# torognes/vsearch

Measured on AMD Instinct MI355X. Metric: GCUPS (useful DP cells/s of the search16 global-alignment path: DP + traceback + CIGAR), higher is better.
Workload: dtype int16

## Files before the change

include/vsx.h:

```cpp
#ifndef VSX_H
#define VSX_H

#include <stddef.h>
#include <stdint.h>

#ifdef __cplusplus
extern "C" {
#endif

#define VSX_API_VERSION 1000
#define VSX_SCORE_SENTINEL 32767

#define VSX_OK         0
#define VSX_EINVAL    -1
#define VSX_ENODEVICE -2
#define VSX_ENOMEM    -3
#define VSX_EHIP      -4

typedef struct vsx_ctx vsx_ctx;
typedef struct vsx_seqset vsx_seqset;
typedef struct vsx_plan vsx_plan;

typedef struct vsx_scoring {
  int64_t match;
  int64_t mismatch;
  int64_t gap_open_query_left;
  int64_t gap_open_target_left;
  int64_t gap_open_query_interior;
  int64_t gap_open_target_interior;
  int64_t gap_open_query_right;
  int64_t gap_open_target_right;
  int64_t gap_ext_query_left;
  int64_t gap_ext_target_left;
  int64_t gap_ext_query_interior;
  int64_t gap_ext_target_interior;
  int64_t gap_ext_query_right;
  int64_t gap_ext_target_right;
  int32_t n_mismatch;
} vsx_scoring;

typedef struct vsx_results {
  uint64_t   n_pairs;
  int16_t  * score;
  uint16_t * aligned;
  uint16_t * matches;
  uint16_t * mismatches;
  uint16_t * gaps;
  uint64_t * cigar_off;
  char     * cigar_blob;
  uint64_t   cigar_bytes;
  uint8_t  * verdict;
} vsx_results;

#define VSX_VERDICT_UNDECIDED 0
#define VSX_VERDICT_ACCEPTED  1
#define VSX_VERDICT_WEAK      2
#define VSX_VERDICT_REJECTED  3
typedef struct vsx_filter {
  int32_t iddef;
  int32_t leftjust, rightjust;
  int32_t pad;
  double  id, weak_id, maxid, mid, query_cov, target_cov;
  int64_t maxsubs, maxgaps, mincols, maxdiffs;
} vsx_filter;
int vsx_plan_set_filter(vsx_plan * plan, const vsx_filter * f);

typedef struct vsx_timing {
  float    forward_ms;
  float    traceback_ms;
  float    total_ms;
  uint32_t forward_launches;
  uint32_t traceback_launches;
  uint64_t cells;
  uint64_t dir_bytes;
} vsx_timing;

typedef struct vsx_plan_info {
  uint64_t tasks;
  uint64_t tasks_tilted;
  uint64_t tasks_tracked;
  uint32_t rows_dominant;
  uint32_t chunks;
  uint64_t tasks_max3;
  uint64_t tasks_sparse;
  uint64_t waves;
  uint64_t tasks_pair;
} vsx_plan_info;

const char * vsx_version_string(void);
int vsx_device_count(void);
const char * vsx_last_error(void);

int vsx_create(vsx_ctx ** out, const vsx_scoring * scoring, int device);
void vsx_destroy(vsx_ctx * ctx);


int vsx_seqset_create(vsx_ctx * ctx, vsx_seqset ** out, uint64_t n,
                      const char * blob, uint64_t blob_bytes,
                      const uint64_t * offsets, const uint32_t * lengths);
int vsx_seqset_create_from_device(vsx_ctx * ctx, vsx_seqset ** out, uint64_t n,
                                  const void * d_blob, uint64_t blob_bytes,
                                  const uint64_t * offsets, const uint32_t * lengths);
int vsx_seqset_create_both_strands(vsx_ctx * ctx, vsx_seqset ** out, uint64_t n,
                                   const char * blob, uint64_t blob_bytes,
                                   const uint64_t * offsets, const uint32_t * lengths);
void vsx_seqset_destroy(vsx_seqset * s);
uint64_t vsx_seqset_count(const vsx_seqset * s);

int vsx_plan_create(vsx_ctx * ctx, vsx_plan ** out,
                    const vsx_seqset * queries, const vsx_seqset * targets,
                    uint64_t n_pairs, const uint32_t * qidx, const uint32_t * tidx,
                    uint64_t dir_budget_bytes);
int vsx_plan_run(vsx_plan * plan);
int vsx_plan_sync(vsx_plan * plan, vsx_timing * timing );
int vsx_plan_fetch(vsx_plan * plan, vsx_results * out);
int vsx_plan_describe(const vsx_plan * plan, vsx_plan_info * info);
#define VSX_HIT_RECORD_BYTES 24
int vsx_plan_export_hits(vsx_plan * plan, void * d_dst, uint64_t dst_bytes);
int vsx_plan_export_runs(vsx_plan * plan, void * d_dst, uint64_t dst_bytes, uint64_t * n_runs);
int64_t vsx_cigar_from_runs(const uint32_t * runs, uint32_t n, char * dst, uint64_t cap);
void vsx_plan_destroy(vsx_plan * plan);

int vsx_align_pairs_filtered(vsx_ctx * ctx, const vsx_seqset * queries, const vsx_seqset * targets,
                             uint64_t n_pairs, const uint32_t * qidx, const uint32_t * tidx,
                             const vsx_filter * filter, vsx_results * out);
int vsx_align_pairs(vsx_ctx * ctx, const vsx_seqset * queries, const vsx_seqset * targets,
                    uint64_t n_pairs, const uint32_t * qidx, const uint32_t * tidx,
                    vsx_results * out);
void vsx_results_free(vsx_results * r);

typedef struct vsx_ranked {
  uint64_t   n_pairs, n_hits;
  uint32_t * pair;
  int16_t  * score;
  uint16_t * aligned, * matches, * mismatches, * gaps;
  uint8_t  * verdict;
  double   * id;
  uint64_t * cigar_off;
  char     * cigar_blob;
  uint64_t   cigar_bytes;
  uint64_t   n_undecided;
  uint32_t * undecided;
} vsx_ranked;
int vsx_align_pairs_ranked(vsx_ctx * ctx, const vsx_seqset * queries, const vsx_seqset * targets,
                           uint64_t n_pairs, const uint32_t * qidx, const uint32_t * tidx,
                           const vsx_filter * filter, int keep_weak, vsx_ranked * out);
void vsx_ranked_free(vsx_ranked * r);

#ifdef __cplusplus
}
#endif
#endif
```

profiles/valu_budget.py:

```python
#!/usr/bin/env python3
import argparse
import collections
import os
import re
import shutil
import subprocess
import sys
import tempfile

LLVM = "/opt/rocm/llvm/bin"
ROOT = os.path.dirname(os.path.dirname(os.path.abspath(__file__)))


def mangled(args):
    a = [x.strip() for x in args.split(",")]
    enc = "".join(("Li%sE" % x) if x.lstrip("-").isdigit() else ("Lb%dE" % (x == "true")) for x in a)
    return "_Z18vsx_forward_kernelI" + enc + "Ev12VsxDevParamsPK7VsxTaskPKhS5_PjP15HIP_vector_typeIjLj2EEP10VsxSlotOutj"


def extract(lib, sym, tmp):
    shutil.copy(lib, os.path.join(tmp, "lib.so"))
    subprocess.run([LLVM + "/llvm-objdump", "--offloading", "lib.so"], cwd=tmp, capture_output=True, check=True)
    for f in sorted(os.listdir(tmp)):
        if "gfx950" not in f:
            continue
        p = os.path.join(tmp, f)
        syms = subprocess.run([LLVM + "/llvm-readelf", "-s", "--wide", p], capture_output=True, text=True).stdout
        if (" " + sym + "\n") in syms:
            return p, syms
    sys.exit("kernel %s not found in %s" % (sym, lib))


def meta(syms, sym):
    out = {}
    for k in ("num_vgpr", "numbered_sgpr", "private_seg_size"):
        m = re.search(r"\s([0-9a-f]+)\s+0\s+NOTYPE\s+LOCAL\s+DEFAULT\s+ABS\s+" + re.escape(sym) + r"\." + k + r"\n", syms)
        out[k] = int(m.group(1), 16) if m else None
    m = re.search(r"\s([0-9a-f]+)\s+(\d+)\s+FUNC\s+\S+\s+\S+\s+\S+\s+" + re.escape(sym) + r"\n", syms)
    out["start"], out["size"] = int(m.group(1), 16), int(m.group(2))
    return out


def disasm(co, sym, start):
    txt = subprocess.run([LLVM + "/llvm-objdump", "-d", "--mcpu=gfx950", "--disassemble-symbols=" + sym, co],
                         capture_output=True, text=True, check=True).stdout
    ins = []
    for line in txt.splitlines():
        m = re.match(r"\s+(\S+)\s*(.*?)\s*//\s*([0-9A-F]+):", line)
        if not m:
            continue
        op, rest, addr = m.group(1), m.group(2), int(m.group(3), 16) - start
        t = re.search(r"<" + re.escape(sym) + r"\+0x([0-9a-f]+)>", line)
        ins.append((addr, op, rest, int(t.group(1), 16) if t else None))
    return ins


def is_valu(op):
    return op.startswith("v_")


def category(op, rest):
    if op in ("v_pk_maximum3_f16", "v_pk_max_u16", "v_subrev_u32_e32", "v_sub_u32_e32", "v_subrev_u32_e64", "v_sub_u32_e64"):
        return "row body"
    if op == "v_mov_b32_dpp":
        return "DPP hand-overs (feed, H, F)"
    if op == "v_add_u32_sdwa":
        return "profile row addresses"
    if op in ("v_pk_ashrrev_i16", "v_bfi_b32"):
        return "leave-column tracking"
    if op in ("v_lshl_add_u32", "v_lshlrev_b32_e32", "v_or_b32_e32", "v_and_or_b32") and "s" in rest.split(",")[1]:
        return "feed-slot addresses"
    if op in ("v_lshl_add_u64", "v_add_co_u32_e32", "v_addc_co_u32_e32", "v_mad_u64_u32"):
        return "checkpoint addresses"
    if op == "v_mov_b32_e32":
        return "register copies"
    return None


def budget(body, R, S):
    c = collections.Counter()
    quota = {"v_perm_b32": R * S, "v_add_u32_e32": R * S}
    npk = sum(1 for op, _ in body if op == "v_pk_sub_i16")
    nashr = sum(1 for op, _ in body if op == "v_pk_ashrrev_i16")
    pk = [("row body", S), ("last row's own e / hf subtractions", 2 * S), ("leave-column tracking", nashr)]
    for op, rest in body:
        if not is_valu(op):
            continue
        k = category(op, rest)
        if k is None and op in quota:
            if op == "v_add_u32_e32" and re.search(r"0x(1|2)000(1|2)\b", rest):
                k = "leave-column tracking"
            elif quota[op] > 0:
                quota[op] -= 1
                k = "row body"
            else:
                k = "checkpoint pack" if op == "v_perm_b32" else "other"
        if k is None and op == "v_pk_sub_i16":
            for i, (name, n) in enumerate(pk):
                if n > 0:
                    pk[i] = (name, n - 1)
                    k = name
                    break
            else:
                k = "checkpoint pack"
        c[k or "other"] += 1
    return c, npk


def main():
    ap = argparse.ArgumentParser()
    ap.add_argument("--lib", default=os.path.join(ROOT, "vsearch_amd", "libvsx.so"))
    ap.add_argument("--kernel", default="16,true,false,true,true,true,1,false,true", help="template arguments of vsx_forward_kernel")
    ap.add_argument("--rows", type=int, default=None, help="R (default: the first template argument)")
    ap.add_argument("--loop", type=int, default=None, help="loop index to budget (default: most v_pk_maximum3_f16)")
    ap.add_argument("--ops", action="store_true", help="print the opcode histogram of the loop too")
    a = ap.parse_args()
    R = a.rows or int(a.kernel.split(",")[0])
    sym = mangled(a.kernel)
    tmp = tempfile.mkdtemp(prefix="vsx_budget_")
    try:
        co, syms = extract(a.lib, sym, tmp)
        md = meta(syms, sym)
        ins = disasm(co, sym, md["start"])
    finally:
        shutil.rmtree(tmp, ignore_errors=True)
    print("vsx_forward_kernel<%s>  (%s)" % (a.kernel, os.path.relpath(a.lib, ROOT) if a.lib.startswith(ROOT) else a.lib))
    print("  code %d B, %d instructions, %d VALU;  VGPR %s  SGPR %s  scratch %s B" % (
        md["size"], len(ins), sum(is_valu(op) for _, op, _, _ in ins), md["num_vgpr"], md["numbered_sgpr"], md["private_seg_size"]))
    idx = {addr: k for k, (addr, _, _, _) in enumerate(ins)}
    heads = collections.OrderedDict()
    for k, (addr, op, _, tgt) in enumerate(ins):
        if op.startswith("s_branch") or op.startswith("s_cbranch"):
            if tgt is not None and tgt <= addr and tgt in idx:
                h = idx[tgt]
                heads.setdefault(h, []).append(k)
    loops = []
    for h, bs in heads.items():
        first_back, last = min(bs), max(bs)
        main_path = set(range(h, first_back + 1))
        for k in range(h, first_back + 1):
            addr, op, _, tgt = ins[k]
            if op.startswith("s_cbranch") and tgt is not None and tgt > addr and tgt in idx and idx[tgt] <= first_back + 1:
                for j in range(k + 1, idx[tgt]):
                    main_path.discard(j)
        cond = [j for j in range(h, last + 1) if j not in main_path]
        mp = sorted(main_path)
        loops.append(dict(head=h, end=last, main=mp, cond=cond,
                          max3=sum(1 for j in mp if ins[j][1] == "v_pk_maximum3_f16"),
                          valu_main=sum(1 for j in mp if is_valu(ins[j][1])), valu_cond=sum(1 for j in cond if is_valu(ins[j][1]))))
    print("  loops (offset range: VALU on the always-taken path + in branch-guarded regions, v_pk_maximum3_f16):")
    for n, L in enumerate(loops):
        print("    [%d] +0x%04x..+0x%04x: %4d + %4d VALU, %3d max3" % (n, ins[L["head"]][0], ins[L["end"]][0], L["valu_main"], L["valu_cond"], L["max3"]))
    if not loops:
        return
    n = a.loop if a.loop is not None else max(range(len(loops)), key=lambda i: (loops[i]["max3"], -i))
    L = loops[n]
    S = max(1, round(L["max3"] / R))
    body = [(ins[j][1], ins[j][2]) for j in L["main"]]
    cond = [(ins[j][1], ins[j][2]) for j in L["cond"]]
    cm, _ = budget(body, R, S)
    per_step = L["valu_main"] / S + L["valu_cond"] / 16.0
    print("  loop [%d]: %d steps per iteration (R = %d)" % (n, S, R))
    print("    VALU per two steps, always-taken path: %.1f" % (2.0 * L["valu_main"] / S))
    print("    VALU in branch-guarded regions (once per 16 steps): %d" % L["valu_cond"])
    print("    VALU per 16-step block: %.0f   per step: %.2f   (row body %d per step = %.1f %%)" % (
        16 * per_step, per_step, 6 * R, 100.0 * 6 * R / per_step))
    print("    per step, by category (always-taken path / S, + branch-guarded / 16):")
    order = ["row body", "DPP hand-overs (feed, H, F)", "profile row addresses", "feed-slot addresses", "last row's own e / hf subtractions",
             "leave-column tracking", "checkpoint pack", "checkpoint addresses", "register copies", "other"]
    for k in order:
        v = cm.get(k, 0) / S
        if v:
            print("      %-38s %6.2f" % (k, v))
    if L["valu_cond"]:
        print("      %-38s %6.2f  (%d VALU / 16)" % ("16-step block boundary (guarded)", L["valu_cond"] / 16.0, L["valu_cond"]))
    if a.ops:
        for name, lst in (("always-taken path", body), ("branch-guarded", cond)):
            h = collections.Counter(op for op, _ in lst if is_valu(op))
            print("    %s opcodes: %s" % (name, ", ".join("%s %d" % kv for kv in h.most_common())))


if __name__ == "__main__":
    main()
```

vsearch_amd/_lib.py:

```python
import ctypes as C
import os

HERE = os.path.dirname(os.path.abspath(__file__))
LIB_PATH = os.environ.get("VSX_LIBRARY") or os.path.join(HERE, "libvsx.so")

VSX_OK, VSX_EINVAL, VSX_ENODEVICE, VSX_ENOMEM, VSX_EHIP = 0, -1, -2, -3, -4
SENTINEL = 32767

SYMBOLS = [
    "vsx_version_string", "vsx_device_count", "vsx_last_error", "vsx_create", "vsx_destroy",
    "vsx_seqset_create", "vsx_seqset_create_both_strands", "vsx_seqset_create_from_device", "vsx_seqset_destroy", "vsx_seqset_count",
    "vsx_plan_create", "vsx_plan_run", "vsx_plan_sync", "vsx_plan_fetch", "vsx_plan_export_hits", "vsx_plan_export_runs",
    "vsx_cigar_from_runs", "vsx_plan_destroy",
    "vsx_align_pairs", "vsx_align_pairs_filtered", "vsx_align_pairs_ranked", "vsx_ranked_free", "vsx_plan_set_filter", "vsx_results_free", "vsx_plan_describe",
]
SEARCH_SYMBOLS = ["vsx_search_opts_default", "vsx_searcher_create", "vsx_searcher_destroy", "vsx_searcher_db_text", "vsx_search_batch",
                  "vsx_search_batch_meta", "vsx_searcher_set_meta",
                  "vsx_hits_free", "vsx_search_candidates", "vsx_search_candidates_batch", "vsx_candidates_free", "vsx_lma_align", "vsx_allpairs_block", "vsx_allpairs_rows", "vsx_allpairs_stream", "vsx_cluster_fast", "vsx_cluster_out_free", "vsx_msa", "vsx_msa_out_free",
                  "vsx_msa_device", "vsx_msa_device_batch", "vsx_dust_mask", "vsx_abundance_ratio_cmp",
                  "vsx_multi_searcher_create", "vsx_multi_searcher_destroy", "vsx_multi_searcher_devices", "vsx_multi_searcher_replica",
                  "vsx_multi_search_batch", "vsx_multi_allpairs"]


class Candidates(C.Structure):
    _fields_ = [("n_queries", C.c_uint64), ("start", C.POINTER(C.c_uint64)), ("target", C.POINTER(C.c_uint32)),
                ("count", C.POINTER(C.c_uint32)), ("seconds", C.c_double), ("kernel_ms", C.c_double),
                ("index_build_ms", C.c_double), ("index_postings", C.c_uint64), ("postings_streamed", C.c_uint64),
                ("bytes_streamed", C.c_uint64)]


class SearchOpts(C.Structure):
    _fields_ = [("id", C.c_double), ("weak_id", C.c_double), ("maxaccepts", C.c_int64), ("maxrejects", C.c_int64),
                ("wordlength", C.c_int64), ("minwordmatches", C.c_int64), ("iddef", C.c_int32), ("soft_mask", C.c_int32),
                ("maxsubs", C.c_int64), ("maxgaps", C.c_int64), ("mincols", C.c_int64), ("maxdiffs", C.c_int64),
                ("query_cov", C.c_double), ("target_cov", C.c_double), ("maxid", C.c_double), ("mid", C.c_double),
                ("leftjust", C.c_int32), ("rightjust", C.c_int32),
                ("minqt", C.c_double), ("maxqt", C.c_double), ("minsl", C.c_double), ("maxsl", C.c_double),
                ("idprefix", C.c_int64), ("idsuffix", C.c_int64), ("selfid", C.c_int32), ("threads", C.c_int32),
                ("window", C.c_int64), ("gap_infinite", C.c_uint32), ("strand_both", C.c_uint32),
                ("maxqsize", C.c_int64), ("mintsize", C.c_int64), ("minsizeratio", C.c_double), ("maxsizeratio", C.c_double),
                ("self", C.c_int32), ("sizeorder", C.c_int32), ("cluster_unoise", C.c_int32), ("qmask", C.c_int32),
                ("unoise_alpha", C.c_double), ("hardmask", C.c_int32)]


class SeqMeta(C.Structure):
    _fields_ = [("abundance", C.POINTER(C.c_uint64)), ("label", C.POINTER(C.c_char_p))]


class Hit(C.Structure):
    _fields_ = [("query", C.c_uint32), ("target", C.c_uint32), ("count", C.c_uint32),
                ("accepted", C.c_uint8), ("weak", C.c_uint8), ("used_fallback", C.c_uint8), ("strand", C.c_uint8),
                ("nwscore", C.c_int32), ("nwdiff", C.c_int32), ("nwgaps", C.c_int32), ("nwindels", C.c_int32),
                ("nwalignmentlength", C.c_int32), ("matches", C.c_int32), ("mismatches", C.c_int32),
                ("internal_alignmentlength", C.c_int32), ("internal_gaps", C.c_int32), ("internal_indels", C.c_int32),
                ("trim_q_left", C.c_int32), ("trim_q_right", C.c_int32), ("trim_t_left", C.c_int32), ("trim_t_right", C.c_int32),
                ("shortest", C.c_int32), ("longest", C.c_int32),
                ("nwid", C.c_double), ("id", C.c_double), ("id0", C.c_double), ("id1", C.c_double), ("id2", C.c_double),
                ("id3", C.c_double), ("id4", C.c_double), ("cigar_off", C.c_uint64)]


class Hits(C.Structure):
    _fields_ = [("n_queries", C.c_uint64), ("n_hits", C.c_uint64), ("first", C.POINTER(C.c_uint64)),
                ("hit", C.POINTER(Hit)), ("cigar_blob", C.POINTER(C.c_char)), ("cigar_bytes", C.c_uint64),
                ("pairs_aligned", C.c_uint64), ("cells_aligned", C.c_uint64), ("stages", C.c_uint64),
                ("sentinel_pairs", C.c_uint64), ("seconds_kmer", C.c_double), ("seconds_align", C.c_double),
                ("seconds_total", C.c_double)]


class Scoring(C.Structure):
    _fields_ = [(n, C.c_int64) for n in (
        "match", "mismatch", "gap_open_query_left", "gap_open_target_left", "gap_open_query_interior",
        "gap_open_target_interior", "gap_open_query_right", "gap_open_target_right",
        "gap_ext_query_left", "gap_ext_target_left", "gap_ext_query_interior", "gap_ext_target_interior",
        "gap_ext_query_right", "gap_ext_target_right")] + [("n_mismatch", C.c_int32)]


class Results(C.Structure):
    _fields_ = [("n_pairs", C.c_uint64), ("score", C.POINTER(C.c_int16)), ("aligned", C.POINTER(C.c_uint16)),
                ("matches", C.POINTER(C.c_uint16)), ("mismatches", C.POINTER(C.c_uint16)),
                ("gaps", C.POINTER(C.c_uint16)), ("cigar_off", C.POINTER(C.c_uint64)),
                ("cigar_blob", C.POINTER(C.c_char)), ("cigar_bytes", C.c_uint64), ("verdict", C.POINTER(C.c_uint8))]


class Ranked(C.Structure):
    _fields_ = [("n_pairs", C.c_uint64), ("n_hits", C.c_uint64), ("pair", C.POINTER(C.c_uint32)), ("score", C.POINTER(C.c_int16)),
                ("aligned", C.POINTER(C.c_uint16)), ("matches", C.POINTER(C.c_uint16)), ("mismatches", C.POINTER(C.c_uint16)),
                ("gaps", C.POINTER(C.c_uint16)), ("verdict", C.POINTER(C.c_uint8)), ("id", C.POINTER(C.c_double)),
                ("cigar_off", C.POINTER(C.c_uint64)), ("cigar_blob", C.POINTER(C.c_char)), ("cigar_bytes", C.c_uint64),
                ("n_undecided", C.c_uint64), ("undecided", C.POINTER(C.c_uint32))]


class Filter(C.Structure):
    _fields_ = [("iddef", C.c_int32), ("leftjust", C.c_int32), ("rightjust", C.c_int32), ("pad", C.c_int32),
                ("id", C.c_double), ("weak_id", C.c_double), ("maxid", C.c_double), ("mid", C.c_double),
                ("query_cov", C.c_double), ("target_cov", C.c_double),
                ("maxsubs", C.c_int64), ("maxgaps", C.c_int64), ("mincols", C.c_int64), ("maxdiffs", C.c_int64)]


class PlanInfo(C.Structure):
    _fields_ = [("tasks", C.c_uint64), ("tasks_tilted", C.c_uint64), ("tasks_tracked", C.c_uint64),
                ("rows_dominant", C.c_uint32), ("chunks", C.c_uint32), ("tasks_max3", C.c_uint64),
                ("tasks_sparse", C.c_uint64), ("waves", C.c_uint64), ("tasks_pair", C.c_uint64)]


class Timing(C.Structure):
    _fields_ = [("forward_ms", C.c_float), ("traceback_ms", C.c_float), ("total_ms", C.c_float),
                ("forward_launches", C.c_uint32), ("traceback_launches", C.c_uint32),
                ("cells", C.c_uint64), ("dir_bytes", C.c_uint64)]


class ClusterOut(C.Structure):
    _fields_ = [("n", C.c_uint64), ("n_clusters", C.c_uint64), ("clusterno", C.POINTER(C.c_uint32)), ("hits", Hits)]


class MsaOut(C.Structure):
    _fields_ = [("alnlen", C.c_uint64), ("n_rows", C.c_uint64), ("conslen", C.c_uint64), ("rows", C.POINTER(C.c_char)),
                ("consensus", C.POINTER(C.c_char)), ("profile", C.POINTER(C.c_uint64))]


_lib = None


def load():
    global _lib
    if _lib is not None:
        return _lib
    if not os.path.exists(LIB_PATH):
        raise ImportError(
            f"{LIB_PATH} not found: build the HIP extension first (python -c 'import __graft_entry__ as g; "
            "g.build()' or make -C vsearch_amd/csrc). vsearch_amd has no CPU fallback.")
    lib = C.CDLL(LIB_PATH)
    vp = C.c_void_p
    lib.vsx_version_string.restype = C.c_char_p
    lib.vsx_last_error.restype = C.c_char_p
    lib.vsx_device_count.restype = C.c_int
    lib.vsx_create.argtypes = [C.POINTER(vp), C.POINTER(Scoring), C.c_int]
    lib.vsx_destroy.argtypes = [vp]
    lib.vsx_destroy.restype = None
    lib.vsx_seqset_create.argtypes = [vp, C.POINTER(vp), C.c_uint64, vp, C.c_uint64, vp, vp]
    lib.vsx_seqset_create_both_strands.argtypes = [vp, C.POINTER(vp), C.c_uint64, vp, C.c_uint64, vp, vp]
    lib.vsx_seqset_create_from_device.argtypes = [vp, C.POINTER(vp), C.c_uint64, vp, C.c_uint64, vp, vp]
    lib.vsx_seqset_destroy.argtypes = [vp]
    lib.vsx_seqset_destroy.restype = None
    lib.vsx_seqset_count.argtypes = [vp]
    lib.vsx_seqset_count.restype = C.c_uint64
    lib.vsx_plan_create.argtypes = [vp, C.POINTER(vp), vp, vp, C.c_uint64, vp, vp, C.c_uint64]
    lib.vsx_plan_run.argtypes = [vp]
    lib.vsx_plan_sync.argtypes = [vp, C.POINTER(Timing)]
    lib.vsx_plan_fetch.argtypes = [vp, C.POINTER(Results)]
    lib.vsx_plan_export_hits.argtypes = [vp, vp, C.c_uint64]
    lib.vsx_plan_export_runs.argtypes = [vp, vp, C.c_uint64, C.POINTER(C.c_uint64)]
    lib.vsx_cigar_from_runs.argtypes = [vp, C.c_uint32, vp, C.c_uint64]
    lib.vsx_cigar_from_runs.restype = C.c_int64
    lib.vsx_plan_destroy.argtypes = [vp]
    lib.vsx_plan_destroy.restype = None
    lib.vsx_plan_describe.argtypes = [vp, C.POINTER(PlanInfo)]
    lib.vsx_align_pairs.argtypes = [vp, vp, vp, C.c_uint64, vp, vp, C.POINTER(Results)]
    lib.vsx_align_pairs_filtered.argtypes = [vp, vp, vp, C.c_uint64, vp, vp, C.POINTER(Filter), C.POINTER(Results)]
    lib.vsx_align_pairs_ranked.argtypes = [vp, vp, vp, C.c_uint64, vp, vp, C.POINTER(Filter), C.c_int, C.POINTER(Ranked)]
    lib.vsx_ranked_free.argtypes = [C.POINTER(Ranked)]
    lib.vsx_ranked_free.restype = None
    lib.vsx_plan_set_filter.argtypes = [vp, C.POINTER(Filter)]
    lib.vsx_results_free.argtypes = [C.POINTER(Results)]
    lib.vsx_results_free.restype = None
    lib.vsx_search_opts_default.argtypes = [C.POINTER(SearchOpts)]
    lib.vsx_search_opts_default.restype = None
    lib.vsx_searcher_create.argtypes = [vp, C.POINTER(vp), C.POINTER(SearchOpts), C.c_uint64, vp, C.c_uint64, vp, vp]
    lib.vsx_searcher_destroy.argtypes = [vp]
    lib.vsx_searcher_destroy.restype = None
    lib.vsx_search_batch.argtypes = [vp, C.c_uint64, vp, C.c_uint64, vp, vp, C.POINTER(Hits)]
    lib.vsx_search_batch_meta.argtypes = [vp, C.c_uint64, vp, C.c_uint64, vp, vp, C.POINTER(SeqMeta), C.POINTER(Hits)]
    lib.vsx_searcher_set_meta.argtypes = [vp, C.POINTER(SeqMeta)]
    lib.vsx_hits_free.argtypes = [C.POINTER(Hits)]
    lib.vsx_hits_free.restype = None
    lib.vsx_search_candidates.argtypes = [vp, C.c_char_p, C.c_uint32, vp, vp, C.c_uint64]
    lib.vsx_search_candidates.restype = C.c_int64
    lib.vsx_search_candidates_batch.argtypes = [vp, C.c_int32, C.c_uint64, vp, C.c_uint64, vp, vp, C.POINTER(Candidates)]
    lib.vsx_candidates_free.argtypes = [C.POINTER(Candidates)]
    lib.vsx_candidates_free.restype = None
    lib.vsx_allpairs_block.argtypes = [vp, C.c_int32, C.c_uint64, C.c_uint64, C.POINTER(Hits)]
    lib.vsx_allpairs_rows.argtypes = [vp, C.c_int32, vp, C.c_uint64, C.POINTER(Hits)]
    lib.vsx_allpairs_stream.argtypes = [vp, C.c_int32, C.c_uint64, C.c_uint64, C.c_uint64, vp, vp]
    lib.vsx_dust_mask.argtypes = [vp, C.c_uint64, vp, vp, C.c_int32]
    lib.vsx_multi_searcher_create.argtypes = [C.POINTER(vp), vp, vp, C.c_int32, vp, C.c_uint64, vp, C.c_uint64, vp, vp, vp]
    lib.vsx_multi_searcher_destroy.argtypes = [vp]
    lib.vsx_multi_searcher_destroy.restype = None
    lib.vsx_multi_searcher_devices.argtypes = [vp]
    lib.vsx_multi_searcher_devices.restype = C.c_int32
    lib.vsx_multi_searcher_replica.argtypes = [vp, C.c_int32]
    lib.vsx_multi_searcher_replica.restype = vp
    lib.vsx_multi_search_batch.argtypes = [vp, C.c_uint64, vp, C.c_uint64, vp, vp, vp, C.POINTER(Hits)]
    lib.vsx_multi_allpairs.argtypes = [vp, C.c_int32, C.c_uint64, C.c_uint64, C.POINTER(Hits)]
    lib.vsx_abundance_ratio_cmp.argtypes = [C.c_int64, C.c_double, C.c_int64]
    lib.vsx_abundance_ratio_cmp.restype = C.c_int
    lib.vsx_cluster_fast.argtypes = [vp, C.c_uint64, C.POINTER(ClusterOut)]
    lib.vsx_cluster_out_free.argtypes = [C.POINTER(ClusterOut)]
    lib.vsx_cluster_out_free.restype = None
    lib.vsx_msa.argtypes = [C.c_uint32, vp, vp, vp, vp, C.POINTER(MsaOut)]
    lib.vsx_msa_device.argtypes = [vp, C.c_uint32, vp, vp, vp, vp, C.POINTER(MsaOut)]
    lib.vsx_msa_device_batch.argtypes = [vp, C.c_uint32, vp, vp, vp, vp, vp, C.POINTER(MsaOut)]
    lib.vsx_msa_out_free.argtypes = [C.POINTER(MsaOut)]
    lib.vsx_msa_out_free.restype = None
    lib.vsx_lma_align.argtypes = [C.POINTER(Scoring), C.c_char_p, C.c_uint64, C.c_char_p, C.c_uint64] + \
        [C.POINTER(C.c_int64)] * 5 + [C.POINTER(vp)]
    _lib = lib
    return lib


class VsxError(RuntimeError):
    def __init__(self, code, where):
        msg = load().vsx_last_error().decode(errors="replace")
        super().__init__(f"{where}: error {code}: {msg}")
        self.code = code


def check(code, where):
    if code != VSX_OK:
        raise VsxError(code, where)
```

vsearch_amd/csrc/ubench_valu.hip:

```cpp
#include <hip/hip_runtime.h>
#include <cstdio>
#include <cstdlib>

#define CK(x) do { hipError_t e = (x); if (e != hipSuccess) { fprintf(stderr, "%s:%d %s\n", __FILE__, __LINE__, hipGetErrorString(e)); exit(1); } } while (0)

#define BODY16(INS) \
  asm volatile(INS(%0) INS(%1) INS(%2) INS(%3) INS(%4) INS(%5) INS(%6) INS(%7) \
               INS(%8) INS(%9) INS(%10) INS(%11) INS(%12) INS(%13) INS(%14) INS(%15) \
               : "+v"(r[0]), "+v"(r[1]), "+v"(r[2]), "+v"(r[3]), "+v"(r[4]), "+v"(r[5]), "+v"(r[6]), "+v"(r[7]), \
                 "+v"(r[8]), "+v"(r[9]), "+v"(r[10]), "+v"(r[11]), "+v"(r[12]), "+v"(r[13]), "+v"(r[14]), "+v"(r[15]) \
               : "v"(b), "v"(c) : "vcc")

#define I_PK_ADD(x)   "v_pk_add_i16 " #x ", " #x ", %16 clamp\n"
#define I_PK_SUB(x)   "v_pk_sub_i16 " #x ", " #x ", %16 clamp\n"
#define I_PK_MAX(x)   "v_pk_max_i16 " #x ", " #x ", %16\n"
#define I_PK_MIN(x)   "v_pk_min_u16 " #x ", " #x ", %16\n"
#define I_PK_LSHR(x)  "v_pk_lshrrev_b16 " #x ", 1, " #x "\n"
#define I_PK_ASHR(x)  "v_pk_ashrrev_i16 " #x ", 15, " #x "\n"
#define I_PK_MAD(x)   "v_pk_mad_u16 " #x ", " #x ", %16, %17\n"
#define I_PK_MUL(x)   "v_pk_mul_lo_u16 " #x ", " #x ", %16\n"
#define I_XOR(x)      "v_xor_b32 " #x ", " #x ", %16\n"
#define I_ANDOR(x)    "v_and_or_b32 " #x ", " #x ", %16, %17\n"
#define I_LSHR(x)     "v_lshrrev_b32 " #x ", 1, " #x "\n"
#define I_BFI(x)      "v_bfi_b32 " #x ", %16, " #x ", %17\n"
#define I_LSHLOR(x)   "v_lshl_or_b32 " #x ", " #x ", 1, %16\n"
#define I_ADD32(x)    "v_add_u32 " #x ", " #x ", %16\n"
#define I_ADD3(x)     "v_add3_u32 " #x ", " #x ", %16, %17\n"
#define I_MAX32(x)    "v_max_i32 " #x ", " #x ", %16\n"
#define I_MAX3_32(x)  "v_max3_i32 " #x ", " #x ", %16, %17\n"
#define I_ADD16(x)    "v_add_i16 " #x ", " #x ", %16 clamp\n"
#define I_MAX16(x)    "v_max_i16 " #x ", " #x ", %16\n"
#define I_MAX3_16(x)  "v_max3_i16 " #x ", " #x ", %16, %17\n"
#define I_DPP(x)      "v_mov_b32_dpp " #x ", %16 row_shr:1 row_mask:0xf bank_mask:0xf\n"
#define I_PERM(x)     "v_perm_b32 " #x ", " #x ", %16, %17\n"
#define I_CNDMASK(x)  "v_cndmask_b32 " #x ", " #x ", %16, vcc\n"
#define I_CMP16(x)    "v_cmp_gt_i16 vcc, " #x ", %16\n"
#define I_MOV(x)      "v_mov_b32 " #x ", %16\n"
#define I_ALIGNBIT(x) "v_alignbit_b32 " #x ", " #x ", %16, 1\n"
#define I_DOT2(x)     "v_dot2_u32_u16 " #x ", " #x ", %16, %17\n"
#define I_SAD16(x)    "v_sad_u16 " #x ", " #x ", %16, %17\n"
#define I_MAD_I32_I16(x) "v_mad_i32_i16 " #x ", " #x ", %16, %17\n"

#define I_SUB32(x)    "v_sub_u32 " #x ", " #x ", %16\n"
#define I_SUBREV32(x) "v_subrev_u32 " #x ", " #x ", %16\n"
#define I_MIN32(x)    "v_min_i32 " #x ", " #x ", %16\n"
#define I_MAXU32(x)   "v_max_u32 " #x ", " #x ", %16\n"
#define I_ASHR32(x)   "v_ashrrev_i32 " #x ", 31, " #x "\n"
#define I_AND32(x)    "v_and_b32 " #x ", " #x ", %16\n"
#define I_OR32(x)     "v_or_b32 " #x ", " #x ", %16\n"
#define I_LSHL32(x)   "v_lshlrev_b32 " #x ", 1, " #x "\n"
#define I_ADDCO(x)    "v_add_co_u32 " #x ", vcc, " #x ", %16\n"
#define I_ADDC(x)     "v_addc_co_u32 " #x ", vcc, " #x ", %16, vcc\n"
#define I_MIN16(x)    "v_min_i16 " #x ", " #x ", %16\n"
#define I_ADDU16(x)   "v_add_u16 " #x ", " #x ", %16\n"
#define I_SUBU16(x)   "v_sub_u16 " #x ", " #x ", %16\n"
#define I_CMP32(x)    "v_cmp_lt_i32 vcc, " #x ", %16\n"
#define I_LSHLADD(x)  "v_lshl_add_u32 " #x ", " #x ", 1, %16\n"
#define I_MADU24(x)   "v_mad_u32_u24 " #x ", " #x ", %16, %17\n"
#define I_MULU24(x)   "v_mul_u32_u24 " #x ", " #x ", %16\n"
#define I_SUBI32C(x)  "v_sub_i32 " #x ", " #x ", %16 clamp\n"
#define I_MED3(x)     "v_med3_i32 " #x ", " #x ", %16, %17\n"
#define I_BFE(x)      "v_bfe_u32 " #x ", " #x ", 8, 8\n"
#define I_ADDSDWA(x)  "v_add_u32_sdwa " #x ", " #x ", %16 dst_sel:DWORD dst_unused:UNUSED_PAD src0_sel:DWORD src1_sel:BYTE_1\n"
#define I_MAX16SDWA(x) "v_max_i16_sdwa " #x ", " #x ", %16 dst_sel:WORD_1 dst_unused:UNUSED_PRESERVE src0_sel:WORD_1 src1_sel:WORD_1\n"
#define I_MOVDPP(x)   "v_mov_b32_dpp " #x ", %16 row_ror:15 row_mask:0xf bank_mask:0xf\n"
#define I_ADDDPP(x)   "v_add_u32_dpp " #x ", %16, " #x " row_shr:1 row_mask:0xf bank_mask:0xf\n"
#define I_MOV64(x)    "v_mov_b64 %18, %19\n"
#define I_PKMAX3F(x)  "v_pk_maximum3_f16 " #x ", " #x ", %16, %17\n"
#define I_PKMAXU(x)   "v_pk_max_u16 " #x ", " #x ", %16\n"
#define I_MIXAM(x)    "v_add_u32 " #x ", " #x ", %16\n" "v_pk_max_u16 " #x ", " #x ", %17\n"
#define I_MIXAM3(x)   "v_add_u32 " #x ", " #x ", %16\n" "v_pk_maximum3_f16 " #x ", " #x ", %16, %17\n"

#define DEFK(NAME, INS) \
  __global__ void __launch_bounds__(256) NAME(int iters, int * out, int seed) { \
    int r[16]; int b = seed + threadIdx.x, c = seed * 7 + 3; \
    for (int i = 0; i < 16; ++i) r[i] = i * 1315423911 + threadIdx.x; \
    for (int it = 0; it < iters; ++it) { \
      BODY16(INS); BODY16(INS); BODY16(INS); BODY16(INS); BODY16(INS); BODY16(INS); BODY16(INS); BODY16(INS); } \
    int acc = 0; for (int i = 0; i < 16; ++i) acc ^= r[i]; \
    if (acc == 0x12345678) out[0] = acc; }

DEFK(k_pk_add, I_PK_ADD)
DEFK(k_pk_sub, I_PK_SUB)
DEFK(k_pk_max, I_PK_MAX)
DEFK(k_pk_min, I_PK_MIN)
DEFK(k_pk_lshr, I_PK_LSHR)
DEFK(k_pk_ashr, I_PK_ASHR)
DEFK(k_pk_mad, I_PK_MAD)
DEFK(k_pk_mul, I_PK_MUL)
DEFK(k_xor, I_XOR)
DEFK(k_andor, I_ANDOR)
DEFK(k_lshr, I_LSHR)
DEFK(k_bfi, I_BFI)
DEFK(k_lshlor, I_LSHLOR)
DEFK(k_add32, I_ADD32)
DEFK(k_add3, I_ADD3)
DEFK(k_max32, I_MAX32)
DEFK(k_max3_32, I_MAX3_32)
DEFK(k_add16, I_ADD16)
DEFK(k_max16, I_MAX16)
DEFK(k_max3_16, I_MAX3_16)
DEFK(k_dpp, I_DPP)
DEFK(k_perm, I_PERM)
DEFK(k_cndmask, I_CNDMASK)
DEFK(k_cmp16, I_CMP16)
DEFK(k_mov, I_MOV)
DEFK(k_alignbit, I_ALIGNBIT)
DEFK(k_dot2, I_DOT2)
DEFK(k_sad16, I_SAD16)
DEFK(k_mad_i32_i16, I_MAD_I32_I16)

DEFK(k2_sub32, I_SUB32)
DEFK(k2_subrev32, I_SUBREV32)
DEFK(k2_min32, I_MIN32)
DEFK(k2_maxu32, I_MAXU32)
DEFK(k2_ashr32, I_ASHR32)
DEFK(k2_and32, I_AND32)
DEFK(k2_or32, I_OR32)
DEFK(k2_lshl32, I_LSHL32)
DEFK(k2_addco, I_ADDCO)
DEFK(k2_addc, I_ADDC)
DEFK(k2_min16, I_MIN16)
DEFK(k2_addu16, I_ADDU16)
DEFK(k2_subu16, I_SUBU16)
DEFK(k2_cmp32, I_CMP32)
DEFK(k2_lshladd, I_LSHLADD)
DEFK(k2_madu24, I_MADU24)
DEFK(k2_mulu24, I_MULU24)
DEFK(k2_subi32c, I_SUBI32C)
DEFK(k2_med3, I_MED3)
DEFK(k2_bfe, I_BFE)
DEFK(k2_addsdwa, I_ADDSDWA)
DEFK(k2_max16sdwa, I_MAX16SDWA)
DEFK(k2_movdpp, I_MOVDPP)
DEFK(k2_adddpp, I_ADDDPP)
DEFK(k3_pkmax3f, I_PKMAX3F)
DEFK(k3_pkmaxu, I_PKMAXU)
DEFK(k3_mix_add_max, I_MIXAM)
DEFK(k3_mix_add_max3, I_MIXAM3)

template <int MODE>
__global__ void __launch_bounds__(256) k_rowbody(int iters, int * out, int seed)
{
  typedef unsigned short us2 __attribute__((ext_vector_type(2)));
  auto pmaxu = [](unsigned a, unsigned b) -> unsigned {
    return __builtin_bit_cast(unsigned, __builtin_elementwise_max(__builtin_bit_cast(us2, a), __builtin_bit_cast(us2, b)));
  };
  unsigned H[16], E[16], pa[4], pb[4];
  for (int i = 0; i < 16; ++i) { H[i] = 0x80008000u + (unsigned) (i * 77 + (int) threadIdx.x); E[i] = 0x80008000u - (unsigned) (i * 13 + seed); }
  for (int i = 0; i < 4; ++i) { pa[i] = 0x06000600u + (unsigned) seed * (unsigned) i; pb[i] = 0x00060006u + (unsigned) i; }
  unsigned F = 0x80008000u, diag = 0x80008000u;
  const unsigned go = 0x00120012u;
  for (int it = 0; it < iters; ++it)
    {
      unsigned Hd = diag;
#pragma unroll
      for (int r = 0; r < 16; ++r)
        {
          const unsigned V = __builtin_amdgcn_perm(pb[r >> 2], pa[r >> 2], 0x0C040C00u + 0x00010001u * (unsigned) (r & 3));
          const unsigned h0 = Hd + V;
          if (MODE == 1)
            {
              const unsigned m = pmaxu(h0, E[r]);
              const unsigned mg = m - go;
              const unsigned h2 = pmaxu(m, F);
              F = pmaxu(F, mg);
              Hd = H[r];
              H[r] = h2;
              E[r] = pmaxu(E[r], h2 - go);
            }
          else
            {
              const unsigned Fin = (MODE == 2) ? go + (unsigned) r : F;
              const unsigned h1 = pmaxu(h0, Fin);
              const unsigned h2 = pmaxu(h1, E[r]);
              Hd = H[r];
              H[r] = h2;
              const unsigned he = h2 - go;
              if (MODE == 2) F ^= pmaxu(Fin, he); else F = pmaxu(F, he);
              E[r] = pmaxu(E[r], he);
            }
        }
      diag = H[15] + (unsigned) it;
      pa[it & 3] ^= F;
    }
  unsigned acc = F;
  for (int i = 0; i < 16; ++i) acc ^= H[i] ^ E[i];
  if (acc == 0x12345678u) out[0] = (int) acc;
}

typedef void (*kfn)(int, int *, int);

static void run(const char * name, kfn k, int waves_per_simd)
{
  int * out; CK(hipMalloc(&out, 4));
  const int iters = 1000;
  const int blocks = 256 * waves_per_simd;
  hipEvent_t e0, e1; CK(hipEventCreate(&e0)); CK(hipEventCreate(&e1));
  hipLaunchKernelGGL(k, dim3(blocks), dim3(256), 0, 0, 10, out, 1);
  CK(hipDeviceSynchronize());
  CK(hipEventRecord(e0));
  hipLaunchKernelGGL(k, dim3(blocks), dim3(256), 0, 0, iters, out, 1);
  CK(hipEventRecord(e1));
  CK(hipEventSynchronize(e1));
  float ms; CK(hipEventElapsedTime(&ms, e0, e1));
  double instr = (double) iters * 8 * 16 * blocks * 256;
  double rate = instr / (ms * 1e-3) / 1e12;
  printf("%-22s w/simd=%d %8.3f ms  %7.2f T lane-instr/s  (%.1f lanes/clk/SIMD @2.4GHz)\n", name, waves_per_simd, ms, rate,
         rate * 1e12 / (1024 * 2.4e9));
  CK(hipFree(out));
}

static void run_rowbody(int waves_per_simd, int mode)
{
  int * out; CK(hipMalloc(&out, 4));
  const int iters = 20000;
  const int blocks = 256 * waves_per_simd;
  hipEvent_t e0, e1; CK(hipEventCreate(&e0)); CK(hipEventCreate(&e1));
  auto launch = [&](int n) {
    if (mode == 0) hipLaunchKernelGGL(k_rowbody<0>, dim3(blocks), dim3(256), 0, 0, n, out, 1);
    if (mode == 1) hipLaunchKernelGGL(k_rowbody<1>, dim3(blocks), dim3(256), 0, 0, n, out, 1);
    if (mode == 2) hipLaunchKernelGGL(k_rowbody<2>, dim3(blocks), dim3(256), 0, 0, n, out, 1);
  };
  launch(10);
  CK(hipDeviceSynchronize());
  CK(hipEventRecord(e0));
  launch(iters);
  CK(hipEventRecord(e1));
  CK(hipEventSynchronize(e1));
  float ms; CK(hipEventElapsedTime(&ms, e0, e1));
  const int per_row = (mode == 1) ? 8 : ((mode == 2) ? 8 : 7);
  const double wave_instr_per_simd = (double) iters * 16 * per_row * waves_per_simd;
  const double cycles = ms * 1e-3 * 2.4e9;
  const char * what[] = {"kernel row body, F chain of 4 per row (perm, add, 2 max, sub, 2 max)", "F chain of 1 per row (perm, add, max, sub, 2 max, sub, max)",
                         "no chain (+1 xor per row)"};
  printf("%-70s x 16 rows  w/simd=%d %8.3f ms  %.3f cycles per instruction  %.1f cycles per lane-row\n",
         what[mode], waves_per_simd, ms, cycles / wave_instr_per_simd, per_row * cycles / wave_instr_per_simd);
  CK(hipFree(out));
}

int main()
{
  hipDeviceProp_t p; CK(hipGetDeviceProperties(&p, 0));
  printf("device %s  CUs %d  clock %d kHz  arch %s\n", p.name, p.multiProcessorCount, p.clockRate, p.gcnArchName);
  if (getenv("UB_ROWBODY")) { for (int m = 0; m < 3; ++m) for (int w = 1; w <= 8; w *= 2) run_rowbody(w, m); run_rowbody(3, 0); return 0; }
#define R(NAME) run(#NAME, NAME, 4);
  if (getenv("UB_MAX3")) { R(k3_pkmaxu) R(k3_pkmax3f) R(k_add32) R(k3_mix_add_max) R(k3_mix_add_max3) return 0; }
  if (getenv("UB_NEW")) { R(k2_sub32) R(k2_subrev32) R(k2_min32) R(k2_maxu32) R(k2_ashr32) R(k2_and32) R(k2_or32) R(k2_lshl32) R(k2_addco) R(k2_addc) R(k2_min16) R(k2_addu16) R(k2_subu16) R(k2_cmp32) R(k2_lshladd) R(k2_madu24) R(k2_mulu24) R(k2_subi32c) R(k2_med3) R(k2_bfe) R(k2_addsdwa) R(k2_max16sdwa) R(k2_movdpp) R(k2_adddpp) return 0; }
  R(k_pk_add) R(k_pk_sub) R(k_pk_max) R(k_pk_min) R(k_pk_lshr) R(k_pk_ashr) R(k_pk_mad) R(k_pk_mul)
  R(k_xor) R(k_andor) R(k_lshr) R(k_bfi) R(k_lshlor) R(k_add32) R(k_add3) R(k_max32) R(k_max3_32)
  R(k_add16) R(k_max16) R(k_max3_16) R(k_dpp) R(k_perm) R(k_cndmask) R(k_cmp16) R(k_mov) R(k_alignbit)
  R(k_dot2) R(k_sad16) R(k_mad_i32_i16)
  if (getenv("UB_NEW")) { R(k2_sub32) R(k2_subrev32) R(k2_min32) R(k2_maxu32) R(k2_ashr32) R(k2_and32) R(k2_or32) R(k2_lshl32) R(k2_addco) R(k2_addc) R(k2_min16) R(k2_addu16) R(k2_subu16) R(k2_cmp32) R(k2_lshladd) R(k2_madu24) R(k2_mulu24) R(k2_subi32c) R(k2_med3) R(k2_bfe) R(k2_addsdwa) R(k2_max16sdwa) R(k2_movdpp) R(k2_adddpp) return 0; }
  run("k_pk_add", k_pk_add, 1); run("k_pk_add", k_pk_add, 2); run("k_pk_add", k_pk_add, 8);
  run("k_xor", k_xor, 1); run("k_xor", k_xor, 2); run("k_xor", k_xor, 8);
  return 0;
}
```

vsearch_amd/csrc/vsx_device.hip:

```cpp
#include <hip/hip_runtime.h>
#include <type_traits>
#include <cstdlib>
#include <atomic>
#include "vsx_internal.h"

typedef unsigned int u32;
typedef unsigned int u32x4 __attribute__((ext_vector_type(4)));
typedef unsigned int u32x3 __attribute__((ext_vector_type(3)));
typedef short s2 __attribute__((ext_vector_type(2)));
typedef unsigned short us2 __attribute__((ext_vector_type(2)));

#define DEV __device__ __forceinline__
struct __attribute__((aligned(4))) Pair2 { unsigned int x, y; };

#define SIGN2 0x80008000u

DEV s2 S2(u32 x) { return __builtin_bit_cast(s2, x); }
DEV us2 U2(u32 x) { return __builtin_bit_cast(us2, x); }
DEV u32 UI(s2 x) { return __builtin_bit_cast(u32, x); }
DEV u32 UI(us2 x) { return __builtin_bit_cast(u32, x); }

DEV u32 sadd(u32 a, u32 b) { return UI(__builtin_elementwise_add_sat(S2(a), S2(b))); }
DEV u32 ssub(u32 a, u32 b) { return UI(__builtin_elementwise_sub_sat(S2(a), S2(b))); }
DEV u32 pmax(u32 a, u32 b) { return UI(__builtin_elementwise_max(S2(a), S2(b))); }
DEV u32 pmin(u32 a, u32 b) { return UI(__builtin_elementwise_min(S2(a), S2(b))); }
DEV u32 pminu(u32 a, u32 b) { return UI(__builtin_elementwise_min(U2(a), U2(b))); }
DEV u32 pmaxu(u32 a, u32 b) { return UI(__builtin_elementwise_max(U2(a), U2(b))); }
DEV u32 psubw(u32 a, u32 b) { return UI((us2) (U2(a) - U2(b))); }
DEV u32 pmad(u32 a, u32 b, u32 c) { return UI((us2) (U2(a) * U2(b) + U2(c))); }
DEV u32 pashr15(u32 a) { return UI((s2) (S2(a) >> (s2){15, 15})); }
DEV u32 bfi(u32 mask, u32 a, u32 b) { return (a & mask) | (b & ~mask); }
DEV u32 a_pk_minu(u32 a, u32 b) { u32 r; asm("v_pk_min_u16 %0, %1, %2" : "=v"(r) : "v"(a), "s"(b)); return r; }
DEV u32 a_pk_mad(u32 a, u32 b, u32 c) { u32 r; asm("v_pk_mad_u16 %0, %1, %2, %3" : "=v"(r) : "v"(a), "v"(b), "s"(c)); return r; }
DEV u32 a_bfi(u32 mask, u32 a, u32 b) { u32 r; asm("v_bfi_b32 %0, %1, %2, %3" : "=v"(r) : "s"(mask), "v"(a), "v"(b)); return r; }
DEV u32 a_bfi_v(u32 mask, u32 a, u32 b) { u32 r; asm("v_bfi_b32 %0, %1, %2, %3" : "=v"(r) : "v"(mask), "v"(a), "v"(b)); return r; }
DEV u32 a_bfi_vs(u32 mask, u32 a, u32 b) { u32 r; asm("v_bfi_b32 %0, %1, %2, %3" : "=v"(r) : "v"(mask), "v"(a), "s"(b)); return r; }
DEV u32 a_lshr1(u32 a) { u32 r; asm("v_lshrrev_b32 %0, 1, %1" : "=v"(r) : "v"(a)); return r; }
DEV u32 a_pk_ashr15(u32 a) { u32 r; asm("v_pk_ashrrev_i16 %0, 15, %1 op_sel_hi:[0,1]" : "=v"(r) : "v"(a)); return r; }
DEV u32 funnel(u32 acc, u32 d) { return a_bfi(SIGN2, d, a_lshr1(acc)); }
DEV u32 pack16(int v) { const u32 x = (u32) v & 0xffffu; return x | (x << 16); }

DEV u32 dpp_shr1(u32 feed, u32 src) { return (u32) __builtin_amdgcn_update_dpp((int) feed, (int) src, 0x111, 0xF, 0xF, false); }
DEV u32 dpp_rol1(u32 src) { return (u32) __builtin_amdgcn_update_dpp((int) src, (int) src, 0x12F, 0xF, 0xF, false); }


#define VSX_COLCK_G 64
#define VSX_COLCK_DW(R_, lane_, block_) ((((size_t) ((lane_) / VSX_COLCK_G) * (size_t) ((2 * (R_)) / 4) + (size_t) (block_)) * VSX_COLCK_G + (size_t) ((lane_) % VSX_COLCK_G)) * 4)
#define VSX_RB 1
#define VSX_ROWCK_PAIR_DW(TILT_) ((TILT_) ? 192 : 256)
#define VSX_COLCK_NBH(RT_) (((RT_) + ((RT_) + 1) / 2 + 3) / 4)
#define VSX_COLCK_NB(R_, TILT_) ((TILT_) ? (VSX_MID(R_, true) ? 2 * VSX_COLCK_NBH((R_) / 2) : ((R_) + ((R_) + 1) / 2 + 3) / 4) : (2 * (R_)) / 4)
#ifndef VSX_CK_TASKMAJOR
#define VSX_CK_TASKMAJOR 1
#endif
#define VSX_CK_SLOT(TILT_, g_, l_) (((TILT_) && VSX_CK_TASKMAJOR) ? ((l_) * 4 + (g_)) : ((g_) * 16 + (l_)))
#ifndef VSX_COLCK_CG
#define VSX_COLCK_CG 64
#endif
#define VSX_CKT_BLOCK_DW 768
#define VSX_COLCK_NCHUNK(R_) ((VSX_COLCK_NB(R_, true) + 2) / 3)
#define VSX_COLCK_CDW(NB_, lane_, block_) ((((size_t) ((lane_) / VSX_COLCK_CG) * (size_t) (NB_) + (size_t) (block_)) * VSX_COLCK_CG + (size_t) ((lane_) % VSX_COLCK_CG)) * 4)
#ifndef VSX_FWD_WAVES
#define VSX_FWD_WAVES(R_, TILT_) ((R_) <= 16 ? 4 : ((R_) <= 24 ? 3 : 2))
#endif
#ifndef VSX_FWD_WAVES_ONE
#define VSX_FWD_WAVES_ONE(R_, TILT_) ((R_) == 26 ? 3 : VSX_FWD_WAVES(R_, TILT_))
#endif
typedef _Float16 f16x2 __attribute__((ext_vector_type(2)));
DEV u32 pk_max3_bits(u32 a, u32 b, u32 c)
{
  const f16x2 x = __builtin_bit_cast(f16x2, a), y = __builtin_bit_cast(f16x2, b), z = __builtin_bit_cast(f16x2, c);
  return __builtin_bit_cast(u32, __builtin_elementwise_maximum(__builtin_elementwise_maximum(x, y), z));
}
#ifndef VSX_FWD_WAVES_NQ
#define VSX_FWD_WAVES_NQ(R_, NQ_) ((NQ_) == 4 ? 2 : ((R_) <= 24 ? 3 : 2))
#endif
template <int R, bool GENERIC, bool TRACK, bool CKPT, bool TILT = false, bool MAX3 = false, int NQ = 1, bool PAIR = false, bool ONE = false>
__global__ void __launch_bounds__(PAIR ? 256 : 64) __attribute__((amdgpu_waves_per_eu(NQ == 1 ? (ONE ? VSX_FWD_WAVES_ONE(R, TILT) : VSX_FWD_WAVES(R, TILT)) : VSX_FWD_WAVES_NQ(R, NQ), 8)))
vsx_forward_kernel(const VsxDevParams P, const VsxTask * __restrict__ tasks,
                   const uint8_t * __restrict__ qc, const uint8_t * __restrict__ tc,
                   u32 * __restrict__ dir, uint2 * strip, VsxSlotOut * __restrict__ slot_out, const u32 ntasks)
{
  constexpr int ND = (R + 3) / 4;
  constexpr bool TOPPAD = CKPT && GENERIC && !TRACK;
  static_assert(!TILT || TOPPAD, "tilted coordinates exist for the TOPPAD class only");
  const int tl = TILT ? P.tilt : 0;
  static_assert(!MAX3 || TILT, "the MAX3 arithmetic is a sub-class of TILT");
  constexpr u32 BIAS16 = MAX3 ? 0x3E00u : (TILT ? 0x8000u : 0u);
  constexpr u32 BIAS = BIAS16 * 0x10001u;
  constexpr u32 CK_REBIAS = 0u;
  auto bpack = [](int v) -> u32 { return pack16(v + (int) BIAS16); };
  auto vadd = [](u32 a, u32 b) -> u32 { return TILT ? a + b : sadd(a, b); };
  auto vsubk = [](u32 a, u32 b) -> u32 { return TILT ? a - b : ssub(a, b); };
  auto vsub = [](u32 a, u32 b) -> u32 { return TILT ? psubw(a, b) : ssub(a, b); };
  auto vmax = [](u32 a, u32 b) -> u32 { return TILT ? pmaxu(a, b) : pmax(a, b); };
  constexpr bool MIDCK = VSX_MID(R, TILT);
  constexpr int RT = MIDCK ? R / 2 : R;
  constexpr bool CKST = TILT && (VSX_CKT != 0);
  static_assert(!(MAX3 && CKST), "the transposed A/B layout predates the MAX3 class");
  constexpr bool QPL = TILT && (VSX_QPL != 0);
  constexpr bool QP8 = CKST || QPL;
  constexpr int RP = (R + 3) & ~3;
  static_assert(NQ == 1 || NQ == 2 || NQ == 4, "tasks per wave");
  static_assert(NQ == 1 || (TILT && VSX_QPL != 0 && !VSX_CKT), "the sparse-task classes exist for the look-ahead TILT kernels only");
  static_assert(!PAIR || (NQ == 1 && TILT && VSX_QPL != 0 && VSX_FEED2 != 0 && !VSX_CKT && GENERIC), "the pair-profile classes extend the FEED2 look-ahead kernels");
  constexpr int WPB = PAIR ? 4 : 1;
  constexpr int QPBYTES = 16 * 16 * RP;
  constexpr int RPP = ((RP / 4) & 1) ? RP : RP + 4;
  __shared__ __attribute__((aligned(16))) u32 PPf[PAIR ? 16 * 16 * RPP : 4];
  __shared__ __attribute__((aligned(16))) int16_t QP[(GENERIC && !PAIR) ? (QP8 ? (NQ * QPBYTES) / 2 : 16 * 16 * R) : 8];
  uint8_t * const QPb = reinterpret_cast<uint8_t *>(QP);
  __shared__ __attribute__((aligned(16))) u32 RS[CKST ? 64 * 12 : 4];
  constexpr int FSZ = (TILT && VSX_QPL ? 2 : 1) * 4 * 16;
  __shared__ uint4 FEED4a[FSZ * WPB];
  __shared__ u32 FEEDFa[FSZ * WPB], FEEDN[GENERIC ? 1 : 4 * 16];
  constexpr bool FEED2 = (VSX_FEED2 != 0) && TOPPAD && (TILT && (VSX_QPL != 0));
  __shared__ uint2 FEEDBa[FEED2 ? 2 * 4 * 16 * WPB : 1];

  const int wv = PAIR ? __builtin_amdgcn_readfirstlane((int) (threadIdx.x >> 6)) : 0;
  uint4 * const FEED4 = FEED4a + wv * FSZ;
  u32 * const FEEDF = FEEDFa + wv * FSZ;
  uint2 * const FEEDB = FEEDBa + (FEED2 ? wv * FSZ : 0);
  const int lane = PAIR ? (int) (threadIdx.x & 63) : (int) threadIdx.x;
  const int gw = lane >> 4;
  constexpr int GPT = 4 / NQ;
  const int sq = (NQ == 1) ? 0 : gw / GPT;
  const int g = (NQ == 1) ? gw : gw % GPT;
  const int l = lane & 15;
  const u32 tix = PAIR ? blockIdx.x * 4u + (u32) wv : ((NQ == 1) ? blockIdx.x : blockIdx.x * (u32) NQ + (u32) sq);
  const bool sub_on = (NQ == 1 && !PAIR) ? true : (tix < ntasks);
  const VsxTask & T = tasks[sub_on ? tix : ntasks - 1];
  uint8_t * const QPl = reinterpret_cast<uint8_t *>(QP) + ((NQ == 1) ? 0 : sq * QPBYTES);

  const int Q = (int) T.qlen;
  const int total_lanes = (Q + R - 1) / R;
  const int rcnt0 = Q - (total_lanes - 1) * R;
  const int rc0 = __builtin_amdgcn_readfirstlane(rcnt0);
  static_assert(!PAIR || ONE, "the pair-profile classes are planned for single-strip queries only");
  const int nstrips = (NQ == 1 && !ONE) ? (total_lanes + 15) >> 4 : 1;
  const int steps = (NQ == 1) ? (int) T.steps : __builtin_amdgcn_readfirstlane((int) T.steps);

  const int DA = sub_on ? (int) T.tlen[2 * g] : 0;
  const int DB = sub_on ? (int) T.tlen[2 * g + 1] : 0;
  const int DpA = (DA + 3) & ~3;
  const int DpB = (DB + 3) & ~3;
  const int Dpg = DpA > DpB ? DpA : DpB;
  const uint8_t * __restrict__ tA = tc + T.toff[2 * g];
  const uint8_t * __restrict__ tB = tc + T.toff[2 * g + 1];
  const uint8_t * __restrict__ qq = qc + T.qoff;

  const u32 qrt_i_pk = pack16(P.qrt_i);
  u32 hmin = 0, hmax = 0;
  u32 score = 0;
  u32 lv1 = 0xFFFFFFFFu, leave = 0;

  for (int s = 0; s < nstrips; ++s)
    {
      const int L = 16 * s + l;
      const bool lane_on = (L < total_lanes) && (Dpg > 0);
      const bool first = (L == 0);
      const int pad = TOPPAD ? R - rcnt0 : 0;
      const int i0 = first ? -pad : rcnt0 + (L - 1) * R;

      if (GENERIC)
        {
          __syncthreads();
          if (PAIR)
            {
              for (int idx = (int) threadIdx.x; idx < 16 * 16 * RP; idx += 256)
                {
                  const int pr = idx / (16 * RP), row = idx % (16 * RP);
                  const int Lr = 16 * s + row / RP, rr = row % RP;
                  int va = 0, vb = 0;
                  if (rr < R)
                    {
                      if (Lr == 0 && rr < pad) va = vb = -P.top_step + 2 * tl;
                      else if (Lr < total_lanes)
                        {
                          const int gi = (Lr == 0) ? rr - pad : rcnt0 + (Lr - 1) * R + rr;
                          const int qs = (int) qq[gi];
                          va = P.matrix[(1 << (pr >> 2)) * 16 + qs];
                          vb = P.matrix[(1 << (pr & 3)) * 16 + qs];
                        }
                    }
                  PPf[(pr * 16 + row / RP) * RPP + rr] = ((u32) va & 0xffu) | (((u32) vb & 0xffu) << 16);
                }
            }
          else if (QP8)
            {
              constexpr int LPT = 64 / NQ;
              for (int idx = (NQ == 1) ? lane : lane % LPT; idx < 16 * 16 * RP; idx += LPT)
                {
                  const int code = idx / (16 * RP), row = idx % (16 * RP);
                  const int Lr = 16 * s + row / RP, rr = row % RP;
                  int v = 0;
                  if (rr < R)
                    {
                      if (Lr == 0 && rr < pad) v = -P.top_step + 2 * tl;
                      else if (Lr < total_lanes)
                        {
                          const int gi = (Lr == 0) ? rr - pad : rcnt0 + (Lr - 1) * R + rr;
                          v = P.matrix[code * 16 + (int) qq[gi]];
                        }
                    }
                  QPl[idx] = (uint8_t) v;
                }
            }
          else
          for (int idx = lane; idx < 16 * 16 * R; idx += 64)
            {
              const int code = idx / (16 * R), row = idx % (16 * R);
              const int Lr = 16 * s + row / R, rr = row % R;
              int v = 0;
              if (TOPPAD && Lr == 0 && rr < pad) v = -P.top_step + 2 * tl;
              else if (Lr < total_lanes && (TOPPAD || !(Lr == 0 && rr >= rcnt0)))
                {
                  const int gi = (Lr == 0) ? rr - pad : rcnt0 + (Lr - 1) * R + rr;
                  v = P.matrix[code * 16 + (int) qq[gi]];
                }
              QP[idx] = (int16_t) v;
            }
          __syncthreads();
        }

      u32 hprev[R];
      u32 hnext[R];
      u32 E[R];
      u32 ac[R];
#pragma unroll
      for (int r = 0; r < R; ++r)
        {
          int i = i0 + r;
          const bool dummy = TOPPAD && first && r < pad;
          if (i > Q - 1) i = Q - 1;
          if (i < 0) i = 0;
          const u32 a = qq[i];
          ac[r] = a | (a << 16);
          u32 hl = bpack(P.hleft[i]);
          u32 e0 = vsub(hl, (i < Q - 1) ? P.qrq_i_pk : P.qrq_r_pk);
          if (dummy)
            {
              const int sh = (r - pad - 1) * tl;
              hl = bpack(((r == pad - 1) ? 0 : -P.top_open) + sh);
              e0 = vsub(bpack(-P.top_open - P.top_step + sh), P.qrq_i_pk);
            }
          hprev[r] = hl;
          hnext[r] = hl;
          E[r] = e0;
        }
      u32 diag = first ? bpack(((TOPPAD && pad > 0) ? -P.top_open : 0) - (pad + 2) * tl) : bpack(P.hleft[i0 - 1]);
      const bool lastpos = (L == total_lanes - 1);
      const u32 qrq_last = lastpos ? P.qrq_r_pk : P.qrq_i_pk;
      const u32 rq_last = lastpos ? P.rq_r_pk : P.rq_i_pk;

      u32 sym = 0, nd = 0, qrt = 0, rt = 0;
      u32 symf = 0;
      u32 outH = 0, outF = 0;
      u32 f_sym = 0, f_nd = 0, f_qrt = 0, f_rt = 0, f_H = 0, f_F = 0;
      u32 rawA = 0, rawB = 0;
      int rawH = 0;
      uint2 rawS = make_uint2(0, 0);
      const uint2 * strip_in = strip + T.strip_off + (size_t) (((s + 1) & 1) * 4 + g) * (size_t) steps;
      uint2 * strip_outp = strip + T.strip_off + (size_t) ((s & 1) * 4 + g) * (size_t) steps;

      auto prefetch = [&](int blk) {
        const int c = 16 * blk + l;
        rawA = (c < DA) ? (u32) tA[c] : 0u;
        rawB = (c < DB) ? (u32) tB[c] : 0u;
        if (s == 0) rawH = P.htop[c];
        else if (c < Dpg) rawS = strip_in[c];
      };
      prefetch(0);

      auto build_feed = [&](int blk, auto lean_tag) __attribute__((always_inline)) {
              constexpr bool LEAN = FEED2 && decltype(lean_tag)::value;
              const int c = 16 * blk + l;
              if (LEAN)
                {
                  f_H = (s == 0) ? bpack(rawH - pad * tl) : rawS.x;
                  f_F = (s == 0) ? vsub(f_H, qrt_i_pk) : rawS.y;
                  const u32 f_off = PAIR ? (((rawA >> 1) - (rawA >> 3)) * 4u + ((rawB >> 1) - (rawB >> 3))) * (u32) (16 * RPP * 4)
                                         : (rawA * (u32) (16 * RP) | ((rawB * (u32) (16 * RP)) << 16));
                  FEED4[(blk & 1) * 64 + gw * 16 + l] = make_uint4(f_off, 0u, f_H, f_F);
                  prefetch(blk + 1);
                  return;
                }
              auto mne = [&](u32 code) -> int {
                const bool unamb = (code != 0) && ((code & (code - 1)) == 0);
                return unamb ? P.mismatch : ((P.n_mismatch && code == 15) ? P.mismatch : 0);
              };
              const u32 ndA = (u32) (mne(rawA) - P.match) & 0xffffu;
              const u32 ndB = (u32) (mne(rawB) - P.match) & 0xffffu;
              const u32 qA = (u32) ((c < DA - 1) ? P.qrt_i : P.qrt_r) & 0xffffu;
              const u32 qB = (u32) ((c < DB - 1) ? P.qrt_i : P.qrt_r) & 0xffffu;
              const u32 rA = (u32) ((c < DA - 1) ? P.rt_i : P.rt_r) & 0xffffu;
              const u32 rB = (u32) ((c < DB - 1) ? P.rt_i : P.rt_r) & 0xffffu;
              const u32 sA = rawA | ((c == DA - 1) ? 0x100u : 0u) | ((c < DpA) ? 0x200u : 0u);
              const u32 sB = rawB | ((c == DB - 1) ? 0x100u : 0u) | ((c < DpB) ? 0x200u : 0u);
              f_sym = sA | (sB << 16);
              f_nd = ndA | (ndB << 16);
              f_qrt = qA | (qB << 16);
              f_rt = rA | (rB << 16);
              if (s == 0)
                {
                  f_H = bpack(rawH - pad * tl);
                  f_F = vsub(f_H, f_qrt);
                }
              else
                {
                  f_H = rawS.x;
                  f_F = rawS.y;
                }
              const int fo = QPL ? (blk & 1) * 64 : 0;
              if (FEED2)
                {
                  const u32 f_off = PAIR ? (((rawA >> 1) - (rawA >> 3)) * 4u + ((rawB >> 1) - (rawB >> 3))) * (u32) (16 * RPP * 4)
                                         : (rawA * (u32) (16 * RP) | ((rawB * (u32) (16 * RP)) << 16));
                  FEED4[fo + gw * 16 + l] = make_uint4(f_off, f_sym, f_H, f_F);
                  FEEDB[fo + gw * 16 + l] = make_uint2(f_qrt, f_rt);
                }
              else
                {
                  FEED4[fo + gw * 16 + l] = make_uint4(f_sym, f_qrt, f_rt, f_H);
                  FEEDF[fo + gw * 16 + l] = f_F;
                }
              if (!GENERIC) FEEDN[gw * 16 + l] = f_nd;
              prefetch(blk + 1);
      };
      constexpr int PD = RP / 4;
      u32 profA[2][(QPL && !PAIR) ? PD : 1], profB[2][(QPL && !PAIR) ? PD : 1];
      auto load_profile = [&](u32 (&buf)[2][(QPL && !PAIR) ? PD : 1], u32 sy) __attribute__((always_inline)) {
        if (PAIR) return;
        const u32 cd = sy & 0x000F000Fu;
        constexpr int QPA = (RP % 16 == 0) ? 16 : ((RP % 8 == 0) ? 8 : 4);
        if (FEED2)
          {
            const uint8_t * pa = QPl + l * RP + (sy & 0xFFFFu);
            const uint8_t * pb = QPl + l * RP + (sy >> 16);
            constexpr int PDN = (QPL && !PAIR) ? PD : 1;
            if constexpr (PAIR) { }
            else if constexpr (QPA == 16)
              {
#pragma unroll
                for (int k = 0; k < PDN; k += 4)
                  {
                    const uint4 va = *reinterpret_cast<const uint4 *>(pa + 4 * k), vb = *reinterpret_cast<const uint4 *>(pb + 4 * k);
                    buf[0][k] = va.x; buf[0][k + 1] = va.y; buf[0][k + 2] = va.z; buf[0][k + 3] = va.w;
                    buf[1][k] = vb.x; buf[1][k + 1] = vb.y; buf[1][k + 2] = vb.z; buf[1][k + 3] = vb.w;
                  }
              }
            else if constexpr (QPA == 8)
              {
#pragma unroll
                for (int k = 0; k < PDN; k += 2)
                  {
                    const uint2 va = *reinterpret_cast<const uint2 *>(pa + 4 * k), vb = *reinterpret_cast<const uint2 *>(pb + 4 * k);
                    buf[0][k] = va.x; buf[0][k + 1] = va.y;
                    buf[1][k] = vb.x; buf[1][k + 1] = vb.y;
                  }
              }
            else
              {
#pragma unroll
                for (int k = 0; k < PDN; ++k)
                  { buf[0][k] = reinterpret_cast<const u32 *>(pa)[k]; buf[1][k] = reinterpret_cast<const u32 *>(pb)[k]; }
              }
            return;
          }
        const u32 * a = reinterpret_cast<const u32 *>(QPl + (cd & 0xFu) * (16 * RP) + l * RP);
        const u32 * b = reinterpret_cast<const u32 *>(QPl + (cd >> 16) * (16 * RP) + l * RP);
#pragma unroll
        for (int k = 0; k < ((QPL && !PAIR) ? PD : 1); ++k) { buf[0][k] = a[k]; buf[1][k] = b[k]; }
      };
      if (QPL)
        {
          build_feed(0, std::false_type {});
          sym = dpp_shr1(FEED4[gw * 16].x, 0u);
          load_profile(profA, sym);
        }

      const uint4 * const feed4_g = FEED4 + gw * 16;
      const u32 * const feedf_g = FEEDF + gw * 16;
      u32 pendH = 0, pendF = 0;
      u32 pendMH = 0, pendMF = 0, curMH = 0, curMF = 0;
      bool pend_on = false;
      const size_t ck_rowdw = ((((size_t) nstrips * steps + 1) & ~(size_t) 1) >> 1) * VSX_ROWCK_PAIR_DW(TILT);
      const size_t ck_nblk = ((size_t) steps + 15) >> 4;
      constexpr int CK_LANE_DW = TILT ? 3 : 4;
      constexpr size_t CK_COL_DW = TILT ? (size_t) 64 * 4 * VSX_COLCK_NB(R, true) : (size_t) 64 * (2 * R);
      const int ck_slot = VSX_CK_SLOT(TILT, gw, l);
      u32 * const rck_base = dir + T.dir_off + ((((size_t) s * steps) >> 1) * 64 + ck_slot) * CK_LANE_DW;
      u32 * const cck_base = dir + T.dir_off + ck_rowdw + (size_t) s * ck_nblk * CK_COL_DW;
      u32 * const mck_base = dir + T.dir_off + ck_rowdw + (size_t) nstrips * ck_nblk * CK_COL_DW
                             + ((((size_t) s * steps) >> 1) * 64 + ck_slot) * CK_LANE_DW;
      u32 * const rck_blk = dir + T.dir_off + (((size_t) s * steps) >> 3) * VSX_CKT_BLOCK_DW;
      u32 * const cck_blk = dir + T.dir_off + (((size_t) nstrips * steps) >> 3) * VSX_CKT_BLOCK_DW
                            + (size_t) s * ck_nblk * VSX_COLCK_NCHUNK(R) * VSX_CKT_BLOCK_DW;
      auto flush_block = [&](u32 * gdst) __attribute__((always_inline)) {
        __syncthreads();
#pragma unroll
        for (int k = 0; k < 3; ++k)
          {
            const u32x4 v = *reinterpret_cast<const u32x4 *>(RS + (k * 64 + lane) * 4);
            __builtin_nontemporal_store(v, reinterpret_cast<u32x4 *>(gdst + (k * 64 + lane) * 4));
          }
        __syncthreads();
      };

      auto step = [&](const int t, u32 (&hin)[R], u32 (&hout)[R], u32 (&pc)[2][(QPL && !PAIR) ? PD : 1], u32 (&pn)[2][(QPL && !PAIR) ? PD : 1],
                      auto interior_tag, auto odd_tag, auto steady_tag) __attribute__((always_inline)) {
          constexpr bool INTERIOR = decltype(interior_tag)::value;
          constexpr bool ODD = decltype(odd_tag)::value;
          constexpr bool STEADY = decltype(steady_tag)::value != 0;
          constexpr bool LEANFEED = decltype(steady_tag)::value == 2;
          u32 symn = 0;
          u32 pp[PAIR ? RP : 1];
          if (PAIR)
            {
              const u32 * ppa = PPf + (sym >> 2) + l * RPP;
#pragma unroll
              for (int k = 0; k < (PAIR ? RP : 0); k += 4)
                {
                  const uint4 v = *reinterpret_cast<const uint4 *>(ppa + k);
                  pp[k] = v.x; pp[k + 1] = v.y; pp[k + 2] = v.z; pp[k + 3] = v.w;
                }
            }
          if (QPL) { if ((t & 15) == 15) build_feed((t >> 4) + 1, std::integral_constant<bool, LEANFEED> {}); }
          else if ((t & 15) == 0) build_feed(t >> 4, std::false_type {});

          const int fo = QPL ? ((t >> 4) & 1) * 64 : 0;
          const u32 fslot = (u32) (fo + (t & 15));
          const uint4 fv = feed4_g[fslot];
          const u32 fF = FEED2 ? fv.w : feedf_g[fslot];
          if (QPL)
            {
              const int t1 = t + 1;
              symn = dpp_shr1(feed4_g[(u32) (((t1 >> 4) & 1) * 64 + (t1 & 15))].x, sym);
              load_profile(pn, symn);
            }
          else sym = dpp_shr1(fv.x, sym);
          if (!GENERIC) nd = dpp_shr1(FEEDN[gw * 16 + (t & 15)], nd);
          if (!INTERIOR)
            {
              if (FEED2)
                {
                  const uint2 fb = FEEDB[fo + gw * 16 + (t & 15)];
                  qrt = dpp_shr1(fb.x, qrt); rt = dpp_shr1(fb.y, rt);
                  symf = dpp_shr1(fv.y, symf);
                }
              else { qrt = dpp_shr1(fv.y, qrt); rt = dpp_shr1(fv.z, rt); }
            }
          const u32 inH = dpp_shr1(FEED2 ? fv.z : fv.w, outH);
          const u32 inF = dpp_shr1(fF, outF);

          const int j = t - l;
          const bool active = STEADY ? true : (lane_on && j >= 0 && j < Dpg);
          if (active)
            {
              const u32 code = sym & 0x000F000Fu;
              const int16_t * qpA = QP + (code & 0xFu) * (16 * R) + l * R;
              const int16_t * qpB = QP + (code >> 16) * (16 * R) + l * R;
              u32 pa = 0, pb = 0;
              u32 Hd = diag;
              u32 F = inF;
              u32 smn = 0x7FFF7FFFu, smx = 0x80008000u;
              u32 acc = 0, h2 = 0;
              u32 capH = 0, capF = 0, capmn = 0, capmx = 0;
              u32 dw[ND];
              u32 lastL = 0, lastEL = 0;
              u32 midH = 0, midF = 0;
              auto rows = [&](auto shared_tag) __attribute__((always_inline)) {
              constexpr bool SHARED = decltype(shared_tag)::value;
              constexpr bool LASTFAST = MAX3 && SHARED && CKPT;
#pragma unroll
              for (int r = 0; r < R; ++r)
                {
                  u32 V;
                  if (PAIR) V = pp[r];
                  else if (GENERIC && QP8)
                    {
                      if ((r & 3) == 0)
                        {
                          if (QPL) { pa = pc[0][r >> 2]; pb = pc[1][r >> 2]; }
                          else
                            {
                              pa = *reinterpret_cast<const u32 *>(QPb + (code & 0xFu) * (16 * RP) + l * RP + r);
                              pb = *reinterpret_cast<const u32 *>(QPb + (code >> 16) * (16 * RP) + l * RP + r);
                            }
                        }
                      V = __builtin_amdgcn_perm(pb, pa, 0x0C040C00u + 0x00010001u * (u32) (r & 3));
                    }
                  else if (GENERIC)
                    {
                      if (R % 2 == 0)
                        {
                          if ((r & 3) == 0 && r + 3 < R)
                            {
                              typedef typename std::conditional<R % 4 == 0, uint2, Pair2>::type Rows4;
                              const Rows4 va = *reinterpret_cast<const Rows4 *>(qpA + r);
                              const Rows4 vb = *reinterpret_cast<const Rows4 *>(qpB + r);
                              pa = va.x; pb = vb.x;
                              ac[r + 1] = va.y; ac[r + 2] = vb.y;
                            }
                          else if ((r & 3) == 0)
                            {
                              pa = *reinterpret_cast<const u32 *>(qpA + r);
                              pb = *reinterpret_cast<const u32 *>(qpB + r);
                            }
                          else if ((r & 3) == 2) { pa = ac[r - 1]; pb = ac[r]; }
                          V = (r & 1) ? __builtin_amdgcn_perm(pb, pa, 0x07060302u) : __builtin_amdgcn_perm(pb, pa, 0x05040100u);
                        }
                      else V = (u32) (uint16_t) qpA[r] | ((u32) (uint16_t) qpB[r] << 16);
                    }
                  else V = a_pk_mad(a_pk_minu(ac[r] ^ code, 0x00010001u), nd, P.match_pk);
                  const u32 h0 = vadd(Hd, V);
                  const bool ONE_MAX = MAX3 && (r < R - 1 || LASTFAST);
                  const u32 h1 = ONE_MAX ? 0u : vmax(h0, F);
                  h2 = ONE_MAX ? pk_max3_bits(h0, F, E[r]) : vmax(h1, E[r]);
                  if (TRACK) { smn = pmin(smn, h2); smx = pmax(smx, h2); }
                  Hd = hin[r];
                  hout[r] = h2;
                  const u32 qrq = (r == R - 1) ? qrq_last : P.qrq_i_pk;
                  const u32 rq = (r == R - 1) ? rq_last : P.rq_i_pk;
                  const u32 he = (r < R - 1) ? vsubk(h2, qrq) : vsub(h2, qrq);
                  const u32 hf = (SHARED && r < R - 1) ? he : vsub(h2, qrt);
                  const u32 f = (TILT && INTERIOR) ? F : vsub(F, rt);
                  const u32 e = (TILT && INTERIOR && r < R - 1) ? E[r] : vsub(E[r], rq);
                  if (CKPT && r == R - 1) { lastL = LASTFAST ? 0u : vsub(h1, E[r]); lastEL = vsub(he, e); }
                  if (!CKPT)
                    {
                      const u32 dU = ssub(h0, F);
                      const u32 dL = ssub(h1, E[r]);
                      const u32 dEU = ssub(hf, f);
                      const u32 dEL = ssub(he, e);
                      acc = funnel(funnel(funnel(funnel(acc, dU), dL), dEU), dEL);
                      if ((r & 3) == 3 || r == R - 1) dw[r >> 2] = acc;
                    }
                  F = vmax(f, hf);
                  E[r] = vmax(e, he);
                  if (MIDCK && r == RT - 1) { midH = h2; midF = F; }
                  if (!TOPPAD && __builtin_expect(rc0 == r + 1, 0)) { capH = h2; capF = F; capmn = smn; capmx = smx; }
                }
              };
              if (INTERIOR) rows(std::true_type {});
              else rows(std::false_type {});
              const u32 hl = (!TOPPAD && first) ? capH : h2;
              F = (!TOPPAD && first) ? capF : F;
              smn = (!TOPPAD && first) ? capmn : smn;
              smx = (!TOPPAD && first) ? capmx : smx;
              outH = hl;
              outF = F;
              diag = inH;
              if (CKPT)
                {
                  const u32 jpk = (u32) j | ((u32) j << 16);
                  if (!INTERIOR)
                    {
                      const u32 atlast = a_pk_ashr15((FEED2 ? symf : sym) << 7);
                      leave = a_bfi_v(atlast, a_bfi_v(a_pk_ashr15(lastL), lv1, jpk), leave);
                    }
                  const u32 lmask = a_pk_ashr15((MAX3 && INTERIOR) ? lastEL : (lastL | lastEL));
                  lv1 = STEADY ? a_bfi_vs(lmask, lv1, (u32) t * 0x00010001u) : a_bfi_v(lmask, lv1, jpk);
                }

              if (TRACK)
                {
                  const u32 vm = a_pk_ashr15(sym << 6);
                  hmin = pmin(hmin, a_bfi_v(vm, smn, 0x7FFF7FFFu));
                  hmax = pmax(hmax, a_bfi_v(vm, smx, 0x80008000u));
                }
              if (!INTERIOR)
                {
                  const u32 lm = a_pk_ashr15((FEED2 ? symf : sym) << 7);
                  score = a_bfi_v(lm, hl, score);
                }

              const size_t gt = (size_t) s * steps + t;
              if (CKPT)
                {
                  if (!ODD) { pendH = outH; pendF = outF; }
                  if (MIDCK) { if (!ODD) { pendMH = midH; pendMF = midF; } else { curMH = midH; curMF = midF; } }
                }
              else
                {
                  u32 * dp = dir + T.dir_off + (((gt >> 2) * 64 + lane) * 4 + (gt & 3)) * ND;
                  if (ND == 4) *reinterpret_cast<uint4 *>(dp) = make_uint4(dw[0], dw[1], dw[2], dw[3]);
                  else if (ND == 2) *reinterpret_cast<uint2 *>(dp) = make_uint2(dw[0], dw[1]);
                  else
                    {
#pragma unroll
                      for (int w = 0; w < ND; ++w) dp[w] = dw[w];
                    }
                }
              if (l == 15 && s + 1 < nstrips) strip_outp[j] = make_uint2(outH, outF);
            }
          if (CKPT && CKST)
            {
              if (!ODD) pend_on = active;
              else
                {
                  const u32 dpk = __builtin_amdgcn_perm(psubw(outH, outF), psubw(pendH, pendF), 0x06040200u);
                  u32 * rs = RS + ck_slot * 12;
                  const int i = t & 7;
                  *reinterpret_cast<uint2 *>(rs + (i - 1)) = make_uint2(pendH, outH);
                  rs[8 + (i >> 1)] = dpk;
                  if (i == 7) flush_block(rck_blk + (size_t) (t >> 3) * VSX_CKT_BLOCK_DW);
                }
            }
          else if (CKPT)
            {
              if (!ODD) pend_on = active;
              else if (pend_on || active)
                {
                  if (TILT && !CKST)
                    {
                      const size_t ckp = LEANFEED ? (size_t) ((t & ~15) >> 1) * 192 + (size_t) (((t & 15) >> 1) * 192) : (size_t) (t >> 1) * 192;
                      const u32 dpk = __builtin_amdgcn_perm(psubw(outH, outF), psubw(pendH, pendF), 0x06040200u);
                      __builtin_nontemporal_store((u32x3) {pendH + CK_REBIAS, outH + CK_REBIAS, dpk}, reinterpret_cast<u32x3 *>(rck_base + ckp));
                      if (MIDCK)
                        {
                          const u32 dpm = __builtin_amdgcn_perm(psubw(curMH, curMF), psubw(pendMH, pendMF), 0x06040200u);
                          __builtin_nontemporal_store((u32x3) {pendMH + CK_REBIAS, curMH + CK_REBIAS, dpm}, reinterpret_cast<u32x3 *>(mck_base + ckp));
                        }
                    }
                  else
                    __builtin_nontemporal_store((u32x4) {pendH, pendF, outH, outF}, reinterpret_cast<u32x4 *>(rck_base + (size_t) (t >> 1) * 256));
                }
            }
          if (CKPT && (t & 15) == 15)
            {
              u32 * cb = cck_base + (size_t) (t >> 4) * CK_COL_DW;
              if (TILT)
                {
                  constexpr int NF = R + (R + 1) / 2;
                  constexpr int NFH = RT + (RT + 1) / 2, ZH = 4 * VSX_COLCK_NBH(RT);
                  auto flatc = [&](int z) -> u32 {
                    if (MIDCK)
                      {
                        const int hh = z / ZH, zz = z % ZH, r00 = hh * RT;
                        if (zz < RT) return hout[r00 + zz] + CK_REBIAS;
                        if (zz < NFH)
                          {
                            const int r0 = r00 + 2 * (zz - RT), r1 = (r0 + 1 < r00 + RT) ? r0 + 1 : r0;
                            return __builtin_amdgcn_perm(psubw(hout[r1], E[r1]), psubw(hout[r0], E[r0]), 0x06040200u);
                          }
                        return 0u;
                      }
                    if (z < R) return hout[z] + CK_REBIAS;
                    if (z < NF)
                      {
                        const int r0 = 2 * (z - R), r1 = r0 + 1 < R ? r0 + 1 : r0;
                        return __builtin_amdgcn_perm(psubw(hout[r1], E[r1]), psubw(hout[r0], E[r0]), 0x06040200u);
                      }
                    return 0u;
                  };
                  if (CKST)
                    {
                      constexpr int NBC = VSX_COLCK_NB(R, true);
#pragma unroll
                      for (int c = 0; c < VSX_COLCK_NCHUNK(R); ++c)
                        {
#pragma unroll
                          for (int pc = 0; pc < 3; ++pc)
                            {
                              const int z = 4 * (3 * c + pc);
                              if (3 * c + pc < NBC)
                                *reinterpret_cast<u32x4 *>(RS + ck_slot * 12 + pc * 4) = (u32x4) {flatc(z), flatc(z + 1), flatc(z + 2), flatc(z + 3)};
                            }
// ... 1332 lines not shown
  u32 verdict = 0;
  double idv = 0.0;
  if (FL.enabled && nruns > 0) verdict = accept_verdict(FL, Q, D, (int) al, (int) ma, (int) mi, (int) ga, my[nruns - 1], my[0], &idv);
  if (verdict == 3u) nruns = 0;
  rank_note(FL, pair_ids[k], verdict, (int) so.score, idv);

  const unsigned long long base = atomicAdd(cursor, (unsigned long long) nruns);
  if (base + nruns <= runs_capacity)
    for (u32 x = 0; x < nruns; ++x) runs[base + x] = my[x];

  o.score = so.score;
  o.aligned = (uint16_t) al; o.matches = (uint16_t) ma; o.mismatches = (uint16_t) mi; o.gaps = (uint16_t) ga;
  o.pad = (uint16_t) verdict;
  o.nruns = nruns;
  o.run_off = base;
  out[pair_ids[k]] = o;
}

DEV u32 map4(u32 ch)
{
  const u32 c = ch | 0x20u;
  if (((ch | 0x20u) < 'a') || ((ch | 0x20u) > 'z') || ((ch & 0xC0u) != 0x40u)) return 0;
  switch (c)
    {
    case 'a': return 1;  case 'b': return 14; case 'c': return 2;  case 'd': return 13;
    case 'g': return 4;  case 'h': return 11; case 'k': return 12; case 'm': return 3;
    case 'n': return 15; case 'r': return 5;  case 's': return 6;  case 't': return 8;
    case 'u': return 8;  case 'v': return 7;  case 'w': return 9;  case 'y': return 10;
    default: return 0;
    }
}

__global__ void __launch_bounds__(256)
vsx_encode_kernel(const uint8_t * __restrict__ ascii, uint8_t * __restrict__ codes, uint64_t nbytes)
{
  __shared__ uint8_t lut[256];
  lut[threadIdx.x] = (uint8_t) map4(threadIdx.x);
  __syncthreads();
  const uint64_t nvec = nbytes >> 4;
  const uint64_t stride = (uint64_t) gridDim.x * blockDim.x;
  for (uint64_t v = (uint64_t) blockIdx.x * blockDim.x + threadIdx.x; v < nvec; v += stride)
    {
      const uint4 in = reinterpret_cast<const uint4 *>(ascii)[v];
      u32 w[4] = {in.x, in.y, in.z, in.w};
      u32 o[4];
#pragma unroll
      for (int x = 0; x < 4; ++x)
        o[x] = (u32) lut[w[x] & 0xff] | ((u32) lut[(w[x] >> 8) & 0xff] << 8) |
               ((u32) lut[(w[x] >> 16) & 0xff] << 16) | ((u32) lut[w[x] >> 24] << 24);
      reinterpret_cast<uint4 *>(codes)[v] = make_uint4(o[0], o[1], o[2], o[3]);
    }
  if (blockIdx.x == 0 && threadIdx.x < (nbytes & 15))
    {
      const uint64_t p = (nvec << 4) + threadIdx.x;
      codes[p] = lut[ascii[p]];
    }
}

__global__ void __launch_bounds__(256)
vsx_purity_kernel(const uint8_t * __restrict__ codes, const uint64_t * __restrict__ off,
                  const uint32_t * __restrict__ len, uint64_t nseq, uint8_t * __restrict__ impure)
{
  const uint64_t s = (uint64_t) blockIdx.x * 4 + (threadIdx.x >> 6);
  if (s >= nseq) return;
  const int lane = threadIdx.x & 63;
  const uint8_t * p = codes + off[s];
  const uint32_t n = len[s];
  int bad = 0;
  for (uint32_t x = lane; x < n; x += 64)
    {
      const u32 c = p[x];
      bad |= !((c != 0) && ((c & (c - 1)) == 0));
    }
  const unsigned long long any = __ballot(bad);
  if (lane == 0) impure[s] = any ? 1 : 0;
}

__global__ void __launch_bounds__(256)
vsx_max3_selftest_kernel(u32 * bad)
{
  const u32 x = blockIdx.x * 256u + threadIdx.x;
  if (x > 0x7BFFu) return;
  const u32 edge[8] = {0u, 1u, 0x03FFu, 0x0400u, 0x3C00u, 0x3E00u, 0x7BFEu, 0x7BFFu};
  u32 wrong = 0;
  for (u32 k = 0; k < 64; ++k)
    {
      const u32 h = (x * 2654435761u) ^ (k * 0x9E3779B9u);
      const u32 y = (k < 8) ? edge[k] : (h >> 7) % 0x7C00u;
      const u32 z = (k < 16) ? edge[(k + 3) & 7] : (h >> 17) % 0x7C00u;
      const u32 a = x | (y << 16), b = y | (z << 16), c = z | (x << 16);
      const u32 got = pk_max3_bits(a, b, c);
      const u32 m = x > y ? (x > z ? x : z) : (y > z ? y : z);
      if (got != (m | (m << 16))) ++wrong;
      const u32 pa = h ^ (x << 13), pb = (h * 0x85EBCA6Bu) ^ k;
      const u32 pg = __builtin_amdgcn_perm(pa, pb, 0x0B0A0908u);
      const u32 pe = ((pb >> 15) & 1u) * 0xFFu | (((pb >> 31) & 1u) * 0xFFu) << 8 | (((pa >> 15) & 1u) * 0xFFu) << 16 | (((pa >> 31) & 1u) * 0xFFu) << 24;
      if (pg != pe) atomicAdd(bad + 1, 1u);
    }
  if (wrong) atomicAdd(bad, wrong);
}
static std::atomic<int> g_tb_v1_dev[65];
extern "C" void vsx_internal_set_tb_v2(int device, int on) { g_tb_v1_dev[device < 0 || device > 64 ? 64 : device].store(on ? 0 : 1); }
extern "C" hipError_t vsx_launch_max3_selftest(u32 * d_bad, hipStream_t st)
{
  hipLaunchKernelGGL(vsx_max3_selftest_kernel, dim3((0x7C00 + 255) / 256), dim3(256), 0, st, d_bad);
  return hipGetLastError();
}

static const int kRows[] = {1, 4, 8, 10, 12, 14, 16, 18, 20, 22, 24, 26, 28, 32};

extern "C" const int * vsx_supported_rows(int * count)
{
  *count = (int) (sizeof(kRows) / sizeof(kRows[0]));
  return kRows;
}

extern "C" hipError_t vsx_launch_encode(const uint8_t * d_ascii, uint8_t * d_codes, uint64_t nbytes, hipStream_t st)
{
  if (nbytes == 0) return hipSuccess;
  uint64_t blocks = ((nbytes >> 4) + 255) / 256;
  if (blocks < 1) blocks = 1;
  if (blocks > 256 * 8) blocks = 256 * 8;
  hipLaunchKernelGGL(vsx_encode_kernel, dim3((unsigned) blocks), dim3(256), 0, st, d_ascii, d_codes, nbytes);
  return hipGetLastError();
}

extern "C" hipError_t vsx_launch_purity(const uint8_t * d_codes, const uint64_t * d_off, const uint32_t * d_len,
                                        uint64_t nseq, uint8_t * d_impure, hipStream_t st)
{
  if (nseq == 0) return hipSuccess;
  hipLaunchKernelGGL(vsx_purity_kernel, dim3((unsigned) ((nseq + 3) / 4)), dim3(256), 0, st,
                     d_codes, d_off, d_len, nseq, d_impure);
  return hipGetLastError();
}

#define VSX_FWD_GO(GRID_, ...) hipLaunchKernelGGL((vsx_forward_kernel<__VA_ARGS__>), dim3(GRID_), dim3(64), 0, st, P, d_tasks, q, t, dir, strip, slot, ntasks)
#define VSX_FWD_GO4(GRID_, ...) hipLaunchKernelGGL((vsx_forward_kernel<__VA_ARGS__>), dim3(GRID_), dim3(256), 0, st, P, d_tasks, q, t, dir, strip, slot, ntasks)
template <int R, bool CK>
static hipError_t launch_fwd2(int generic, int track, int nq, int one, const VsxDevParams & P, const VsxTask * d_tasks, uint32_t ntasks,
                              const uint8_t * q, const uint8_t * t, uint32_t * dir, uint2 * strip,
                              VsxSlotOut * slot, hipStream_t st)
{
  if (nq == 8)
    {
      if (!(P.tilt != 0 && CK && generic && !track) || (ntasks & 3u)) return hipErrorInvalidValue;
      if constexpr (CK && R >= 4 && VSX_QPL != 0 && VSX_FEED2 != 0 && !VSX_CKT)
        {
          if (!one) return hipErrorInvalidValue;
          if (P.max3) VSX_FWD_GO4(ntasks / 4, R, true, false, true, true, true, 1, true, true); else VSX_FWD_GO4(ntasks / 4, R, true, false, true, true, false, 1, true, true);
          return hipGetLastError();
        }
      else return hipErrorInvalidValue;
    }
  if (nq != 1)
    {
      if (!(P.tilt != 0 && CK && generic && !track && (nq == 2 || nq == 4))) return hipErrorInvalidValue;
      if constexpr (CK && R >= 4 && VSX_QPL != 0 && !VSX_CKT)
        {
          const uint32_t grid = (ntasks + (uint32_t) nq - 1) / (uint32_t) nq;
          if (nq == 2) { if (P.max3) VSX_FWD_GO(grid, R, true, false, true, true, true, 2); else VSX_FWD_GO(grid, R, true, false, true, true, false, 2); }
          else         { if (P.max3) VSX_FWD_GO(grid, R, true, false, true, true, true, 4); else VSX_FWD_GO(grid, R, true, false, true, true, false, 4); }
          return hipGetLastError();
        }
      else return hipErrorInvalidValue;
    }
  if (P.tilt != 0)
    {
      if (!(CK && generic && !track)) return hipErrorInvalidValue;
      if constexpr (CK)
        {
          if constexpr (R >= 4 && VSX_QPL != 0 && !VSX_CKT)
            {
              if (one)
                {
                  if (P.max3) VSX_FWD_GO(ntasks, R, true, false, true, true, true, 1, false, true);
                  else VSX_FWD_GO(ntasks, R, true, false, true, true, false, 1, false, true);
                  return hipGetLastError();
                }
            }
          if (P.max3 && !VSX_CKT) VSX_FWD_GO(ntasks, R, true, false, true, true, (VSX_CKT == 0));
          else VSX_FWD_GO(ntasks, R, true, false, true, true);
        }
    }
  else if (generic && track) VSX_FWD_GO(ntasks, R, true, true, CK);
  else if (generic) VSX_FWD_GO(ntasks, R, true, false, CK);
  else if (track) VSX_FWD_GO(ntasks, R, false, true, CK);
  else VSX_FWD_GO(ntasks, R, false, false, CK);
  return hipGetLastError();
}
#undef VSX_FWD_GO
#undef VSX_FWD_GO4

extern "C" hipError_t vsx_launch_forward(int rows, int generic, int track, int ckpt, int nq, int one, VsxDevParams P, const VsxTask * d_tasks, uint32_t ntasks,
                                         const uint8_t * q, const uint8_t * t, uint32_t * dir, uint2 * strip,
                                         VsxSlotOut * slot, hipStream_t st)
{
  if (ntasks == 0) return hipSuccess;
#define FWDR(RR) case RR: return ckpt ? launch_fwd2<RR, true>(generic, track, nq, one, P, d_tasks, ntasks, q, t, dir, strip, slot, st) \
                                       : launch_fwd2<RR, false>(generic, track, nq, one, P, d_tasks, ntasks, q, t, dir, strip, slot, st)
  switch (rows)
    {
    FWDR(1); FWDR(4); FWDR(8); FWDR(10); FWDR(12); FWDR(14); FWDR(16); FWDR(18); FWDR(20); FWDR(22); FWDR(24); FWDR(26); FWDR(28); FWDR(32);
    default: return hipErrorInvalidValue;
    }
#undef FWDR
}

extern "C" hipError_t vsx_launch_traceback(VsxDevParams P, const VsxTask * d_tasks, const uint32_t * d_pair_slot,
                                           const uint32_t * d_pair_ids, uint32_t npairs,
                                           const uint8_t * q, const uint8_t * t,
                                           const uint32_t * dir, const VsxSlotOut * slot,
                                           uint32_t * slab, const uint64_t * slab_off,
                                           uint32_t * runs, uint64_t runs_capacity, unsigned long long * cursor,
                                           VsxPairOut * out, hipStream_t st)
{
  if (npairs == 0) return hipSuccess;
  hipLaunchKernelGGL(vsx_traceback_kernel, dim3((npairs + 255) / 256), dim3(256), 0, st,
                     P, d_tasks, d_pair_slot, d_pair_ids, npairs, q, t, dir, slot, slab, slab_off,
                     runs, runs_capacity, cursor, out);
  return hipGetLastError();
}

template <int R, bool MID>
static hipError_t launch_tbtilt(const VsxDevParams & P, const VsxFilterDev & F, const VsxTask * d_tasks, const uint32_t * d_pair_slot,
                                const uint32_t * d_pair_ids, uint32_t npairs, const uint8_t * q, const uint8_t * t,
                                const uint32_t * ck, const VsxSlotOut * slot, uint32_t * slab, const uint64_t * slab_off,
                                uint32_t * runs, uint64_t cap, unsigned long long * cursor, VsxPairOut * out, hipStream_t st)
{
  if constexpr (R >= 4)
    hipLaunchKernelGGL((vsx_traceback_tilt_kernel<R, MID>), dim3((npairs + 63) / 64), dim3(64), 0, st,
                       P, F, d_tasks, d_pair_slot, d_pair_ids, npairs, q, t, ck, slot, slab, slab_off, runs, cap, cursor, out);
  return hipGetLastError();
}

template <int R, bool FAST, bool CK8 = false, bool MID = false>
static hipError_t launch_tbck(const VsxDevParams & P, const VsxFilterDev & F, const VsxTask * d_tasks, const uint32_t * d_pair_slot,
                              const uint32_t * d_pair_ids, uint32_t npairs, const uint8_t * q, const uint8_t * t,
                              const uint32_t * ck, const VsxSlotOut * slot, uint32_t * slab, const uint64_t * slab_off,
                              uint32_t * runs, uint64_t cap, unsigned long long * cursor, VsxPairOut * out, hipStream_t st)
{
  hipLaunchKernelGGL((vsx_traceback_ck_kernel<R, FAST, CK8, MID>), dim3((npairs + 127) / 128), dim3(128), 0, st,
                     P, F, d_tasks, d_pair_slot, d_pair_ids, npairs, q, t, ck, slot, slab, slab_off, runs, cap, cursor, out);
  return hipGetLastError();
}

extern "C" hipError_t vsx_launch_traceback_ck(int rows, int fast16, VsxDevParams P, VsxFilterDev F, const VsxTask * d_tasks, const uint32_t * d_pair_slot,
                                              const uint32_t * d_pair_ids, uint32_t npairs,
                                              const uint8_t * q, const uint8_t * t,
                                              const uint32_t * ck, const VsxSlotOut * slot,
                                              uint32_t * slab, const uint64_t * slab_off,
                                              uint32_t * runs, uint64_t runs_capacity, unsigned long long * cursor,
                                              VsxPairOut * out, hipStream_t st)
{
  if (npairs == 0) return hipSuccess;
  static const bool v1_env = std::getenv("VSX_TB_V1") != nullptr;
  int dev_now = 0;
  if (hipGetDevice(&dev_now) != hipSuccess) { (void) hipGetLastError(); dev_now = 64; }
  const bool v2 = g_tb_v1_dev[dev_now < 0 || dev_now > 64 ? 64 : dev_now].load(std::memory_order_relaxed) == 0 && !v1_env && !VSX_CKT;
#define TBCK(RR) case RR: return (fast16 && P.tilt != 0 && v2 && RR >= 4) ? launch_tbtilt<RR, VSX_MID(RR, true)>(P, F, d_tasks, d_pair_slot, d_pair_ids, npairs, q, t, ck, slot, slab, slab_off, runs, runs_capacity, cursor, out, st) \
                                 : (fast16 && P.tilt != 0) ? launch_tbck<RR, true, true, VSX_MID(RR, true)>(P, F, d_tasks, d_pair_slot, d_pair_ids, npairs, q, t, ck, slot, slab, slab_off, runs, runs_capacity, cursor, out, st) \
                                 : fast16 ? launch_tbck<RR, true>(P, F, d_tasks, d_pair_slot, d_pair_ids, npairs, q, t, ck, slot, slab, slab_off, runs, runs_capacity, cursor, out, st) \
                                        : launch_tbck<RR, false>(P, F, d_tasks, d_pair_slot, d_pair_ids, npairs, q, t, ck, slot, slab, slab_off, runs, runs_capacity, cursor, out, st)
  switch (rows)
    {
    TBCK(1); TBCK(4); TBCK(8); TBCK(10); TBCK(12); TBCK(14); TBCK(16); TBCK(18); TBCK(20); TBCK(22); TBCK(24); TBCK(26); TBCK(28); TBCK(32);
    default: return hipErrorInvalidValue;
    }
#undef TBCK
}

extern "C" uint64_t vsx_ckpt_dwords(uint64_t nstrips, uint64_t steps, uint64_t rows, int tilt)
{
  const uint64_t nblk = (steps + 15) >> 4;
  if (tilt && VSX_CKT)
    return ((nstrips * steps) >> 3) * VSX_CKT_BLOCK_DW + nstrips * nblk * (uint64_t) VSX_COLCK_NCHUNK(rows) * VSX_CKT_BLOCK_DW;
  const uint64_t rowck = (((nstrips * steps) + 1) >> 1) * VSX_ROWCK_PAIR_DW(tilt != 0);
  if (tilt)
    {
      const bool mid = VSX_MID(rows, true);
      const uint64_t rt = mid ? rows / 2 : rows;
      const uint64_t nbh = (rt + (rt + 1) / 2 + 3) / 4;
      const uint64_t nb = mid ? 2 * nbh : nbh;
      return rowck + nstrips * nblk * 64 * 4 * nb + (mid ? rowck : 0);
    }
  return rowck + nstrips * nblk * 64 * 2 * rows;
}
```

vsearch_amd/csrc/vsx_host.cpp:

```cpp
#include "../../include/vsx.h"
#include "vsx_internal.h"

#include <hip/hip_runtime.h>
#include <cstdlib>
extern "C" uint64_t vsx_internal_memory_pressure(int device);
extern "C" void vsx_internal_poison(void * p, size_t bytes)
{
  static const bool on = std::getenv("VSX_POISON") != nullptr;
  if (on && p && bytes) { (void) hipMemset(p, 0xA5, bytes); (void) hipDeviceSynchronize(); }
}

#include <algorithm>
#include <cinttypes>
#include <cstdarg>
#include <cstdio>
#include <cstdlib>
#include <cstring>
#include <sched.h>
#include <thread>
#include <atomic>
#include <condition_variable>
#include <mutex>
#include <chrono>
#include <deque>
// ... 143 lines not shown
        (void) hipFree(free_blocks[m].p);
        free_blocks.erase(free_blocks.begin() + (long) m);
      }
  }
  void retire() { trim(); std::lock_guard<std::mutex> lk(mu); retired = true; }
};

template <typename T>
struct PoolBuf {
  T * p = nullptr;
  size_t n = 0, bytes = 0;
  ScratchPool * pool = nullptr;
  ~PoolBuf() { release(); }
  void release() { if (p && pool) pool->put(p, bytes); else if (p) (void) hipFree(p); p = nullptr; n = 0; bytes = 0; }
  hipError_t alloc(ScratchPool * pl, size_t count)
  {
    release();
    pool = pl;
    if (count == 0) count = 1;
    void * q = nullptr;
    size_t got = count * sizeof(T);
    hipError_t e = pl ? pl->get(count * sizeof(T), &q, &got) : hipMalloc(&q, count * sizeof(T));
    if (e == hipSuccess) { p = static_cast<T *>(q); n = count; bytes = got; }
    return e;
  }
};

struct SharedBlock {
  void * p = nullptr;
  size_t bytes = 0;
  ScratchPool * pool = nullptr;
  ~SharedBlock() { if (p) { if (pool) pool->put(p, bytes); else (void) hipFree(p); } }
};
struct SharedSlot;
thread_local const SharedSlot * tl_acquiring_slot = nullptr;
struct SharedSlot {
  std::mutex mu;
  std::shared_ptr<SharedBlock> cur;
  hipError_t acquire(ScratchPool * pool, size_t bytes, std::shared_ptr<SharedBlock> & out, bool headroom = true)
  {
    std::lock_guard<std::mutex> lk(mu);
    struct Mark { const SharedSlot * prev; explicit Mark(const SharedSlot * s) : prev(tl_acquiring_slot) { tl_acquiring_slot = s; } ~Mark() { tl_acquiring_slot = prev; } } mark(this);
    if (cur && cur->bytes >= bytes) { out = cur; return hipSuccess; }
    cur.reset();
    auto b = std::make_shared<SharedBlock>();
    static const bool dbg = std::getenv("VSX_DEBUG_TIMING") != nullptr;
    const auto t0 = std::chrono::steady_clock::now();
    hipError_t e = pool->get(headroom ? bytes + bytes / 8 : bytes, &b->p, &b->bytes);
    if (dbg) std::fprintf(stderr, "  shared block: %zu bytes wanted (had %zu), got %zu in %.2f ms\n", bytes, cur ? cur->bytes : (size_t) 0, b->bytes,
                          std::chrono::duration<double>(std::chrono::steady_clock::now() - t0).count() * 1e3);
    if (e == hipErrorOutOfMemory) { (void) hipGetLastError(); e = pool->get(bytes, &b->p, &b->bytes); }
    if (e != hipSuccess) { b->p = nullptr; return e; }
    b->pool = pool;
    cur = b;
    out = b;
    return hipSuccess;
  }
  void reset() { std::lock_guard<std::mutex> lk(mu); cur.reset(); }
  void try_reset() { if (tl_acquiring_slot == this) return; if (mu.try_lock()) { cur.reset(); mu.unlock(); } }
  size_t bytes() { std::lock_guard<std::mutex> lk(mu); return cur ? cur->bytes : 0; }
};
template <typename T>
struct SharedBuf {
  std::shared_ptr<SharedBlock> blk;
  T * p = nullptr;
  hipError_t alloc(SharedSlot & slot, ScratchPool * pool, size_t count)
  {
    hipError_t e = slot.acquire(pool, std::max<size_t>(count, 1) * sizeof(T), blk);
    p = (e == hipSuccess) ? static_cast<T *>(blk->p) : nullptr;
    return e;
  }
};

}

struct vsx_ctx {
  int device = 0;
  hipStream_t stream = nullptr;
  hipStream_t stream2 = nullptr;
  hipStream_t stream_b = nullptr;
  hipStream_t stream_up = nullptr;
  hipStream_t stream_dn = nullptr;
  vsx_scoring sc {};
  bool force_fallback = false;
  bool tb_packed = false;
  bool ckpt = true;
  int pen[12] {};
  VsxDevParams P {};
  DevBuf<int16_t> d_htop, d_hleft, d_matrix;
  VsxDevParams Pt {};
  DevBuf<int16_t> d_htop_t, d_hleft_t, d_matrix_t;
  std::shared_ptr<ScratchPool> pool_owner = std::make_shared<ScratchPool>();
  ScratchPool & pool = *pool_owner;
  SharedSlot shared_dir[3], shared_slab;
  std::atomic<uint64_t> req_hwm[2] {{0}, {0}};
  hipEvent_t ev_tb[3] = {nullptr, nullptr, nullptr};
  bool ev_tb_used[3] = {false, false, false};
  int last_tb_slot = -1;
  std::atomic<unsigned> plan_seq {0};
  std::mutex slot_mu;
  int slot_refs[3] = {0, 0, 0};
  unsigned slot_stamp[3] = {0, 0, 0};
  std::mutex stage_mu;
  uint8_t * stage = nullptr;
  size_t stage_bytes = 0;
  std::vector<unsigned long long *> cursor_slots;
  ~vsx_ctx()
  {
    for (hipEvent_t e : ev_tb) if (e) (void) hipEventDestroy(e);
    if (stage) (void) hipHostFree(stage);
    for (auto * c : cursor_slots) (void) hipHostFree(c);
  }
};

#define VSX_SEQSET_POOLED_BYTES (64ull << 20)
struct vsx_seqset {
  vsx_ctx * ctx = nullptr;
  int device = 0;
  uint64_t n = 0;
  uint64_t bytes = 0;
  std::vector<uint64_t> off;
  std::vector<uint32_t> len;
  std::shared_ptr<ScratchPool> pool_ref;
  PoolBuf<uint8_t> d_codes;
  uint8_t * codes() const { return d_codes.p + VSX_CODE_SLACK; }
  PoolBuf<uint64_t> d_off;
  PoolBuf<uint32_t> d_len;
  PoolBuf<uint8_t> d_lower;
  uint64_t lower_bytes = 0;
  mutable std::mutex impure_mu;
  mutable std::vector<uint8_t> impure;
  mutable bool have_impure = false;
};

namespace {

struct Launch { int rows; int generic; int track; int tilt; int nq ; uint32_t first, count; uint32_t pair_first, pair_count;
                bool multi = false ; };

struct Chunk {
  uint32_t task_first = 0, task_count = 0;
  uint32_t pair_first = 0, pair_count = 0;
  std::vector<Launch> launches;
  uint64_t dir_dwords = VSX_CK_SLACK_DW, strip_elems = 0, slab_words = 0;
  hipEvent_t e0 = nullptr, e1 = nullptr, e1b = nullptr, e2 = nullptr;
};

}

extern "C" int vsx_internal_usable_cpus(void);
#ifndef VSX_PAIRPROF_DEFAULT
#define VSX_PAIRPROF_DEFAULT 1
#endif
static std::atomic<int> g_max3_state[64];
static std::mutex g_ctx_mu;
static std::vector<vsx_ctx *> g_ctxs;
template <typename T>
static T * dup_array(const std::vector<T> & v)
{
  T * p = (T *) std::malloc(std::max<size_t>(v.size(), 1) * sizeof(T));
  if (p && !v.empty()) std::memcpy(p, v.data(), v.size() * sizeof(T));
  return p;
}


static int copy_threads(uint64_t bytes)
{
  return (int) std::max<uint64_t>(1, std::min<uint64_t>((uint64_t) vsx_internal_usable_cpus(), bytes >> 21));
}

namespace {
class WorkerPool {
 public:
  static WorkerPool & get() { static WorkerPool p; return p; }
  template <typename F>
  void run(int nth, F && f)
  {
    if (nth <= 1) { f(0); return; }
    struct Region { int left; std::mutex m; std::condition_variable cv; };
    Region rg;
    rg.left = nth - 1;
    {
      std::lock_guard<std::mutex> lk(mu_);
      for (int t = 1; t < nth; ++t)
        queue_.push_back([&f, &rg, t]() {
          f(t);
          std::lock_guard<std::mutex> lk2(rg.m);
          if (--rg.left == 0) rg.cv.notify_all();
        });
    }
    cv_.notify_all();
    f(0);
    for (;;)
      {
        { std::lock_guard<std::mutex> lk(rg.m); if (rg.left == 0) break; }
        std::function<void()> job;
        {
          std::lock_guard<std::mutex> lk(mu_);
          if (!queue_.empty()) { job = std::move(queue_.front()); queue_.pop_front(); }
        }
        if (job) { job(); continue; }
        std::unique_lock<std::mutex> lk(rg.m);
        if (rg.cv.wait_for(lk, std::chrono::microseconds(50), [&] { return rg.left == 0; })) break;
      }
  }
 private:
  WorkerPool()
  {
    const int n = std::max(1, vsx_internal_usable_cpus() - 1);
    for (int i = 0; i < n; ++i)
      workers_.emplace_back([this]() {
        for (;;)
          {
            std::function<void()> job;
            {
              std::unique_lock<std::mutex> lk(mu_);
              cv_.wait(lk, [&] { return stop_ || !queue_.empty(); });
              if (stop_ && queue_.empty()) return;
              job = std::move(queue_.front());
              queue_.pop_front();
            }
            job();
          }
      });
  }
  ~WorkerPool()
  {
    { std::lock_guard<std::mutex> lk(mu_); stop_ = true; }
    cv_.notify_all();
    for (auto & w : workers_) w.join();
  }
  std::mutex mu_;
  std::condition_variable cv_;
  std::deque<std::function<void()>> queue_;
  std::vector<std::thread> workers_;
  bool stop_ = false;
};
}

template <typename F>
static void run_threads(int nth, F && f)
{
  WorkerPool::get().run(nth, f);
}

struct vsx_plan {
  vsx_ctx * ctx = nullptr;
  const vsx_seqset * Q = nullptr;
  const vsx_seqset * T = nullptr;
  uint64_t n_pairs = 0;
  VsxFilterDev filter {};
  std::vector<VsxPairOut> host_out;
  std::vector<std::string> host_cigar;
  std::vector<uint32_t> host_cigar_pair;
  std::vector<uint32_t> host_cigar_run;

  std::vector<VsxTask> tasks;
  std::vector<uint32_t> pair_slot, pair_ids;
  std::vector<uint64_t> slab_off;
  std::vector<Chunk> chunks;
  uint64_t cells = 0, dir_bytes_total = 0;

  PoolBuf<VsxTask> d_tasks;
  PoolBuf<uint32_t> d_pair_slot, d_pair_ids;
  SharedBuf<uint32_t> d_dir[1], d_slab;
  int dir_slot = 0;
  bool slot_held = false;
  bool alt_fwd = false;
  PoolBuf<uint32_t> d_runs;
  PoolBuf<uint64_t> d_slab_off;
  PoolBuf<uint2> d_strip;
  PoolBuf<VsxSlotOut> d_slot;
  PoolBuf<VsxPairOut> d_out;
  PoolBuf<unsigned long long> d_cursor;
  PoolBuf<uint8_t> d_text, d_soa;
  PoolBuf<uint32_t> d_rank_counts, d_kept_pair, d_refused_pair;
  PoolBuf<double> d_kept_id;
  VsxSoaOut soa {};
  uint64_t soa_bytes = 0, soa_off[7] {};
  uint64_t text_capacity = 0;
  unsigned long long * h_cursor = nullptr;
  std::vector<uint32_t> host_pairs;
  uint64_t runs_capacity = 0;
  hipEvent_t ev_begin = nullptr, ev_end = nullptr;
  bool ran = false;
  bool host_patched = false;

  ~vsx_plan()
  {
    for (auto & c : chunks)
      {
        if (c.e0) (void) hipEventDestroy(c.e0);
        if (c.e1) (void) hipEventDestroy(c.e1);
        if (c.e1b) (void) hipEventDestroy(c.e1b);
        if (c.e2) (void) hipEventDestroy(c.e2);
      }
    if (ev_begin) (void) hipEventDestroy(ev_begin);
    if (ev_end) (void) hipEventDestroy(ev_end);
    if (h_cursor) { std::lock_guard<std::mutex> lk(ctx->stage_mu); ctx->cursor_slots.push_back(h_cursor); }
    if (slot_held) { std::lock_guard<std::mutex> lk(ctx->slot_mu); --ctx->slot_refs[dir_slot]; }
  }
};

extern "C" {

void vsx_internal_run_threads(int nth, void (*fn)(int, void *), void * arg) { run_threads(nth, [&](int t) { fn(t, arg); }); }
// ... 172 lines not shown
        int v;
        if (P.n_mismatch && (x == 15 || y == 15)) v = mism;
        else if (amb(x) || amb(y)) v = 0;
        else v = (x == y) ? match : mism;
        matrix[x * 16 + y] = (int16_t) v;
      }

  auto cleanup = [&]() {
    if (c->stream) (void) hipStreamDestroy(c->stream);
    if (c->stream2) (void) hipStreamDestroy(c->stream2);
    if (c->stream_b) (void) hipStreamDestroy(c->stream_b);
    if (c->stream_up) (void) hipStreamDestroy(c->stream_up);
    if (c->stream_dn) (void) hipStreamDestroy(c->stream_dn);
    delete c;
  };
  hipError_t e;
  int prio_low = 0, prio_high = 0;
  (void) hipDeviceGetStreamPriorityRange(&prio_low, &prio_high);
  static const bool flat_env = std::getenv("VSX_ALIGN_FLAT_PRIORITY") != nullptr;
  const int prio_dp = (!flat_env && prio_low - prio_high >= 2) ? prio_high + 1 : prio_high;
  if ((e = hipStreamCreateWithPriority(&c->stream, hipStreamNonBlocking, prio_dp)) != hipSuccess ||
      (e = hipStreamCreateWithPriority(&c->stream2, hipStreamNonBlocking, prio_high)) != hipSuccess ||
      (e = hipStreamCreateWithPriority(&c->stream_b, hipStreamNonBlocking, prio_dp)) != hipSuccess ||
      (e = hipStreamCreateWithPriority(&c->stream_up, hipStreamNonBlocking, prio_high)) != hipSuccess ||
      (e = hipStreamCreateWithPriority(&c->stream_dn, hipStreamNonBlocking, prio_high)) != hipSuccess ||
      (e = hipEventCreateWithFlags(&c->ev_tb[0], hipEventDisableTiming)) != hipSuccess ||
      (e = hipEventCreateWithFlags(&c->ev_tb[1], hipEventDisableTiming)) != hipSuccess ||
      (e = hipEventCreateWithFlags(&c->ev_tb[2], hipEventDisableTiming)) != hipSuccess ||
      (e = c->d_htop.alloc(VSX_TABLE_LEN)) != hipSuccess || (e = c->d_hleft.alloc(VSX_TABLE_LEN)) != hipSuccess ||
      (e = c->d_matrix.alloc(256)) != hipSuccess ||
      (e = hipMemcpy(c->d_htop.p, htop.data(), VSX_TABLE_LEN * 2, hipMemcpyHostToDevice)) != hipSuccess ||
      (e = hipMemcpy(c->d_hleft.p, hleft.data(), VSX_TABLE_LEN * 2, hipMemcpyHostToDevice)) != hipSuccess ||
      (e = hipMemcpy(c->d_matrix.p, matrix.data(), 512, hipMemcpyHostToDevice)) != hipSuccess)
    {
      cleanup();
      return fail(VSX_EHIP, "vsx_create: %s", hipGetErrorString(e));
    }
  P.htop = c->d_htop.p;
  P.hleft = c->d_hleft.p;
  P.matrix = c->d_matrix.p;
  P.tilt = 0;
  if (device < 64 && g_max3_state[device].load() == 0)
    {
      DevBuf<uint32_t> d_bad;
      uint32_t bad2[2] = {1, 1};
      if (d_bad.alloc(2) == hipSuccess && hipMemsetAsync(d_bad.p, 0, 8, c->stream) == hipSuccess &&
          vsx_launch_max3_selftest(d_bad.p, c->stream) == hipSuccess &&
          hipMemcpyAsync(bad2, d_bad.p, 8, hipMemcpyDeviceToHost, c->stream) == hipSuccess && hipStreamSynchronize(c->stream) == hipSuccess)
        {
          const uint32_t bad = bad2[0];
          if (bad) std::fprintf(stderr, "libvsx: device %d: v_pk_maximum3_f16 disagrees with the integer maximum on %u probes -- MAX3 class disabled\n", device, bad);
          g_max3_state[device].store(bad ? 2 : 1);
          if (bad2[1])
            {
              std::fprintf(stderr, "libvsx: device %d: v_perm_b32 sign selectors disagree on %u probes -- the first traceback kernel is used\n", device, bad2[1]);
              vsx_internal_set_tb_v2(device, 0);
            }
        }
      else
        {
          (void) hipGetLastError();
          std::fprintf(stderr, "libvsx: device %d: the MAX3 / v_perm_b32 self-test could not run -- MAX3 class and second traceback kernel disabled\n", device);
          g_max3_state[device].store(2);
          vsx_internal_set_tb_v2(device, 0);
        }
    }
  else if (device >= 64) vsx_internal_set_tb_v2(device, 0);

  if (geqi == geti && geti > 0 && P.share_sub && c->ckpt && !c->tb_packed && !c->force_fallback &&
      std::min(match, mism) + 2 * geti >= 0 && 2 * geti - geql >= 0 &&
      std::max(match, mism) + 2 * geti <= 255 && 2 * geti - geql <= 255 &&
      geti <= 127 && std::max({goqi, goti, goqr + geqr - geti, gotr + getr - geti, goql + geql + goqi}) <= 127 &&
      !(std::getenv("VSX_TILT") && std::strcmp(std::getenv("VSX_TILT"), "0") == 0))
    {
      const int g = geti;
      VsxDevParams & T = c->Pt;
      T = P;
      T.tilt = g;
      T.qrq_i_pk = pk(goqi + geqi - g); T.rq_i_pk = pk(geqi - g);
      T.qrq_r_pk = pk(goqr + geqr - g); T.rq_r_pk = pk(geqr - g);
      T.qrt_i = goti + geti - g; T.rt_i = geti - g;
      T.qrt_r = gotr + getr - g; T.rt_r = getr - g;
      std::vector<int16_t> htop_t(VSX_TABLE_LEN), hleft_t(VSX_TABLE_LEN), matrix_t(256);
      for (int j = 0; j < VSX_TABLE_LEN; ++j)
        {
          htop_t[j] = (int16_t) sat16((int) htop[j] + (j - 1) * g);
          hleft_t[j] = (int16_t) sat16((int) hleft[j] + (j - 1) * g);
        }
      for (int x = 0; x < 256; ++x) matrix_t[x] = (int16_t) sat16(matrix[x] + 2 * g);
      if ((e = c->d_htop_t.alloc(VSX_TABLE_LEN)) != hipSuccess || (e = c->d_hleft_t.alloc(VSX_TABLE_LEN)) != hipSuccess ||
          (e = c->d_matrix_t.alloc(256)) != hipSuccess ||
          (e = hipMemcpy(c->d_htop_t.p, htop_t.data(), VSX_TABLE_LEN * 2, hipMemcpyHostToDevice)) != hipSuccess ||
          (e = hipMemcpy(c->d_hleft_t.p, hleft_t.data(), VSX_TABLE_LEN * 2, hipMemcpyHostToDevice)) != hipSuccess ||
          (e = hipMemcpy(c->d_matrix_t.p, matrix_t.data(), 512, hipMemcpyHostToDevice)) != hipSuccess)
        {
          cleanup();
          return fail(VSX_EHIP, "vsx_create: %s", hipGetErrorString(e));
        }
      T.htop = c->d_htop_t.p; T.hleft = c->d_hleft_t.p; T.matrix = c->d_matrix_t.p;
    }
  { std::lock_guard<std::mutex> lk(g_ctx_mu); g_ctxs.push_back(c); }
  *out = c;
  return VSX_OK;
}

void vsx_destroy(vsx_ctx * c)
{
  if (!c) return;
  { std::lock_guard<std::mutex> lk(g_ctx_mu); g_ctxs.erase(std::remove(g_ctxs.begin(), g_ctxs.end(), c), g_ctxs.end()); }
  (void) hipSetDevice(c->device);
  if (c->stream) { (void) hipStreamSynchronize(c->stream); (void) hipStreamDestroy(c->stream); }
  if (c->stream2) { (void) hipStreamSynchronize(c->stream2); (void) hipStreamDestroy(c->stream2); }
  if (c->stream_b) { (void) hipStreamSynchronize(c->stream_b); (void) hipStreamDestroy(c->stream_b); }
  if (c->stream_up) { (void) hipStreamSynchronize(c->stream_up); (void) hipStreamDestroy(c->stream_up); }
  if (c->stream_dn) { (void) hipStreamSynchronize(c->stream_dn); (void) hipStreamDestroy(c->stream_dn); }
  c->shared_dir[0].reset();
  c->shared_dir[1].reset();
  c->shared_dir[2].reset();
  c->shared_slab.reset();
  c->pool.retire();
  delete c;
}

static int seqset_common(vsx_ctx * ctx, vsx_seqset ** out, uint64_t n, const void * blob, bool blob_on_device,
                         uint64_t blob_bytes, const uint64_t * offsets, const uint32_t * lengths, bool both_strands = false,
                         int case_bits = 0 )
{
  if (!ctx || !out || (n && (!offsets || !lengths)) || (blob_bytes && !blob))
    return fail(VSX_EINVAL, "vsx_seqset_create: null argument");
  *out = nullptr;
  for (uint64_t i = 0; i < n; ++i)
    if (offsets[i] + lengths[i] > blob_bytes)
      return fail(VSX_EINVAL, "vsx_seqset_create: sequence %" PRIu64 " exceeds the blob", i);
  HIPCHK(hipSetDevice(ctx->device));
  auto * s = new vsx_seqset;
  s->ctx = ctx;
  s->device = ctx->device;
  s->n = n;
  s->bytes = blob_bytes;
  s->off.assign(offsets, offsets + n);
  s->len.assign(lengths, lengths + n);
  uint64_t code_bytes = blob_bytes;
  if (both_strands)
    {
      s->n = 2 * n;
      s->off.resize(2 * n);
      s->len.resize(2 * n);
      for (uint64_t k = 0; k < n; ++k) { s->off[n + k] = code_bytes; s->len[n + k] = lengths[k]; code_bytes += lengths[k]; }
      s->bytes = code_bytes;
    }
  hipError_t e = hipSuccess;
  ScratchPool * pl = (code_bytes <= VSX_SEQSET_POOLED_BYTES) ? &ctx->pool : nullptr;
  if (pl) s->pool_ref = ctx->pool_owner;
  PoolBuf<uint8_t> staging;
  const uint8_t * d_ascii = static_cast<const uint8_t *>(blob);
  do {
    if ((e = s->d_codes.alloc(pl, code_bytes + 2 * VSX_CODE_SLACK)) != hipSuccess) break;
    if ((e = s->d_off.alloc(pl, s->n)) != hipSuccess) break;
    if ((e = s->d_len.alloc(pl, s->n)) != hipSuccess) break;
    if (n)
      {
        if ((e = hipMemcpyAsync(s->d_off.p, s->off.data(), s->n * 8, hipMemcpyHostToDevice, ctx->stream)) != hipSuccess) break;
        if ((e = hipMemcpyAsync(s->d_len.p, s->len.data(), s->n * 4, hipMemcpyHostToDevice, ctx->stream)) != hipSuccess) break;
      }
    if (!blob_on_device && blob_bytes)
      {
        if ((e = staging.alloc(pl, blob_bytes + 16)) != hipSuccess) break;
        if ((e = hipMemcpyAsync(staging.p, blob, blob_bytes, hipMemcpyHostToDevice, ctx->stream)) != hipSuccess) break;
        d_ascii = staging.p;
      }
    if ((e = vsx_launch_encode(d_ascii, s->codes(), blob_bytes, ctx->stream)) != hipSuccess) break;
    if (case_bits)
      {
        const uint64_t nb = (blob_bytes + 7) / 8 + 16;
        if ((e = s->d_lower.alloc(pl, nb)) != hipSuccess) break;
        if ((e = hipMemsetAsync(s->d_lower.p, 0, nb, ctx->stream)) != hipSuccess) break;
        if ((e = vsx_kmer_launch_case_bits(d_ascii, blob_bytes, s->d_lower.p, case_bits == 2, ctx->stream)) != hipSuccess) break;
        if (case_bits == 2 && (e = vsx_launch_dust(s->codes(), s->d_off.p, s->d_len.p, n, s->d_lower.p, ctx->stream)) != hipSuccess) break;
        s->lower_bytes = (blob_bytes + 7) / 8;
      }
    if (both_strands && (e = vsx_launch_revcomp(s->codes(), s->d_off.p, s->d_off.p + n, s->d_len.p, n, ctx->stream)) != hipSuccess) break;
    e = hipStreamSynchronize(ctx->stream);
  } while (false);
  if (e != hipSuccess)
    {
      delete s;
      return fail(e == hipErrorOutOfMemory ? VSX_ENOMEM : VSX_EHIP, "vsx_seqset_create: %s", hipGetErrorString(e));
    }
  *out = s;
  return VSX_OK;
}

int vsx_seqset_create(vsx_ctx * ctx, vsx_seqset ** out, uint64_t n, const char * blob, uint64_t blob_bytes,
                      const uint64_t * offsets, const uint32_t * lengths)
{
  return seqset_common(ctx, out, n, blob, false, blob_bytes, offsets, lengths);
}

int vsx_seqset_create_both_strands(vsx_ctx * ctx, vsx_seqset ** out, uint64_t n, const char * blob, uint64_t blob_bytes,
                                   const uint64_t * offsets, const uint32_t * lengths)
{
  return seqset_common(ctx, out, n, blob, false, blob_bytes, offsets, lengths, true);
}

int vsx_internal_seqset_create_cased(vsx_ctx * ctx, vsx_seqset ** out, uint64_t n, const char * blob, uint64_t blob_bytes,
                                     const uint64_t * offsets, const uint32_t * lengths, int mode)
{
  if (mode != 1 && mode != 2) return fail(VSX_EINVAL, "vsx_internal_seqset_create_cased: mode must be 1 (soft) or 2 (dust)");
  return seqset_common(ctx, out, n, blob, false, blob_bytes, offsets, lengths, false, mode);
}
const uint8_t * vsx_internal_seqset_lower(const vsx_seqset * s) { return s ? s->d_lower.p : nullptr; }
int vsx_internal_seqset_lower_download(const vsx_seqset * s, uint8_t * dst, uint64_t nbytes)
{
  if (!s || !s->d_lower.p || nbytes > s->lower_bytes) return fail(VSX_EINVAL, "vsx_internal_seqset_lower_download: no case bitmap of that size");
  HIPCHK(hipSetDevice(s->device));
  if (nbytes) HIPCHK(hipMemcpy(dst, s->d_lower.p, nbytes, hipMemcpyDeviceToHost));
  return VSX_OK;
}

int vsx_internal_mask_bits(vsx_ctx * ctx, uint64_t n, const char * blob, uint64_t blob_bytes, const uint64_t * offsets,
                           const uint32_t * lengths, int mode, uint8_t * bits_out)
{
  vsx_seqset * s = nullptr;
  int rc = vsx_internal_seqset_create_cased(ctx, &s, n, blob, blob_bytes, offsets, lengths, mode);
  if (rc != VSX_OK) return rc;
  rc = vsx_internal_seqset_lower_download(s, bits_out, (blob_bytes + 7) / 8);
  vsx_seqset_destroy(s);
  return rc;
}

int vsx_seqset_create_from_device(vsx_ctx * ctx, vsx_seqset ** out, uint64_t n, const void * d_blob,
                                  uint64_t blob_bytes, const uint64_t * offsets, const uint32_t * lengths)
{
  return seqset_common(ctx, out, n, d_blob, true, blob_bytes, offsets, lengths);
}

void vsx_seqset_destroy(vsx_seqset * s)
{
  if (!s) return;
  (void) hipSetDevice(s->device);
  delete s;
}

uint64_t vsx_seqset_count(const vsx_seqset * s) { return s ? s->n : 0; }

static int ensure_impure(const vsx_seqset * s)
{
  std::lock_guard<std::mutex> lk(s->impure_mu);
  if (s->have_impure) return VSX_OK;
  vsx_ctx * ctx = s->ctx;
  HIPCHK(hipSetDevice(ctx->device));
  PoolBuf<uint8_t> d_flags;
  HIPCHK(d_flags.alloc(s->pool_ref ? s->pool_ref.get() : nullptr, s->n));
  HIPCHK(vsx_launch_purity(s->codes(), s->d_off.p, s->d_len.p, s->n, d_flags.p, ctx->stream));
  s->impure.assign(s->n, 0);
  if (s->n) HIPCHK(hipMemcpyAsync(s->impure.data(), d_flags.p, s->n, hipMemcpyDeviceToHost, ctx->stream));
  HIPCHK(hipStreamSynchronize(ctx->stream));
  s->have_impure = true;
  return VSX_OK;
}

static bool no_overflow_possible(const vsx_ctx * ctx, int64_t Q, int64_t D)
{
  int64_t B = std::max<int64_t>(std::llabs(ctx->P.match), std::llabs(ctx->P.mismatch));
  int64_t G = 0;
  for (int k = 0; k < 12; ++k)
    {
      if (ctx->pen[k] < 0) return false;
      if (k < 6) G = std::max<int64_t>(G, ctx->pen[k]); else B = std::max<int64_t>(B, ctx->pen[k]);
    }
  if (ctx->pen[2] + ctx->pen[8] < ctx->pen[6] || ctx->pen[8] < ctx->pen[6]) return false;
  const int64_t Dp = (D + 3) & ~3ll;
  return 4 * G + (Q + Dp + 16) * B < 32000;
}

static int tilt_possible(const vsx_ctx * ctx, int64_t Q, int64_t D)
{
  if (ctx->Pt.tilt == 0) return 0;
  static const bool max3_off = std::getenv("VSX_MAX3") && std::strcmp(std::getenv("VSX_MAX3"), "0") == 0;
  int64_t B = std::max<int64_t>(std::llabs(ctx->P.match), std::llabs(ctx->P.mismatch));
  int64_t G = 0;
  for (int k = 0; k < 12; ++k)
    if (k < 6) G = std::max<int64_t>(G, ctx->pen[k]); else B = std::max<int64_t>(B, ctx->pen[k]);
  const int64_t Dp = (D + 3) & ~3ll;
  const int64_t reach = 4 * G + 2 * (Q + Dp + 64) * B;
  if (reach < 15800 && !max3_off && !VSX_CKT && ctx->pen[4] > 0 &&
      ctx->device < 64 && g_max3_state[ctx->device].load(std::memory_order_relaxed) == 1) return 2;
  return reach < 32000 ? 1 : 0;
}

static int pick_rows(int Q)
{
  static const int forced = std::getenv("VSX_ROWS") ? std::atoi(std::getenv("VSX_ROWS")) : 0;
  if (forced > 0 && Q >= forced) return forced;
  int cnt = 0;
  const int * rows = vsx_supported_rows(&cnt);
  int idx = cnt - 1;
  for (int k = 0; k < cnt; ++k)
    if (16 * rows[k] >= Q) { idx = k; break; }
  while (idx > 0 && Q < rows[idx]) --idx;
  return rows[idx];
}

int vsx_plan_create(vsx_ctx * ctx, vsx_plan ** out, const vsx_seqset * queries, const vsx_seqset * targets,
                    uint64_t n_pairs, const uint32_t * qidx, const uint32_t * tidx, uint64_t dir_budget_bytes)
{
  if (!ctx || !out || !queries || !targets || (n_pairs && (!qidx || !tidx)))
    return fail(VSX_EINVAL, "vsx_plan_create: null argument");
  *out = nullptr;
  if (queries->device != ctx->device || targets->device != ctx->device)
    return fail(VSX_EINVAL, "vsx_plan_create: seqset lives on another device");
  if (n_pairs > 0xffffffffull / 8) return fail(VSX_EINVAL, "vsx_plan_create: too many pairs for one plan");
  static const bool timing = std::getenv("VSX_DEBUG_TIMING") != nullptr;
  auto now = []() { return std::chrono::duration<double>(std::chrono::steady_clock::now().time_since_epoch()).count(); };
  const double tc0 = now();
  const int nthc = (int) std::max<uint64_t>(1, std::min<uint64_t>((uint64_t) vsx_internal_usable_cpus(), n_pairs / 32768));
  {
    std::vector<uint64_t> bad((size_t) nthc, UINT64_MAX);
    auto check = [&](int t) {
      const uint64_t lo = n_pairs * (uint64_t) t / (uint64_t) nthc, hi = n_pairs * (uint64_t) (t + 1) / (uint64_t) nthc;
      for (uint64_t k = lo; k < hi; ++k)
        if (qidx[k] >= queries->n || tidx[k] >= targets->n) { bad[(size_t) t] = k; return; }
    };
    run_threads(nthc, check);
    for (int t = 0; t < nthc; ++t)
      if (bad[(size_t) t] != UINT64_MAX)
        return fail(VSX_EINVAL, "vsx_plan_create: pair %" PRIu64 " references a sequence out of range", bad[(size_t) t]);
  }
  HIPCHK(hipSetDevice(ctx->device));
  static const bool arith = std::getenv("VSX_SCORE") && std::strcmp(std::getenv("VSX_SCORE"), "arith") == 0;
  if (arith) { const int rc = ensure_impure(queries); if (rc != VSX_OK) return rc; }
  static const bool pair_env = (std::getenv("VSX_PAIRPROF") ? std::strcmp(std::getenv("VSX_PAIRPROF"), "0") != 0 : (VSX_PAIRPROF_DEFAULT != 0)) &&
                               !arith && VSX_QPL != 0 && VSX_FEED2 != 0 && !VSX_CKT;
  const bool pair_try = pair_env && ctx->ckpt && n_pairs >= 32;

  std::unique_ptr<vsx_plan> pl(new vsx_plan);
  pl->ctx = ctx; pl->Q = queries; pl->T = targets; pl->n_pairs = n_pairs;
  static const unsigned ck_blocks = (std::getenv("VSX_CK_BLOCKS") && std::atoi(std::getenv("VSX_CK_BLOCKS")) == 2) ? 2u : 3u;
  {
    static const bool rotate_env = std::getenv("VSX_CK_ROTATE") && std::strcmp(std::getenv("VSX_CK_ROTATE"), "1") == 0;
    std::lock_guard<std::mutex> lk(ctx->slot_mu);
    const unsigned seq = ctx->plan_seq.fetch_add(1);
    int pick = -1;
    if (rotate_env) pick = (int) (seq % ck_blocks);
    else
      {
        for (int k = 0; k < (int) ck_blocks; ++k)
          if (ctx->slot_refs[k] == 0 && (pick < 0 || ctx->shared_dir[k].bytes() > ctx->shared_dir[pick].bytes())) pick = k;
        if (pick < 0)
          for (int k = 0; k < (int) ck_blocks; ++k)
            if (pick < 0 || (int) (seq - ctx->slot_stamp[k]) > (int) (seq - ctx->slot_stamp[pick])) pick = k;
      }
    ++ctx->slot_refs[pick];
    ctx->slot_stamp[pick] = seq;
    pl->dir_slot = pick;
    pl->slot_held = true;
  }

  std::vector<uint32_t> gpu_pairs;
  {
    std::vector<std::vector<uint32_t>> gp((size_t) nthc), special((size_t) nthc);
    std::vector<uint64_t> pcells((size_t) nthc, 0);
    auto classify = [&](int t) {
      const uint64_t lo = n_pairs * (uint64_t) t / (uint64_t) nthc, hi = n_pairs * (uint64_t) (t + 1) / (uint64_t) nthc;
      gp[(size_t) t].reserve(hi - lo);
      uint64_t cells = 0;
      for (uint64_t k = lo; k < hi; ++k)
        {
          const int64_t Q = queries->len[qidx[k]], D = targets->len[tidx[k]];
          if (ctx->force_fallback || Q == 0 || D == 0 || !fits(Q, D)) { special[(size_t) t].push_back((uint32_t) k); continue; }
          gp[(size_t) t].push_back((uint32_t) k);
          cells += (uint64_t) Q * (uint64_t) D;
        }
      pcells[(size_t) t] = cells;
    };
    run_threads(nthc, classify);
    size_t total = 0;
    for (auto & v : gp) total += v.size();
    gpu_pairs.resize(total);
    {
      std::vector<size_t> base((size_t) nthc);
      size_t acc = 0;
      for (int t = 0; t < nthc; ++t) { base[(size_t) t] = acc; acc += gp[(size_t) t].size(); pl->cells += pcells[(size_t) t]; }
      auto place = [&](int t) { if (!gp[(size_t) t].empty()) std::memcpy(gpu_pairs.data() + base[(size_t) t], gp[(size_t) t].data(), gp[(size_t) t].size() * 4); };
      run_threads(nthc, place);
    }
    for (int t = 0; t < nthc; ++t)
      for (uint32_t k : special[(size_t) t])
        {
          const int64_t Q = queries->len[qidx[k]], D = targets->len[tidx[k]];
          pl->host_pairs.push_back(k);
          pl->host_out.emplace_back();
          VsxPairOut & o = pl->host_out.back();
          auto sentinel = [&]() { o = VsxPairOut {}; o.score = 32767; };
          if (ctx->force_fallback) { sentinel(); continue; }
          if (Q == 0)
            {
              if (!fits(0, D)) { sentinel(); continue; }
              o = VsxPairOut {};
              o.aligned = (uint16_t) D; o.gaps = (uint16_t) D;
              if (D > 0)
                {
                  const int64_t a = -(int64_t) ctx->pen[1] - D * (int64_t) ctx->pen[7];
                  const int64_t b = -(int64_t) ctx->pen[5] - D * (int64_t) ctx->pen[11];
                  o.score = (int16_t) (uint16_t) (std::max(a, b) & 0xffff);
                  pl->host_cigar.push_back(std::to_string(D) + "I");
                  pl->host_cigar_pair.push_back(k);
                  pl->host_cigar_run.push_back(((uint32_t) D << 2) | 1u);
                }
              continue;
            }
          sentinel();
        }
  }
  const double tc1 = now();

  auto by_query = [&](uint32_t a, uint32_t b) { return qidx[a] < qidx[b]; };
  if (!std::is_sorted(gpu_pairs.begin(), gpu_pairs.end(), by_query)) std::stable_sort(gpu_pairs.begin(), gpu_pairs.end(), by_query);
  struct ProtoTask { uint32_t q; int rows; int generic; int track; int tilt; int nq; uint32_t n; uint32_t pair[8]; };
  static const bool sparse_env = !(std::getenv("VSX_SPARSE") && std::strcmp(std::getenv("VSX_SPARSE"), "0") == 0) && VSX_QPL != 0 && !VSX_CKT;
  const bool sparse_on = sparse_env && ctx->ckpt;
  std::vector<size_t> group_begin;
  for (size_t b = 0; b < gpu_pairs.size();)
    {
      group_begin.push_back(b);
      const uint32_t q = qidx[gpu_pairs[b]];
      size_t e = b;
      while (e < gpu_pairs.size() && qidx[gpu_pairs[e]] == q) ++e;
      b = e;
    }
  group_begin.push_back(gpu_pairs.size());
  const size_t ngroups = group_begin.size() - 1;
  const int nth = (int) std::max<size_t>(1, std::min<size_t>((size_t) vsx_internal_usable_cpus(), gpu_pairs.size() / 16384));
  std::vector<std::vector<ProtoTask>> part((size_t) nth);
  std::vector<std::vector<std::pair<size_t, size_t>>> pair_cand((size_t) nth);
  auto work = [&](int t) {
    const size_t p_lo = gpu_pairs.size() * (size_t) t / (size_t) nth, p_hi = gpu_pairs.size() * (size_t) (t + 1) / (size_t) nth;
    const size_t g_lo = (size_t) (std::lower_bound(group_begin.begin(), group_begin.end() - 1, p_lo) - group_begin.begin());
    const size_t g_hi = (t == nth - 1) ? ngroups : (size_t) (std::lower_bound(group_begin.begin(), group_begin.end() - 1, p_hi) - group_begin.begin());
    std::vector<ProtoTask> & outp = part[(size_t) t];
    for (size_t g = g_lo; g < g_hi; ++g)
      {
        const size_t b = group_begin[g], e = group_begin[g + 1];
        const uint32_t q = qidx[gpu_pairs[b]];
        std::stable_sort(gpu_pairs.begin() + (long) b, gpu_pairs.begin() + (long) e,
                         [&](uint32_t x, uint32_t y) { return targets->len[tidx[x]] > targets->len[tidx[y]]; });
        const int rows = pick_rows((int) queries->len[q]);
        const int generic = (!arith || queries->impure[q]) ? 1 : 0;
        const size_t first_of_query = outp.size();
        for (size_t x = b; x < e; x += VSX_TASK_SLOTS)
          {
            ProtoTask pt {};
            pt.q = q; pt.rows = rows; pt.generic = generic;
            pt.n = (uint32_t) std::min<size_t>(VSX_TASK_SLOTS, e - x);
            uint32_t dmax = 0;
            for (uint32_t sidx = 0; sidx < pt.n; ++sidx)
              {
                pt.pair[sidx] = gpu_pairs[x + sidx];
                dmax = std::max(dmax, targets->len[tidx[pt.pair[sidx]]]);
              }
            pt.track = (!ctx->tb_packed && no_overflow_possible(ctx, queries->len[q], dmax)) ? 0 : 1;
            pt.tilt = (pt.track == 0 && generic && ctx->ckpt) ? tilt_possible(ctx, queries->len[q], dmax) : 0;
            pt.nq = 1;
            if (sparse_on && pt.tilt && rows >= 4 && pt.n <= 4 && (int64_t) queries->len[q] <= 16ll * rows)
              pt.nq = pt.n <= 2 ? 4 : 2;
            outp.push_back(pt);
          }
        if (pair_try && rows >= 4 && outp.size() - first_of_query >= 4 && (int64_t) queries->len[q] <= 16ll * rows)
          {
            size_t eligible = 0;
            for (size_t k = first_of_query; k < outp.size(); ++k) eligible += (outp[k].nq == 1 && outp[k].tilt) ? 1 : 0;
            if (eligible >= 4) pair_cand[(size_t) t].emplace_back(first_of_query, outp.size());
          }
      }
  };
  run_threads(nth, work);
  bool any_pair_cand = false;
  for (const auto & v : pair_cand) any_pair_cand = any_pair_cand || !v.empty();
  if (any_pair_cand)
    {
      int rc = ensure_impure(queries);
      if (rc == VSX_OK) rc = ensure_impure(targets);
      if (rc != VSX_OK) return rc;
    }
  auto mark_pairs = [&](int t) {
    std::vector<ProtoTask> & outp = part[(size_t) t];
    for (const std::pair<size_t, size_t> & range : pair_cand[(size_t) t])
      {
        const size_t first_of_query = range.first, end_of_query = range.second;
        if (queries->impure[outp[first_of_query].q]) continue;
          {
            std::vector<size_t> ok;
            for (size_t k = first_of_query; k < end_of_query; ++k)
              {
                ProtoTask & pt = outp[k];
                if (pt.nq != 1 || !pt.tilt) continue;
                bool pure = true;
                for (uint32_t sidx = 0; sidx < pt.n && pure; ++sidx) pure = !targets->impure[tidx[pt.pair[sidx]]];
                if (pure) ok.push_back(k);
              }
            size_t i0 = 0;
            while (i0 < ok.size())
              {
                size_t i1 = i0;
                while (i1 < ok.size() && outp[ok[i1]].tilt == outp[ok[i0]].tilt) ++i1;
                const size_t whole = (i1 - i0) / 4 * 4;
                for (size_t k = i0; k < i0 + whole; ++k) outp[ok[k]].nq = 8;
                i0 = i1;
              }
          }
      }
  };
  if (any_pair_cand) run_threads(nth, mark_pairs);
  std::vector<ProtoTask> protos;
  {
    size_t total = 0;
    for (auto & v : part) total += v.size();
    protos.reserve(total);
    for (auto & v : part) protos.insert(protos.end(), v.begin(), v.end());
  }
  {
    static const bool no_promote = std::getenv("VSX_NO_PROMOTE") != nullptr;
    struct Cls { int rows, generic, track, tilt, nq; size_t count; };
    std::vector<Cls> cls;
    for (const ProtoTask & pt : protos)
      {
        bool found = false;
        for (Cls & c : cls) if (c.rows == pt.rows && c.generic == pt.generic && c.track == pt.track && c.tilt == pt.tilt && c.nq == pt.nq) { ++c.count; found = true; break; }
        if (!found) cls.push_back(Cls {pt.rows, pt.generic, pt.track, pt.tilt, pt.nq, 1});
      }
    std::vector<std::pair<size_t, int>> move;
    for (size_t a = 0; a < cls.size() && !no_promote; ++a)
      {
        int best = 0;
        for (const Cls & c : cls)
          if (c.generic == cls[a].generic && c.track == cls[a].track && c.tilt == cls[a].tilt && c.nq == cls[a].nq && c.rows > cls[a].rows &&
              c.count >= 32 * cls[a].count && (best == 0 || c.rows < best))
            best = c.rows;
        if (best && cls[a].count < 4096) move.emplace_back(a, best);
      }
    for (auto & mv : move)
      for (int hop = 0; hop < 4; ++hop)
        for (const auto & other : move)
          {
            const Cls & a = cls[mv.first], & o = cls[other.first];
            if (o.rows == mv.second && o.generic == a.generic && o.track == a.track && o.tilt == a.tilt && o.nq == a.nq) { mv.second = other.second; break; }
          }
    if (!move.empty())
      for (ProtoTask & pt : protos)
        for (const auto & mv : move)
          {
            const Cls & c = cls[mv.first];
            if (pt.rows == c.rows && pt.generic == c.generic && pt.track == c.track && pt.tilt == c.tilt && pt.nq == c.nq)
              {
                if ((int) queries->len[pt.q] > mv.second) pt.rows = mv.second;
                break;
              }
          }
  }
  if (sparse_on)
    {
      static const size_t sparse_min = std::getenv("VSX_SPARSE_MIN") ? (size_t) std::atoll(std::getenv("VSX_SPARSE_MIN")) : 4096;
      struct Key { int rows, generic, track, tilt, nq; size_t count; };
      std::vector<Key> ks;
      for (const ProtoTask & pt : protos)
        {
          if (pt.nq != 2 && pt.nq != 4) continue;
          bool found = false;
          for (Key & c : ks) if (c.rows == pt.rows && c.generic == pt.generic && c.track == pt.track && c.tilt == pt.tilt && c.nq == pt.nq) { ++c.count; found = true; break; }
          if (!found) ks.push_back(Key {pt.rows, pt.generic, pt.track, pt.tilt, pt.nq, 1});
        }
      bool any = false;
      for (const Key & c : ks) any = any || c.count < sparse_min;
      if (any)
        for (ProtoTask & pt : protos)
          if (pt.nq == 2 || pt.nq == 4)
            for (const Key & c : ks)
              if (c.count < sparse_min && pt.nq == c.nq && pt.rows == c.rows && pt.generic == c.generic && pt.track == c.track && pt.tilt == c.tilt) { pt.nq = 1; break; }
    }
  auto by_class = [](const ProtoTask & a, const ProtoTask & b) {
    if (a.rows != b.rows) return a.rows < b.rows;
    if (a.generic != b.generic) return a.generic < b.generic;
    if (a.track != b.track) return a.track < b.track;
    if (a.tilt != b.tilt) return a.tilt < b.tilt;
    return a.nq < b.nq;
  };
  if (!std::is_sorted(protos.begin(), protos.end(), by_class)) std::stable_sort(protos.begin(), protos.end(), by_class);

  double t_budget = 0;
  if (dir_budget_bytes == 0)
    {
      size_t free_b = 0, total_b = 0;
      const double tb0 = now();
      HIPCHK(hipMemGetInfo(&free_b, &total_b));
      t_budget = now() - tb0;
      free_b += ctx->pool.idle_bytes() + ctx->shared_dir[pl->dir_slot].bytes();
      dir_budget_bytes = std::min<uint64_t>((uint64_t) (free_b * 0.4), 128ull << 30);
      const uint64_t have = ctx->shared_dir[pl->dir_slot].bytes();
      if (have >= dir_budget_bytes / 2) dir_budget_bytes = have;
    }
  const uint64_t budget_dwords = std::max<uint64_t>(dir_budget_bytes / 4, 1);

  const double tc2 = now();
  const size_t NT = protos.size();
  pl->tasks.resize(NT);
  pl->pair_slot.resize(gpu_pairs.size());
  pl->pair_ids.resize(gpu_pairs.size());
  pl->slab_off.resize(gpu_pairs.size());
  std::vector<uint64_t> t_dwords(NT), t_slab(NT), t_pair0(NT);
  const int ntt = (int) std::max<size_t>(1, std::min<size_t>((size_t) vsx_internal_usable_cpus(), NT / 4096));
  run_threads(ntt, [&](int th) {
    const size_t lo = NT * (size_t) th / (size_t) ntt, hi = NT * (size_t) (th + 1) / (size_t) ntt;
    for (size_t x = lo; x < hi; ++x)
      {
        const ProtoTask & pt = protos[x];
        VsxTask t {};
        t.qoff = queries->off[pt.q];
        t.qlen = queries->len[pt.q];
        t.rows = (uint32_t) pt.rows;
        uint32_t dmax = 0;
        uint64_t slab = 0;
        for (uint32_t sl = 0; sl < pt.n; ++sl)
          {
            const uint32_t ti = tidx[pt.pair[sl]];
            t.toff[sl] = targets->off[ti];
            t.tlen[sl] = targets->len[ti];
            dmax = std::max(dmax, (targets->len[ti] + 3u) & ~3u);
            slab += (uint64_t) t.qlen + t.tlen[sl] + 1;
          }
        t.steps = dmax + 16;
        if (pt.tilt && VSX_CKT) t.steps = (t.steps + 7u) & ~7u;
        const uint64_t total_lanes = (t.qlen + pt.rows - 1) / pt.rows;
        const uint64_t nstrips = (total_lanes + 15) / 16;
        const uint64_t nd = (uint64_t) (pt.rows + 3) / 4;
        t_dwords[x] = ctx->ckpt ? vsx_ckpt_dwords(nstrips, t.steps, (uint64_t) pt.rows, pt.tilt)
                                : ((nstrips * t.steps + 3) & ~3ull) * 64 * nd;
        t.strip_off = nstrips > 1 ? 2ull * 4 * t.steps : 0;
        t_slab[x] = slab;
        pl->tasks[x] = t;
      }
  });
  size_t np_out = 0;
  Chunk cur;
  auto close_chunk = [&]() {
    if (cur.task_count) pl->chunks.push_back(cur);
    Chunk nc;
    nc.task_first = cur.task_first + cur.task_count;
    nc.pair_first = cur.pair_first + cur.pair_count;
    cur = nc;
  };
  uint32_t wave_left = 0, wave_steps = 0, wave_group = 0, pair_left = 0;
  uint64_t wave_off = 0;
  auto same_class = [&](size_t a, size_t b) {
    return protos[a].rows == protos[b].rows && protos[a].generic == protos[b].generic && protos[a].track == protos[b].track &&
           protos[a].tilt == protos[b].tilt && protos[a].nq == protos[b].nq;
  };
  for (size_t x = 0; x < NT; ++x)
    {
      const ProtoTask & pt = protos[x];
      VsxTask & t = pl->tasks[x];
      uint64_t dwords = t_dwords[x];
      const uint64_t strip = t.strip_off;
      const bool sparse_task = pt.nq == 2 || pt.nq == 4;
      if (pt.nq == 8)
        {
          if (pair_left == 0)
// ... 49 lines not shown
      {
        const ProtoTask & pt = protos[x];
        const VsxTask & t = pl->tasks[x];
        uint64_t slab = t_slab[x];
        for (uint32_t sl = 0; sl < pt.n; ++sl)
          {
            const size_t o = (size_t) t_pair0[x] + sl;
            pl->pair_slot[o] = (uint32_t) x * VSX_TASK_SLOTS + sl;
            pl->pair_ids[o] = pt.pair[sl];
            pl->slab_off[o] = slab;
            slab += (uint64_t) t.qlen + t.tlen[sl] + 1;
          }
      }
  });
  close_chunk();
  const double tc3 = now();

  uint64_t max_dir = 1, max_strip = 1, max_slab = 1, worst_runs = 0;
  for (const Chunk & c : pl->chunks)
    {
      max_dir = std::max(max_dir, c.dir_dwords + VSX_CK_SLACK_DW);
      max_strip = std::max(max_strip, c.strip_elems);
      max_slab = std::max(max_slab, c.slab_words);
      worst_runs += c.slab_words;
    }
  const size_t ngp = pl->pair_ids.size();
  pl->runs_capacity = std::min<uint64_t>(worst_runs, std::max<uint64_t>(16ull << 20, 48ull * ngp)) + 1;
  HIPCHK(pl->d_tasks.alloc(&ctx->pool, pl->tasks.size()));
  HIPCHK(pl->d_pair_slot.alloc(&ctx->pool, ngp));
  HIPCHK(pl->d_pair_ids.alloc(&ctx->pool, ngp));
  HIPCHK(pl->d_slab_off.alloc(&ctx->pool, ngp));
  HIPCHK(pl->d_slot.alloc(&ctx->pool, pl->tasks.size() * VSX_TASK_SLOTS));
  HIPCHK(pl->d_out.alloc(&ctx->pool, n_pairs));
  HIPCHK(pl->d_cursor.alloc(&ctx->pool, 2));
  {
    const uint64_t np = std::max<uint64_t>(n_pairs, 1);
    const uint64_t width[7] = {2, 2, 2, 2, 2, 1, 8};
    uint64_t at = 0;
    for (int x = 0; x < 7; ++x) { pl->soa_off[x] = at; at += (np * width[x] + 15) & ~15ull; }
    pl->soa_bytes = at;
    HIPCHK(pl->d_soa.alloc(&ctx->pool, at));
    uint8_t * b = pl->d_soa.p;
    pl->soa.score = reinterpret_cast<int16_t *>(b + pl->soa_off[0]);
    pl->soa.aligned = reinterpret_cast<uint16_t *>(b + pl->soa_off[1]);
    pl->soa.matches = reinterpret_cast<uint16_t *>(b + pl->soa_off[2]);
    pl->soa.mismatches = reinterpret_cast<uint16_t *>(b + pl->soa_off[3]);
    pl->soa.gaps = reinterpret_cast<uint16_t *>(b + pl->soa_off[4]);
    pl->soa.verdict = b + pl->soa_off[5];
    pl->soa.text_off = reinterpret_cast<uint64_t *>(b + pl->soa_off[6]);
  }
  {
    std::lock_guard<std::mutex> lk(ctx->stage_mu);
    if (!ctx->cursor_slots.empty()) { pl->h_cursor = ctx->cursor_slots.back(); ctx->cursor_slots.pop_back(); }
  }
  if (!pl->h_cursor) HIPCHK(hipHostMalloc(reinterpret_cast<void **>(&pl->h_cursor), 64, hipHostMallocDefault));
  for (int k = 0; k < 2; ++k)
    {
      const uint64_t need = (k == 0 ? max_dir : max_slab) * 4;
      uint64_t seen = ctx->req_hwm[k].load();
      while (need > seen && !ctx->req_hwm[k].compare_exchange_weak(seen, need)) { }
    }
  HIPCHK(pl->d_dir[0].alloc(ctx->shared_dir[pl->dir_slot], &ctx->pool, max_dir));
  HIPCHK(pl->d_strip.alloc(&ctx->pool, max_strip));
  HIPCHK(pl->d_slab.alloc(ctx->shared_slab, &ctx->pool, max_slab));
  HIPCHK(pl->d_runs.alloc(&ctx->pool, pl->runs_capacity));
  pl->text_capacity = std::min<uint64_t>(6 * worst_runs + 8 * (uint64_t) ngp, std::max<uint64_t>(32ull << 20, 128ull * ngp)) + 16;
  HIPCHK(pl->d_text.alloc(&ctx->pool, pl->text_capacity));
  if (!pl->tasks.empty())
    HIPCHK(hipMemcpyAsync(pl->d_tasks.p, pl->tasks.data(), pl->tasks.size() * sizeof(VsxTask), hipMemcpyHostToDevice, ctx->stream_up));
  if (ngp)
    {
      HIPCHK(hipMemcpyAsync(pl->d_pair_slot.p, pl->pair_slot.data(), ngp * 4, hipMemcpyHostToDevice, ctx->stream_up));
      HIPCHK(hipMemcpyAsync(pl->d_pair_ids.p, pl->pair_ids.data(), ngp * 4, hipMemcpyHostToDevice, ctx->stream_up));
      HIPCHK(hipMemcpyAsync(pl->d_slab_off.p, pl->slab_off.data(), ngp * 8, hipMemcpyHostToDevice, ctx->stream_up));
    }
  HIPCHK(hipEventCreate(&pl->ev_begin));
  HIPCHK(hipEventCreate(&pl->ev_end));
  for (Chunk & c : pl->chunks)
    {
      HIPCHK(hipEventCreate(&c.e0));
      HIPCHK(hipEventCreate(&c.e1));
      HIPCHK(hipEventCreate(&c.e1b));
      HIPCHK(hipEventCreate(&c.e2));
    }
  HIPCHK(hipStreamSynchronize(ctx->stream_up));
  if (timing)
    std::fprintf(stderr, "vsx_plan_create: %llu pairs, %zu tasks: classify %.2f ms, group %.2f ms (budget query %.2f), tasks %.2f ms, device buffers + upload %.2f ms\n",
                 (unsigned long long) n_pairs, pl->tasks.size(), (tc1 - tc0) * 1e3, (tc2 - tc1) * 1e3, t_budget * 1e3, (tc3 - tc2) * 1e3, (now() - tc3) * 1e3);
  *out = pl.release();
  return VSX_OK;
}

int vsx_plan_set_filter(vsx_plan * pl, const vsx_filter * f)
{
  if (!pl) return fail(VSX_EINVAL, "vsx_plan_set_filter: null plan");
  pl->filter = VsxFilterDev {};
  if (!f) return VSX_OK;
  if (!pl->ctx->ckpt) return fail(VSX_EINVAL, "vsx_plan_set_filter: needs the checkpoint traceback (VSX_TRACEBACK=dirs is set)");
  if (f->iddef < 0 || f->iddef > 4) return fail(VSX_EINVAL, "vsx_plan_set_filter: iddef must be 0..4");
  VsxFilterDev & d = pl->filter;
  d.enabled = 1; d.iddef = f->iddef; d.leftjust = f->leftjust; d.rightjust = f->rightjust;
  d.id = f->id; d.weak_id = f->weak_id; d.maxid = f->maxid; d.mid = f->mid; d.query_cov = f->query_cov; d.target_cov = f->target_cov;
  d.maxsubs = f->maxsubs; d.maxgaps = f->maxgaps; d.mincols = f->mincols; d.maxdiffs = f->maxdiffs;
  pl->ran = false;
  return VSX_OK;
}

static bool rank_lists_on()
{
  static const bool prim = std::getenv("VSX_RANK_PRIM") && std::strcmp(std::getenv("VSX_RANK_PRIM"), "1") == 0;
  return !prim;
}
static int plan_set_ranked(vsx_plan * pl)
{
  if (!rank_lists_on() || !pl->filter.enabled) return VSX_OK;
  vsx_ctx * ctx = pl->ctx;
  const size_t n = (size_t) pl->n_pairs;
  HIPCHK(hipSetDevice(ctx->device));
  HIPCHK(pl->d_rank_counts.alloc(&ctx->pool, 2));
  HIPCHK(pl->d_kept_pair.alloc(&ctx->pool, n + 1));
  HIPCHK(pl->d_kept_id.alloc(&ctx->pool, n + 1));
  HIPCHK(pl->d_refused_pair.alloc(&ctx->pool, n + 1));
  pl->filter.rank_counts = pl->d_rank_counts.p;
  pl->filter.kept_pair = pl->d_kept_pair.p;
  pl->filter.kept_id = pl->d_kept_id.p;
  pl->filter.refused_pair = pl->d_refused_pair.p;
  return VSX_OK;
}

int vsx_plan_run(vsx_plan * pl)
{
  if (!pl) return fail(VSX_EINVAL, "vsx_plan_run: null plan");
  vsx_ctx * ctx = pl->ctx;
  HIPCHK(hipSetDevice(ctx->device));
  hipStream_t st = pl->alt_fwd ? ctx->stream_b : ctx->stream, st2 = ctx->stream2;
  const int slot = pl->dir_slot;
  HIPCHK(hipMemsetAsync(pl->d_cursor.p, 0, 2 * sizeof(unsigned long long), st));
  if (pl->filter.rank_counts) HIPCHK(hipMemsetAsync(pl->d_rank_counts.p, 0, 2 * sizeof(uint32_t), st));
  HIPCHK(hipEventRecord(pl->ev_begin, st));
  for (size_t k = 0; k < pl->chunks.size(); ++k)
    {
      Chunk & c = pl->chunks[k];
      uint32_t * dir = pl->d_dir[0].p;
      if (k >= 1) HIPCHK(hipStreamWaitEvent(st, pl->chunks[k - 1].e2, 0));
      else if (ctx->ev_tb_used[slot]) HIPCHK(hipStreamWaitEvent(st, ctx->ev_tb[slot], 0));
      static const bool serial_env = std::getenv("VSX_ALIGN_SERIAL") && std::strcmp(std::getenv("VSX_ALIGN_SERIAL"), "1") == 0;
      if (k == 0 && serial_env && ctx->last_tb_slot >= 0 && ctx->last_tb_slot != slot) HIPCHK(hipStreamWaitEvent(st, ctx->ev_tb[ctx->last_tb_slot], 0));
      HIPCHK(hipEventRecord(c.e0, st));
      for (const Launch & L : c.launches)
        {
          VsxDevParams Pf = L.tilt ? ctx->Pt : ctx->P;
          Pf.max3 = (L.tilt == 2) ? 1 : 0;
          static const bool one_off = std::getenv("VSX_ONESTRIP") && std::strcmp(std::getenv("VSX_ONESTRIP"), "0") == 0;
          HIPCHK(vsx_launch_forward(L.rows, L.generic, L.track, ctx->ckpt ? 1 : 0, L.nq, (L.multi || (one_off && L.nq != 8)) ? 0 : 1, Pf, pl->d_tasks.p + L.first, L.count,
                                    pl->Q->codes(), pl->T->codes(), dir, pl->d_strip.p,
                                    pl->d_slot.p + (size_t) L.first * VSX_TASK_SLOTS, st));
        }
      HIPCHK(hipEventRecord(c.e1, st));
      HIPCHK(hipStreamWaitEvent(st2, c.e1, 0));
      HIPCHK(hipEventRecord(c.e1b, st2));
      if (ctx->ckpt)
        {
          for (size_t li = 0; li < c.launches.size();)
            {
              const Launch & L = c.launches[li];
              uint32_t pair_count = L.pair_count;
              size_t lj = li + 1;
              while (lj < c.launches.size() && c.launches[lj].rows == L.rows && c.launches[lj].generic == L.generic &&
                     c.launches[lj].track == L.track && c.launches[lj].tilt == L.tilt) { pair_count += c.launches[lj].pair_count; ++lj; }
              VsxDevParams Pb = L.tilt ? ctx->Pt : ctx->P;
              Pb.max3 = (L.tilt == 2) ? 1 : 0;
              HIPCHK(vsx_launch_traceback_ck(L.rows, (L.track == 0 && L.generic != 0) ? 1 : 0, Pb, pl->filter, pl->d_tasks.p, pl->d_pair_slot.p + L.pair_first,
                                             pl->d_pair_ids.p + L.pair_first, pair_count, pl->Q->codes(), pl->T->codes(),
                                             dir, pl->d_slot.p, pl->d_slab.p, pl->d_slab_off.p + L.pair_first,
                                             pl->d_runs.p, pl->runs_capacity, pl->d_cursor.p, pl->d_out.p, st2));
              li = lj;
            }
        }
      else
        HIPCHK(vsx_launch_traceback(ctx->P, pl->d_tasks.p, pl->d_pair_slot.p + c.pair_first, pl->d_pair_ids.p + c.pair_first,
                                    c.pair_count, pl->Q->codes(), pl->T->codes(), dir, pl->d_slot.p,
                                    pl->d_slab.p, pl->d_slab_off.p + c.pair_first, pl->d_runs.p, pl->runs_capacity,
                                    pl->d_cursor.p, pl->d_out.p, st2));
      HIPCHK(hipEventRecord(c.e2, st2));
    }
  if (pl->chunks.empty()) HIPCHK(hipStreamWaitEvent(st2, pl->ev_begin, 0));
  HIPCHK(hipEventRecord(ctx->ev_tb[slot], st2));
  ctx->ev_tb_used[slot] = true;
  ctx->last_tb_slot = slot;
  HIPCHK(vsx_launch_cigar_text(pl->d_out.p, pl->d_pair_ids.p, (uint32_t) pl->pair_ids.size(), pl->d_runs.p, pl->runs_capacity,
                               pl->d_text.p, pl->text_capacity, pl->d_cursor.p + 1, pl->soa, st2));
  HIPCHK(hipMemcpyAsync(pl->h_cursor, pl->d_cursor.p, 2 * sizeof(unsigned long long), hipMemcpyDeviceToHost, st2));
  HIPCHK(hipEventRecord(pl->ev_end, st2));
  pl->ran = true;
  pl->host_patched = false;
  return VSX_OK;
}

int vsx_plan_sync(vsx_plan * pl, vsx_timing * tm)
{
  if (!pl) return fail(VSX_EINVAL, "vsx_plan_sync: null plan");
  if (!pl->ran) return fail(VSX_EINVAL, "vsx_plan_sync: plan has not been run");
  HIPCHK(hipSetDevice(pl->ctx->device));
  HIPCHK(hipEventSynchronize(pl->ev_end));
  if (tm)
    {
      *tm = vsx_timing {};
      for (Chunk & c : pl->chunks)
        {
          float a = 0, b = 0;
          HIPCHK(hipEventElapsedTime(&a, c.e0, c.e1));
          HIPCHK(hipEventElapsedTime(&b, c.e1b, c.e2));
          tm->forward_ms += a;
          tm->traceback_ms += b;
          tm->forward_launches += (uint32_t) c.launches.size();
          tm->traceback_launches += 1;
        }
      HIPCHK(hipEventElapsedTime(&tm->total_ms, pl->ev_begin, pl->ev_end));
      tm->cells = pl->cells;
      tm->dir_bytes = pl->dir_bytes_total;
    }
  return VSX_OK;
}

int vsx_plan_describe(const vsx_plan * pl, vsx_plan_info * info)
{
  if (!pl || !info) return fail(VSX_EINVAL, "vsx_plan_describe: null argument");
  *info = vsx_plan_info {};
  info->tasks = pl->tasks.size();
  info->chunks = (uint32_t) pl->chunks.size();
  uint64_t best = 0;
  for (const Chunk & c : pl->chunks)
    for (const Launch & L : c.launches)
      {
        if (L.nq == 2 || L.nq == 4) info->tasks_sparse += L.count;
        if (L.nq == 8) info->tasks_pair += L.count;
        info->waves += (L.nq == 2 || L.nq == 4) ? (L.count + (uint32_t) L.nq - 1) / (uint32_t) L.nq : L.count;
        if (L.tilt) info->tasks_tilted += L.count;
        if (L.tilt == 2) info->tasks_max3 += L.count;
        if (L.track) info->tasks_tracked += L.count;
        if (L.count > best) { best = L.count; info->rows_dominant = (uint32_t) L.rows; }
      }
  return VSX_OK;
}

static void append_cigar(std::string & s, const uint32_t * runs, uint32_t n)
{
  static const char ops[4] = {'M', 'I', 'D', '?'};
  char buf[16];
  for (uint32_t k = n; k-- > 0;)
    {
      const uint32_t len = runs[k] >> 2;
      if (len > 1) { int w = snprintf(buf, sizeof buf, "%u", len); s.append(buf, (size_t) w); }
      s.push_back(ops[runs[k] & 3]);
    }
}

struct FetchDest {
  int16_t * score; uint16_t * aligned, * matches, * mismatches, * gaps; uint64_t * cigar_off; uint8_t * verdict;
  char ** blob; uint64_t * blob_used;
};

static int settle(vsx_plan * pl, unsigned long long & used, unsigned long long & text_used)
{
  vsx_ctx * ctx = pl->ctx;
  if (!pl->ran) { int rc = vsx_plan_run(pl); if (rc != VSX_OK) return rc; }
  int rc = vsx_plan_sync(pl, nullptr);
  if (rc != VSX_OK) return rc;
  HIPCHK(hipSetDevice(ctx->device));
  hipStream_t st = ctx->stream;
  used = pl->h_cursor[0]; text_used = pl->h_cursor[1];
  if (used > pl->runs_capacity)
    {
      pl->runs_capacity = used + 1;
      HIPCHK(pl->d_runs.alloc(&pl->ctx->pool, pl->runs_capacity));
      if ((rc = vsx_plan_run(pl)) != VSX_OK) return rc;
      if ((rc = vsx_plan_sync(pl, nullptr)) != VSX_OK) return rc;
      used = pl->h_cursor[0]; text_used = pl->h_cursor[1];
      if (used > pl->runs_capacity) return fail(VSX_EHIP, "vsx_plan_fetch: run buffer overflow after resize");
    }
  if (text_used > pl->text_capacity)
    {
      pl->text_capacity = text_used + 16;
      HIPCHK(pl->d_text.alloc(&pl->ctx->pool, pl->text_capacity));
      HIPCHK(hipMemsetAsync(pl->d_cursor.p + 1, 0, sizeof(unsigned long long), st));
      HIPCHK(vsx_launch_cigar_text(pl->d_out.p, pl->d_pair_ids.p, (uint32_t) pl->pair_ids.size(), pl->d_runs.p, pl->runs_capacity,
                                   pl->d_text.p, pl->text_capacity, pl->d_cursor.p + 1, pl->soa, st));
      HIPCHK(hipMemcpyAsync(pl->h_cursor, pl->d_cursor.p, 2 * sizeof(unsigned long long), hipMemcpyDeviceToHost, st));
      HIPCHK(hipStreamSynchronize(st));
      text_used = pl->h_cursor[1];
      if (text_used > pl->text_capacity) return fail(VSX_EHIP, "vsx_plan_fetch: text buffer overflow after resize");
    }
  return VSX_OK;
}

static int stage_reserve(vsx_ctx * ctx, uint64_t need)
{
  if (need <= ctx->stage_bytes) return VSX_OK;
  if (ctx->stage) { (void) hipHostFree(ctx->stage); ctx->stage = nullptr; ctx->stage_bytes = 0; }
  const uint64_t want = need + need / 4 + (1u << 20);
  if (hipHostMalloc(reinterpret_cast<void **>(&ctx->stage), want, hipHostMallocDefault) != hipSuccess)
    { (void) hipGetLastError(); return fail(VSX_ENOMEM, "vsx_plan_fetch: pinned staging allocation failed"); }
  ctx->stage_bytes = want;
  return VSX_OK;
}

static int fetch_core(vsx_plan * pl, const FetchDest & D)
{
  vsx_ctx * ctx = pl->ctx;
  unsigned long long used = 0, text_used = 0;
  int rc = settle(pl, used, text_used);
  if (rc != VSX_OK) return rc;

  const uint64_t n = pl->n_pairs;
  uint64_t tail = 0;
  for (size_t h = 0, hc = 0; h < pl->host_pairs.size(); ++h)
    {
      ++tail;
      if (hc < pl->host_cigar_pair.size() && pl->host_cigar_pair[hc] == pl->host_pairs[h]) tail += pl->host_cigar[hc++].size();
    }
  const uint64_t base = *D.blob_used;
  {
    char * nb = (char *) std::realloc(*D.blob, std::max<uint64_t>(base + text_used + tail, 1));
    if (!nb) return fail(VSX_ENOMEM, "vsx_plan_fetch: host allocation failed");
    *D.blob = nb;
  }
  char * const blob = *D.blob;

  {
    std::lock_guard<std::mutex> lk(ctx->stage_mu);
    if ((rc = stage_reserve(ctx, pl->soa_bytes + ((text_used + 15) & ~15ull))) != VSX_OK) return rc;
    hipError_t e = hipSuccess;
    if (n) e = hipMemcpyAsync(ctx->stage, pl->d_soa.p, pl->soa_bytes, hipMemcpyDeviceToHost, ctx->stream_dn);
    if (e == hipSuccess && text_used) e = hipMemcpyAsync(ctx->stage + pl->soa_bytes, pl->d_text.p, text_used, hipMemcpyDeviceToHost, ctx->stream_dn);
    if (e == hipSuccess) e = hipStreamSynchronize(ctx->stream_dn);
    if (e != hipSuccess) return fail(VSX_EHIP, "vsx_plan_fetch: %s", hipGetErrorString(e));
    const uint8_t * sg = ctx->stage;
    const int nth = copy_threads(n * 19 + text_used);
    run_threads(nth, [&](int t) {
      const uint64_t lo = n * (uint64_t) t / (uint64_t) nth, hi = n * (uint64_t) (t + 1) / (uint64_t) nth;
      if (hi > lo)
        {
          std::memcpy(D.score + lo, sg + pl->soa_off[0] + 2 * lo, 2 * (hi - lo));
          std::memcpy(D.aligned + lo, sg + pl->soa_off[1] + 2 * lo, 2 * (hi - lo));
          std::memcpy(D.matches + lo, sg + pl->soa_off[2] + 2 * lo, 2 * (hi - lo));
          std::memcpy(D.mismatches + lo, sg + pl->soa_off[3] + 2 * lo, 2 * (hi - lo));
          std::memcpy(D.gaps + lo, sg + pl->soa_off[4] + 2 * lo, 2 * (hi - lo));
          if (D.verdict) std::memcpy(D.verdict + lo, sg + pl->soa_off[5] + lo, hi - lo);
          const uint64_t * so = reinterpret_cast<const uint64_t *>(sg + pl->soa_off[6]);
          for (uint64_t k = lo; k < hi; ++k) D.cigar_off[k] = so[k] + base;
        }
      const uint64_t blo = text_used * (uint64_t) t / (uint64_t) nth, bhi = text_used * (uint64_t) (t + 1) / (uint64_t) nth;
      if (bhi > blo) std::memcpy(blob + base + blo, sg + pl->soa_bytes + blo, bhi - blo);
    });
  }
  uint64_t at = base + text_used;
  for (size_t h = 0, hc = 0; h < pl->host_pairs.size(); ++h)
    {
      const uint32_t k = pl->host_pairs[h];
      const VsxPairOut & o = pl->host_out[h];
      D.score[k] = o.score; D.aligned[k] = o.aligned; D.matches[k] = o.matches;
      D.mismatches[k] = o.mismatches; D.gaps[k] = o.gaps;
      if (D.verdict) D.verdict[k] = (uint8_t) VSX_VERDICT_UNDECIDED;
      D.cigar_off[k] = at;
      if (hc < pl->host_cigar_pair.size() && pl->host_cigar_pair[hc] == k)
        {
          std::memcpy(blob + at, pl->host_cigar[hc].data(), pl->host_cigar[hc].size());
          at += pl->host_cigar[hc++].size();
        }
      blob[at++] = '\0';
    }
  *D.blob_used = at;
  return VSX_OK;
}

struct RankedSink {
  std::vector<uint32_t> pair, undecided;
  std::vector<int16_t> score;
  std::vector<uint16_t> aligned, matches, mismatches, gaps;
  std::vector<uint8_t> verdict;
  std::vector<double> id;
  std::vector<uint64_t> cigar_off;
  char * blob = nullptr;
  uint64_t blob_used = 0;
  int keep_weak = 0;
  ~RankedSink() { std::free(blob); }
};

static int fetch_ranked_lists(vsx_plan * pl, uint64_t first, const uint32_t * qkey, RankedSink & S, unsigned long long text_used)
// ... 524 lines not shown
```

Measured before the change: 8250.

## Add (score,1) mad-profile kernel class for pure-nucleotide targets at rows 10/26

Adds a new forward-kernel variant (nq==16) in which the query profile stores (score, 1) pairs per target code class. The row body then folds the profile pick and the H add into a single v_pk_mad_u16 with op_sel, replacing the perm plus add pair. It applies only to tilted MAX3 ONE tasks with rows 10 or 26, and only when all targets in the task are pure ACGT. Purity flags are computed on device at seqset creation. The change adds an extra purity kernel and host copy, a new template instantiation and LDS profile layout, and planner logic to route eligible tasks.

```diff
diff --git a/include/vsx.h b/include/vsx.h
--- a/include/vsx.h
+++ b/include/vsx.h
@@ -85,6 +85,7 @@
   uint64_t tasks_sparse;
   uint64_t waves;
   uint64_t tasks_pair;
+  uint64_t tasks_madprof;
 } vsx_plan_info;
 
 const char * vsx_version_string(void);
diff --git a/profiles/valu_budget.py b/profiles/valu_budget.py
--- a/profiles/valu_budget.py
+++ b/profiles/valu_budget.py
@@ -79,7 +79,9 @@
 
 def budget(body, R, S):
     c = collections.Counter()
-    quota = {"v_perm_b32": R * S, "v_add_u32_e32": R * S}
+    madp = sum(1 for op, _ in body if op == "v_pk_mad_u16") >= R * S
+    quota = {"v_perm_b32": 0 if madp else R * S, "v_add_u32_e32": 0 if madp else R * S, "v_pk_mad_u16": R * S if madp else 0}
+    pick = {"v_perm_b32", "v_pk_mad_u16"}
     npk = sum(1 for op, _ in body if op == "v_pk_sub_i16")
     nashr = sum(1 for op, _ in body if op == "v_pk_ashrrev_i16")
     pk = [("row body", S), ("last row's own e / hf subtractions", 2 * S), ("leave-column tracking", nashr)]
@@ -87,12 +89,12 @@
         if not is_valu(op):
             continue
         k = category(op, rest)
-        if k is None and op in quota:
+        if k is None and op in quota and (quota[op] > 0 or op != "v_pk_mad_u16"):
             if op == "v_add_u32_e32" and re.search(r"0x(1|2)000(1|2)\b", rest):
                 k = "leave-column tracking"
             elif quota[op] > 0:
                 quota[op] -= 1
-                k = "row body"
+                k = "score pick" if op in pick else "row body"
             else:
                 k = "checkpoint pack" if op == "v_perm_b32" else "other"
         if k is None and op == "v_pk_sub_i16":
@@ -147,10 +149,12 @@
         mp = sorted(main_path)
         loops.append(dict(head=h, end=last, main=mp, cond=cond,
                           max3=sum(1 for j in mp if ins[j][1] == "v_pk_maximum3_f16"),
+                          scratch=sum(1 for j in range(h, last + 1) if ins[j][1].startswith("scratch_")),
                           valu_main=sum(1 for j in mp if is_valu(ins[j][1])), valu_cond=sum(1 for j in cond if is_valu(ins[j][1]))))
-    print("  loops (offset range: VALU on the always-taken path + in branch-guarded regions, v_pk_maximum3_f16):")
+    print("  loops (offset range: VALU on the always-taken path + in branch-guarded regions, v_pk_maximum3_f16, scratch instructions):")
     for n, L in enumerate(loops):
-        print("    [%d] +0x%04x..+0x%04x: %4d + %4d VALU, %3d max3" % (n, ins[L["head"]][0], ins[L["end"]][0], L["valu_main"], L["valu_cond"], L["max3"]))
+        print("    [%d] +0x%04x..+0x%04x: %4d + %4d VALU, %3d max3, %d scratch" % (n, ins[L["head"]][0], ins[L["end"]][0], L["valu_main"], L["valu_cond"],
+                                                                          L["max3"], L["scratch"]))
     if not loops:
         return
     n = a.loop if a.loop is not None else max(range(len(loops)), key=lambda i: (loops[i]["max3"], -i))
@@ -163,10 +167,11 @@
     print("  loop [%d]: %d steps per iteration (R = %d)" % (n, S, R))
     print("    VALU per two steps, always-taken path: %.1f" % (2.0 * L["valu_main"] / S))
     print("    VALU in branch-guarded regions (once per 16 steps): %d" % L["valu_cond"])
-    print("    VALU per 16-step block: %.0f   per step: %.2f   (row body %d per step = %.1f %%)" % (
-        16 * per_step, per_step, 6 * R, 100.0 * 6 * R / per_step))
+    rb = (cm.get("row body", 0) + cm.get("score pick", 0)) / S
+    print("    VALU per 16-step block: %.0f   per step: %.2f   (row body incl. score pick %.0f per step = %.1f %%)" % (
+        16 * per_step, per_step, rb, 100.0 * rb / per_step))
     print("    per step, by category (always-taken path / S, + branch-guarded / 16):")
-    order = ["row body", "DPP hand-overs (feed, H, F)", "profile row addresses", "feed-slot addresses", "last row's own e / hf subtractions",
+    order = ["score pick", "row body", "DPP hand-overs (feed, H, F)", "profile row addresses", "feed-slot addresses", "last row's own e / hf subtractions",
              "leave-column tracking", "checkpoint pack", "checkpoint addresses", "register copies", "other"]
     for k in order:
         v = cm.get(k, 0) / S
@@ -174,6 +179,9 @@
             print("      %-38s %6.2f" % (k, v))
     if L["valu_cond"]:
         print("      %-38s %6.2f  (%d VALU / 16)" % ("16-step block boundary (guarded)", L["valu_cond"] / 16.0, L["valu_cond"]))
+    h = collections.Counter(op for op, _ in body if is_valu(op))
+    print("    always-taken path per step: v_perm_b32 %.2f, v_pk_mad_u16 %.2f, v_add_u32 %.2f" % (
+        h.get("v_perm_b32", 0) / S, h.get("v_pk_mad_u16", 0) / S, h.get("v_add_u32_e32", 0) / S))
     if a.ops:
         for name, lst in (("always-taken path", body), ("branch-guarded", cond)):
             h = collections.Counter(op for op, _ in lst if is_valu(op))
diff --git a/vsearch_amd/_lib.py b/vsearch_amd/_lib.py
--- a/vsearch_amd/_lib.py
+++ b/vsearch_amd/_lib.py
@@ -100,7 +100,8 @@
 class PlanInfo(C.Structure):
     _fields_ = [("tasks", C.c_uint64), ("tasks_tilted", C.c_uint64), ("tasks_tracked", C.c_uint64),
                 ("rows_dominant", C.c_uint32), ("chunks", C.c_uint32), ("tasks_max3", C.c_uint64),
-                ("tasks_sparse", C.c_uint64), ("waves", C.c_uint64), ("tasks_pair", C.c_uint64)]
+                ("tasks_sparse", C.c_uint64), ("waves", C.c_uint64), ("tasks_pair", C.c_uint64),
+                ("tasks_madprof", C.c_uint64)]
 
 
 class Timing(C.Structure):
diff --git a/vsearch_amd/csrc/ubench_valu.hip b/vsearch_amd/csrc/ubench_valu.hip
--- a/vsearch_amd/csrc/ubench_valu.hip
+++ b/vsearch_amd/csrc/ubench_valu.hip
@@ -70,6 +70,8 @@
 #define I_PKMAXU(x)   "v_pk_max_u16 " #x ", " #x ", %16\n"
 #define I_MIXAM(x)    "v_add_u32 " #x ", " #x ", %16\n" "v_pk_max_u16 " #x ", " #x ", %17\n"
 #define I_MIXAM3(x)   "v_add_u32 " #x ", " #x ", %16\n" "v_pk_maximum3_f16 " #x ", " #x ", %16, %17\n"
+#define I_PK_MADSEL(x) "v_pk_mad_u16 " #x ", %16, %17, " #x " op_sel:[0,1,0] op_sel_hi:[1,0,1]\n"
+#define I_MIXMM3(x)   "v_pk_mad_u16 " #x ", %16, %17, " #x " op_sel:[0,1,0] op_sel_hi:[1,0,1]\n" "v_pk_maximum3_f16 " #x ", " #x ", %16, %17\n"
 
 #define DEFK(NAME, INS) \
   __global__ void __launch_bounds__(256) NAME(int iters, int * out, int seed) { \
@@ -138,6 +140,8 @@
 DEFK(k3_pkmaxu, I_PKMAXU)
 DEFK(k3_mix_add_max, I_MIXAM)
 DEFK(k3_mix_add_max3, I_MIXAM3)
+DEFK(k8_pk_madsel, I_PK_MADSEL)
+DEFK(k8_mix_madsel_max3, I_MIXMM3)
 
 template <int MODE>
 __global__ void __launch_bounds__(256) k_rowbody(int iters, int * out, int seed)
@@ -245,6 +249,7 @@
   printf("device %s  CUs %d  clock %d kHz  arch %s\n", p.name, p.multiProcessorCount, p.clockRate, p.gcnArchName);
   if (getenv("UB_ROWBODY")) { for (int m = 0; m < 3; ++m) for (int w = 1; w <= 8; w *= 2) run_rowbody(w, m); run_rowbody(3, 0); return 0; }
 #define R(NAME) run(#NAME, NAME, 4);
+  if (getenv("UB_MADSEL")) { R(k_pk_mad) R(k8_pk_madsel) R(k_perm) R(k_add32) R(k3_mix_add_max3) R(k8_mix_madsel_max3) return 0; }
   if (getenv("UB_MAX3")) { R(k3_pkmaxu) R(k3_pkmax3f) R(k_add32) R(k3_mix_add_max) R(k3_mix_add_max3) return 0; }
   if (getenv("UB_NEW")) { R(k2_sub32) R(k2_subrev32) R(k2_min32) R(k2_maxu32) R(k2_ashr32) R(k2_and32) R(k2_or32) R(k2_lshl32) R(k2_addco) R(k2_addc) R(k2_min16) R(k2_addu16) R(k2_subu16) R(k2_cmp32) R(k2_lshladd) R(k2_madu24) R(k2_mulu24) R(k2_subi32c) R(k2_med3) R(k2_bfe) R(k2_addsdwa) R(k2_max16sdwa) R(k2_movdpp) R(k2_adddpp) return 0; }
   R(k_pk_add) R(k_pk_sub) R(k_pk_max) R(k_pk_min) R(k_pk_lshr) R(k_pk_ashr) R(k_pk_mad) R(k_pk_mul)
diff --git a/vsearch_amd/csrc/vsx_device.hip b/vsearch_amd/csrc/vsx_device.hip
--- a/vsearch_amd/csrc/vsx_device.hip
+++ b/vsearch_amd/csrc/vsx_device.hip
@@ -39,6 +39,8 @@
 DEV u32 a_pk_ashr15(u32 a) { u32 r; asm("v_pk_ashrrev_i16 %0, 15, %1 op_sel_hi:[0,1]" : "=v"(r) : "v"(a)); return r; }
 DEV u32 funnel(u32 acc, u32 d) { return a_bfi(SIGN2, d, a_lshr1(acc)); }
 DEV u32 pack16(int v) { const u32 x = (u32) v & 0xffffu; return x | (x << 16); }
+DEV u32 pk_mad_x(u32 a, u32 b, u32 c) { u32 r; asm("v_pk_mad_u16 %0, %1, %2, %3 op_sel:[0,1,0] op_sel_hi:[1,0,1]" : "=v"(r) : "v"(a), "v"(b), "v"(c)); return r; }
+DEV u32 madp_code(u32 c) { return ((c >> 1) - (c >> 3)) & 3u; }
 
 DEV u32 dpp_shr1(u32 feed, u32 src) { return (u32) __builtin_amdgcn_update_dpp((int) feed, (int) src, 0x111, 0xF, 0xF, false); }
 DEV u32 dpp_rol1(u32 src) { return (u32) __builtin_amdgcn_update_dpp((int) src, (int) src, 0x12F, 0xF, 0xF, false); }
@@ -75,7 +77,7 @@
 #ifndef VSX_FWD_WAVES_NQ
 #define VSX_FWD_WAVES_NQ(R_, NQ_) ((NQ_) == 4 ? 2 : ((R_) <= 24 ? 3 : 2))
 #endif
-template <int R, bool GENERIC, bool TRACK, bool CKPT, bool TILT = false, bool MAX3 = false, int NQ = 1, bool PAIR = false, bool ONE = false>
+template <int R, bool GENERIC, bool TRACK, bool CKPT, bool TILT = false, bool MAX3 = false, int NQ = 1, bool PAIR = false, bool ONE = false, bool MADP = false>
 __global__ void __launch_bounds__(PAIR ? 256 : 64) __attribute__((amdgpu_waves_per_eu(NQ == 1 ? (ONE ? VSX_FWD_WAVES_ONE(R, TILT) : VSX_FWD_WAVES(R, TILT)) : VSX_FWD_WAVES_NQ(R, NQ), 8)))
 vsx_forward_kernel(const VsxDevParams P, const VsxTask * __restrict__ tasks,
                    const uint8_t * __restrict__ qc, const uint8_t * __restrict__ tc,
@@ -108,7 +110,10 @@
   constexpr int QPBYTES = 16 * 16 * RP;
   constexpr int RPP = ((RP / 4) & 1) ? RP : RP + 4;
   __shared__ __attribute__((aligned(16))) u32 PPf[PAIR ? 16 * 16 * RPP : 4];
-  __shared__ __attribute__((aligned(16))) int16_t QP[(GENERIC && !PAIR) ? (QP8 ? (NQ * QPBYTES) / 2 : 16 * 16 * R) : 8];
+  static_assert(!MADP || (ONE && NQ == 1 && !PAIR && TILT && MAX3 && GENERIC && VSX_QPL != 0 && VSX_FEED2 != 0 && !VSX_CKT),
+                "the (score, 1)-profile classes extend the whole-wave ONE + MAX3 look-ahead kernels");
+  __shared__ __attribute__((aligned(16))) u32 PMf[MADP ? 4 * 16 * RPP : 4];
+  __shared__ __attribute__((aligned(16))) int16_t QP[(GENERIC && !PAIR && !MADP) ? (QP8 ? (NQ * QPBYTES) / 2 : 16 * 16 * R) : 8];
   uint8_t * const QPb = reinterpret_cast<uint8_t *>(QP);
   __shared__ __attribute__((aligned(16))) u32 RS[CKST ? 64 * 12 : 4];
   constexpr int FSZ = (TILT && VSX_QPL ? 2 : 1) * 4 * 16;
@@ -186,6 +191,25 @@
                   PPf[(pr * 16 + row / RP) * RPP + rr] = ((u32) va & 0xffu) | (((u32) vb & 0xffu) << 16);
                 }
             }
+          else if (MADP)
+            {
+              for (int idx = lane; idx < 4 * 16 * RP; idx += 64)
+                {
+                  const int code = idx / (16 * RP), row = idx % (16 * RP);
+                  const int Lr = 16 * s + row / RP, rr = row % RP;
+                  int v = 0;
+                  if (rr < R)
+                    {
+                      if (Lr == 0 && rr < pad) v = -P.top_step + 2 * tl;
+                      else if (Lr < total_lanes)
+                        {
+                          const int gi = (Lr == 0) ? rr - pad : rcnt0 + (Lr - 1) * R + rr;
+                          v = P.matrix[(1 << code) * 16 + (int) qq[gi]];
+                        }
+                    }
+                  PMf[(code * 16 + row / RP) * RPP + rr] = ((u32) v & 0xffu) | 0x10000u;
+                }
+            }
           else if (QP8)
             {
               constexpr int LPT = 64 / NQ;
@@ -280,6 +304,7 @@
                   f_H = (s == 0) ? bpack(rawH - pad * tl) : rawS.x;
                   f_F = (s == 0) ? vsub(f_H, qrt_i_pk) : rawS.y;
                   const u32 f_off = PAIR ? (((rawA >> 1) - (rawA >> 3)) * 4u + ((rawB >> 1) - (rawB >> 3))) * (u32) (16 * RPP * 4)
+                                  : MADP ? (madp_code(rawA) * (u32) (16 * RPP * 4) | ((madp_code(rawB) * (u32) (16 * RPP * 4)) << 16))
                                          : (rawA * (u32) (16 * RP) | ((rawB * (u32) (16 * RP)) << 16));
                   FEED4[(blk & 1) * 64 + gw * 16 + l] = make_uint4(f_off, 0u, f_H, f_F);
                   prefetch(blk + 1);
@@ -315,6 +340,7 @@
               if (FEED2)
                 {
                   const u32 f_off = PAIR ? (((rawA >> 1) - (rawA >> 3)) * 4u + ((rawB >> 1) - (rawB >> 3))) * (u32) (16 * RPP * 4)
+                                  : MADP ? (madp_code(rawA) * (u32) (16 * RPP * 4) | ((madp_code(rawB) * (u32) (16 * RPP * 4)) << 16))
                                          : (rawA * (u32) (16 * RP) | ((rawB * (u32) (16 * RP)) << 16));
                   FEED4[fo + gw * 16 + l] = make_uint4(f_off, f_sym, f_H, f_F);
                   FEEDB[fo + gw * 16 + l] = make_uint2(f_qrt, f_rt);
@@ -328,16 +354,22 @@
               prefetch(blk + 1);
       };
       constexpr int PD = RP / 4;
-      u32 profA[2][(QPL && !PAIR) ? PD : 1], profB[2][(QPL && !PAIR) ? PD : 1];
-      auto load_profile = [&](u32 (&buf)[2][(QPL && !PAIR) ? PD : 1], u32 sy) __attribute__((always_inline)) {
+      constexpr int PDX = (QPL && !PAIR && !MADP) ? PD : 1;
+      u32 profA[2][PDX], profB[2][PDX];
+      auto load_quarter = [&](u32 (&q)[4], u32 off, int k) __attribute__((always_inline)) {
+        const uint4 v = *reinterpret_cast<const uint4 *>(reinterpret_cast<const uint8_t *>(PMf + l * RPP + 4 * k) + off);
+        q[0] = v.x; q[1] = v.y; q[2] = v.z; q[3] = v.w;
+      };
+      auto load_profile = [&](u32 (&buf)[2][PDX], u32 sy) __attribute__((always_inline)) {
         if (PAIR) return;
+        if constexpr (MADP) return;
         const u32 cd = sy & 0x000F000Fu;
         constexpr int QPA = (RP % 16 == 0) ? 16 : ((RP % 8 == 0) ? 8 : 4);
         if (FEED2)
           {
             const uint8_t * pa = QPl + l * RP + (sy & 0xFFFFu);
             const uint8_t * pb = QPl + l * RP + (sy >> 16);
-            constexpr int PDN = (QPL && !PAIR) ? PD : 1;
+            constexpr int PDN = (QPL && !PAIR && !MADP) ? PD : 1;
             if constexpr (PAIR) { }
             else if constexpr (QPA == 16)
               {
@@ -370,7 +402,7 @@
         const u32 * a = reinterpret_cast<const u32 *>(QPl + (cd & 0xFu) * (16 * RP) + l * RP);
         const u32 * b = reinterpret_cast<const u32 *>(QPl + (cd >> 16) * (16 * RP) + l * RP);
 #pragma unroll
-        for (int k = 0; k < ((QPL && !PAIR) ? PD : 1); ++k) { buf[0][k] = a[k]; buf[1][k] = b[k]; }
+        for (int k = 0; k < ((QPL && !PAIR && !MADP) ? PD : 1); ++k) { buf[0][k] = a[k]; buf[1][k] = b[k]; }
       };
       if (QPL)
         {
@@ -407,7 +439,7 @@
         __syncthreads();
       };
 
-      auto step = [&](const int t, u32 (&hin)[R], u32 (&hout)[R], u32 (&pc)[2][(QPL && !PAIR) ? PD : 1], u32 (&pn)[2][(QPL && !PAIR) ? PD : 1],
+      auto step = [&](const int t, u32 (&hin)[R], u32 (&hout)[R], u32 (&pc)[2][PDX], u32 (&pn)[2][PDX],
                       auto interior_tag, auto odd_tag, auto steady_tag) __attribute__((always_inline)) {
           constexpr bool INTERIOR = decltype(interior_tag)::value;
           constexpr bool ODD = decltype(odd_tag)::value;
@@ -425,6 +457,8 @@
                   pp[k] = v.x; pp[k + 1] = v.y; pp[k + 2] = v.z; pp[k + 3] = v.w;
                 }
             }
+          u32 q0a[4], q0b[4];
+          if constexpr (MADP) { load_quarter(q0a, sym & 0xFFFFu, 0); load_quarter(q0b, sym >> 16, 0); }
           if (QPL) { if ((t & 15) == 15) build_feed((t >> 4) + 1, std::integral_constant<bool, LEANFEED> {}); }
           else if ((t & 15) == 0) build_feed(t >> 4, std::false_type {});
 
@@ -436,7 +470,7 @@
             {
               const int t1 = t + 1;
               symn = dpp_shr1(feed4_g[(u32) (((t1 >> 4) & 1) * 64 + (t1 & 15))].x, sym);
-              load_profile(pn, symn);
+              if (!MADP) load_profile(pn, symn);
             }
           else sym = dpp_shr1(fv.x, sym);
           if (!GENERIC) nd = dpp_shr1(FEEDN[gw * 16 + (t & 15)], nd);
@@ -472,11 +506,22 @@
               auto rows = [&](auto shared_tag) __attribute__((always_inline)) {
               constexpr bool SHARED = decltype(shared_tag)::value;
               constexpr bool LASTFAST = MAX3 && SHARED && CKPT;
+              u32 qa[4], qb[4], na[4], nb[4];
 #pragma unroll
               for (int r = 0; r < R; ++r)
                 {
-                  u32 V;
-                  if (PAIR) V = pp[r];
+                  u32 V = 0;
+                  if constexpr (MADP)
+                    {
+                      if ((r & 3) == 0)
+                        {
+                          const int k = r >> 2;
+#pragma unroll
+                          for (int x = 0; x < 4; ++x) { qa[x] = (k == 0) ? q0a[x] : na[x]; qb[x] = (k == 0) ? q0b[x] : nb[x]; }
+                          if (4 * (k + 1) < R) { load_quarter(na, sym & 0xFFFFu, k + 1); load_quarter(nb, sym >> 16, k + 1); }
+                        }
+                    }
+                  else if (PAIR) V = pp[r];
                   else if (GENERIC && QP8)
                     {
                       if ((r & 3) == 0)
@@ -513,7 +558,7 @@
                       else V = (u32) (uint16_t) qpA[r] | ((u32) (uint16_t) qpB[r] << 16);
                     }
                   else V = a_pk_mad(a_pk_minu(ac[r] ^ code, 0x00010001u), nd, P.match_pk);
-                  const u32 h0 = vadd(Hd, V);
+                  const u32 h0 = MADP ? pk_mad_x(qa[r & 3], qb[r & 3], Hd) : vadd(Hd, V);
                   const bool ONE_MAX = MAX3 && (r < R - 1 || LASTFAST);
                   const u32 h1 = ONE_MAX ? 0u : vmax(h0, F);
                   h2 = ONE_MAX ? pk_max3_bits(h0, F, E[r]) : vmax(h1, E[r]);
@@ -2152,6 +2197,16 @@
         }
       else return hipErrorInvalidValue;
     }
+  if (nq == 16)
+    {
+      if (!(P.tilt != 0 && P.max3 && CK && generic && !track && one)) return hipErrorInvalidValue;
+      if constexpr (CK && R >= 4 && VSX_QPL != 0 && VSX_FEED2 != 0 && !VSX_CKT)
+        {
+          VSX_FWD_GO(ntasks, R, true, false, true, true, true, 1, false, true, true);
+          return hipGetLastError();
+        }
+      else return hipErrorInvalidValue;
+    }
   if (nq != 1)
     {
       if (!(P.tilt != 0 && CK && generic && !track && (nq == 2 || nq == 4))) return hipErrorInvalidValue;
diff --git a/vsearch_amd/csrc/vsx_host.cpp b/vsearch_amd/csrc/vsx_host.cpp
--- a/vsearch_amd/csrc/vsx_host.cpp
+++ b/vsearch_amd/csrc/vsx_host.cpp
@@ -319,6 +319,14 @@
 #ifndef VSX_PAIRPROF_DEFAULT
 #define VSX_PAIRPROF_DEFAULT 1
 #endif
+#ifndef VSX_MADPROF_DEFAULT
+#define VSX_MADPROF_DEFAULT 1
+#endif
+static bool madp_rows(int rows)
+{
+  static const bool all = std::getenv("VSX_MADPROF") && std::strcmp(std::getenv("VSX_MADPROF"), "all") == 0;
+  return rows >= 4 && (all || rows == 10 || rows == 26);
+}
 static std::atomic<int> g_max3_state[64];
 static std::mutex g_ctx_mu;
 static std::vector<vsx_ctx *> g_ctxs;
@@ -797,7 +805,7 @@
   hipError_t e = hipSuccess;
   ScratchPool * pl = (code_bytes <= VSX_SEQSET_POOLED_BYTES) ? &ctx->pool : nullptr;
   if (pl) s->pool_ref = ctx->pool_owner;
-  PoolBuf<uint8_t> staging;
+  PoolBuf<uint8_t> staging, flags;
   const uint8_t * d_ascii = static_cast<const uint8_t *>(blob);
   do {
     if ((e = s->d_codes.alloc(pl, code_bytes + 2 * VSX_CODE_SLACK)) != hipSuccess) break;
@@ -825,7 +833,15 @@
         s->lower_bytes = (blob_bytes + 7) / 8;
       }
     if (both_strands && (e = vsx_launch_revcomp(s->codes(), s->d_off.p, s->d_off.p + n, s->d_len.p, n, ctx->stream)) != hipSuccess) break;
+    if (s->n)
+      {
+        if ((e = flags.alloc(pl, s->n)) != hipSuccess) break;
+        if ((e = vsx_launch_purity(s->codes(), s->d_off.p, s->d_len.p, s->n, flags.p, ctx->stream)) != hipSuccess) break;
+        s->impure.assign(s->n, 0);
+        if ((e = hipMemcpyAsync(s->impure.data(), flags.p, s->n, hipMemcpyDeviceToHost, ctx->stream)) != hipSuccess) break;
+      }
     e = hipStreamSynchronize(ctx->stream);
+    if (e == hipSuccess) s->have_impure = true;
   } while (false);
   if (e != hipSuccess)
     {
@@ -978,6 +994,9 @@
   static const bool pair_env = (std::getenv("VSX_PAIRPROF") ? std::strcmp(std::getenv("VSX_PAIRPROF"), "0") != 0 : (VSX_PAIRPROF_DEFAULT != 0)) &&
                                !arith && VSX_QPL != 0 && VSX_FEED2 != 0 && !VSX_CKT;
   const bool pair_try = pair_env && ctx->ckpt && n_pairs >= 32;
+  static const bool madp_env = (std::getenv("VSX_MADPROF") ? std::strcmp(std::getenv("VSX_MADPROF"), "0") != 0 : (VSX_MADPROF_DEFAULT != 0)) &&
+                               !arith && VSX_QPL != 0 && VSX_FEED2 != 0 && !VSX_CKT;
+  const bool madp_try = madp_env && ctx->ckpt;
 
   std::unique_ptr<vsx_plan> pl(new vsx_plan);
   pl->ctx = ctx; pl->Q = queries; pl->T = targets; pl->n_pairs = n_pairs;
@@ -1157,6 +1176,31 @@
       }
   };
   if (any_pair_cand) run_threads(nth, mark_pairs);
+  auto madp_cand = [&](const ProtoTask & pt) {
+    return pt.nq == 1 && pt.tilt == 2 && madp_rows(pt.rows) && (int64_t) queries->len[pt.q] <= 16ll * pt.rows;
+  };
+  bool any_madp_cand = false;
+  if (madp_try)
+    for (const auto & v : part)
+      {
+        for (const ProtoTask & pt : v) if (madp_cand(pt)) { any_madp_cand = true; break; }
+        if (any_madp_cand) break;
+      }
+  if (any_madp_cand)
+    {
+      const int rc = ensure_impure(targets);
+      if (rc != VSX_OK) return rc;
+      auto mark_madp = [&](int t) {
+        for (ProtoTask & pt : part[(size_t) t])
+          {
+            if (!madp_cand(pt)) continue;
+            bool pure = true;
+            for (uint32_t sidx = 0; sidx < pt.n && pure; ++sidx) pure = !targets->impure[tidx[pt.pair[sidx]]];
+            if (pure) pt.nq = 16;
+          }
+      };
+      run_threads(nth, mark_madp);
+    }
   std::vector<ProtoTask> protos;
   {
     size_t total = 0;
@@ -1512,7 +1556,7 @@
           VsxDevParams Pf = L.tilt ? ctx->Pt : ctx->P;
           Pf.max3 = (L.tilt == 2) ? 1 : 0;
           static const bool one_off = std::getenv("VSX_ONESTRIP") && std::strcmp(std::getenv("VSX_ONESTRIP"), "0") == 0;
-          HIPCHK(vsx_launch_forward(L.rows, L.generic, L.track, ctx->ckpt ? 1 : 0, L.nq, (L.multi || (one_off && L.nq != 8)) ? 0 : 1, Pf, pl->d_tasks.p + L.first, L.count,
+          HIPCHK(vsx_launch_forward(L.rows, L.generic, L.track, ctx->ckpt ? 1 : 0, L.nq, (L.multi || (one_off && L.nq != 8 && L.nq != 16)) ? 0 : 1, Pf, pl->d_tasks.p + L.first, L.count,
                                     pl->Q->codes(), pl->T->codes(), dir, pl->d_strip.p,
                                     pl->d_slot.p + (size_t) L.first * VSX_TASK_SLOTS, st));
         }
@@ -1595,6 +1639,7 @@
       {
         if (L.nq == 2 || L.nq == 4) info->tasks_sparse += L.count;
         if (L.nq == 8) info->tasks_pair += L.count;
+        if (L.nq == 16) info->tasks_madprof += L.count;
         info->waves += (L.nq == 2 || L.nq == 4) ? (L.count + (uint32_t) L.nq - 1) / (uint32_t) L.nq : L.count;
         if (L.tilt) info->tasks_tilted += L.count;
         if (L.tilt == 2) info->tasks_max3 += L.count;
```

New measurement: 8255, median of 6. Within noise of the previous version (+0.1%).
